# olofson/audiality2

Hardware: AMD Instinct MI355X
Metric: voice-samples/sec + max realtime voices @48kHz (higher is better)
Workload: dtype int32; 1 GPU; 65536 voices 2xwtosc->panmix, 256 per group voice inline->fbdelay->fbdelay (benchmark/fmtest4.a2s delay settings; 256 groups, 512 fbdelays), 48 kHz, fragment=64, stereo (BASELINE configs[3]); voices_per_gpu=65536, chain=osc2-pan, groups=256

## Files before the change

audiality2_amd/build.py:

```python
import hashlib
import os
import shutil
import subprocess

HERE = os.path.dirname(os.path.abspath(__file__))
ROOT = os.path.dirname(HERE)
HIPCC = shutil.which("hipcc") or "/opt/rocm/bin/hipcc"


MARK = b"A2AMD_SRCHASH:"


def source_hash(sources, cmd=()):
    h = hashlib.sha256()
    for s in sources:
        h.update(os.path.basename(s).encode() + b"\0")
        with open(s, "rb") as f:
            h.update(f.read())
        h.update(b"\0")
    h.update(" ".join(cmd).encode())
    return h.hexdigest()[:32]


def stamped_hash(lib, mark=MARK):
    if not os.path.exists(lib):
        return None
    with open(lib, "rb") as f:
        blob = f.read()
    i = blob.find(mark)
    if i < 0:
        return None
    return blob[i + len(mark):i + len(mark) + 32].decode("ascii", "replace")


ENGMARK = b"A2AMD_ENGHASH:"


def engine_hash(engine):
    files = []
    for d in ("include", "src", os.path.join("src", "units"), os.path.join("src", "drivers")):
        p = os.path.join(engine, d)
        if os.path.isdir(p):
            files += [os.path.join(p, f) for f in sorted(os.listdir(p)) if f.endswith((".h", ".h.cmake", ".h.in"))]
    return source_hash(files, (stamped_hash(os.path.join(HERE, "liba2amd_units.so")) or "",))


def _stale(target, want):
    return stamped_hash(target) != want


def _define(h):
    return '-DA2AMD_SRCHASH="%s"' % h


def build_lib(force=False):
    csrc = os.path.join(HERE, "csrc")
    srcs = [os.path.join(csrc, f) for f in ("a2amd_host.cpp", "a2amd_sched.cpp", "a2amd_render.cpp", "a2amd_dist.cpp",
                                            "a2amd_vm.cpp", "a2amd_kernels.hip", "a2amd_fast.hip", "a2amd_vm.hip", "a2amd_wavecap.hip", "a2amd_wavepost.hip", "a2amd_win.hip", "a2amd_vmwin.hip", "a2amd_noise.hip", "a2amd_noisepan.hip", "a2amd_noisefiltpan.hip", "a2amd_cutsweep.hip", "a2amd_oscbare.hip", "a2amd_osc3filtpan.hip")]
    deps = srcs + [os.path.join(csrc, "a2amd_host.h"), os.path.join(csrc, "a2amd_switches.h"), os.path.join(csrc, "a2amd_device.h"), os.path.join(csrc, "a2amd_dsp.h"),
                   os.path.join(csrc, "a2amd_fm.h"), os.path.join(csrc, "a2amd_vmcore.h"), os.path.join(csrc, "a2amd_taps.h"), os.path.join(csrc, "a2amd_winctl.h"), os.path.join(csrc, "a2amd_vmdev.h"), os.path.join(csrc, "a2amd_noisemap.h"), os.path.join(csrc, "a2amd_noisevoice.h"), os.path.join(csrc, "a2amd_settled.h"), os.path.join(csrc, "a2amd_cutsweep.h"), os.path.join(csrc, "a2amd_filt.h"), os.path.join(csrc, "a2amd_wavepads.h"), os.path.join(ROOT, "include", "a2amd.h"),
                   os.path.join(ROOT, "include", "a2amd_noise.h"), os.path.join(ROOT, "include", "a2amd_noisepan.h"), os.path.join(ROOT, "include", "a2amd_noisefilt.h"), os.path.join(ROOT, "include", "a2amd_sweep.h"), os.path.join(ROOT, "include", "a2amd_wavepost.h"),
                   os.path.join(ROOT, "include", "a2amd_bus.h"), os.path.join(ROOT, "include", "a2amd_oscbare.h"), os.path.join(ROOT, "include", "a2amd_osc3filt.h"), os.path.join(ROOT, "include", "a2amd_fbdpan.h"), os.path.join(ROOT, "include", "a2amd_buswin.h"), os.path.join(ROOT, "include", "a2amd_vmbatch.h"), os.path.join(ROOT, "include", "a2amd_osc2.h"), os.path.join(ROOT, "include", "a2amd_osc2lds.h"), os.path.join(ROOT, "include", "a2amd_vm.h")]
    out = os.path.join(HERE, "liba2amd.so")
    flags = ["--offload-arch=gfx950", "-O3", "-std=c++17", "-fPIC", "-shared", "-Wno-unused-value"]
    want = source_hash(deps, flags)
    if force or _stale(out, want):
        subprocess.run([HIPCC] + flags + [_define(want), "-o", out] + srcs, check=True)
    return out


def build_units(force=False):
    src = os.path.join(HERE, "csrc", "a2amd_units.c")
    deps = [src, os.path.join(ROOT, "include", "a2amd.h"), os.path.join(ROOT, "include", "a2amd_noise.h"), os.path.join(ROOT, "include", "a2amd_noisepan.h"),
            os.path.join(ROOT, "include", "a2amd_noisefilt.h"), os.path.join(ROOT, "include", "a2amd_sweep.h"), os.path.join(ROOT, "include", "a2amd_bus.h"),
            os.path.join(ROOT, "include", "a2amd_wavepost.h"), os.path.join(ROOT, "include", "a2amd_oscbare.h"), os.path.join(ROOT, "include", "a2amd_osc3filt.h"), os.path.join(ROOT, "include", "a2amd_fbdpan.h"), os.path.join(ROOT, "include", "a2amd_buswin.h"), os.path.join(ROOT, "include", "a2amd_vmbatch.h"), os.path.join(ROOT, "include", "a2amd_osc2.h"), os.path.join(ROOT, "include", "a2amd_osc2lds.h"), os.path.join(ROOT, "include", "a2amd_plugin.h"),
            os.path.join(ROOT, "include", "a2amd_walk.h"), os.path.join(ROOT, "include", "a2amd_vm.h")]
    out = os.path.join(HERE, "liba2amd_units.so")
    flags = ["-O2", "-Wall", "-fPIC", "-shared"]
    want = source_hash(deps, flags)
    if force or _stale(out, want):
        subprocess.run(["gcc"] + flags + [_define(want), "-o", out, src,
                        "-L" + HERE, "-la2amd", "-ldl", "-lpthread", "-lm", "-Wl,-rpath,$ORIGIN"], check=True)
    return out


def build_walk(force=False, engine=None):
    engine = engine or os.environ.get("A2_ENGINE_SRC", "/root/reference")
    out = os.path.join(HERE, "liba2amd_walk.so")
    src = os.path.join(HERE, "csrc", "a2amd_walk.c")
    own = [src, os.path.join(ROOT, "include", "a2amd_walk.h"), os.path.join(ROOT, "include", "a2amd_vm.h"),
           os.path.join(ROOT, "include", "a2amd_plugin.h")]
    flags = ["-O2", "-Wall", "-fPIC", "-shared"]
    want = source_hash(own, flags)
    kept = os.path.join(ROOT, "oracle", "_ref", "liba2amd_walk.so")
    if not (os.path.exists(os.path.join(engine, "src", "internals.h")) and shutil.which("cmake")):
        if (not os.path.exists(out) or _stale(out, want)) and not _stale(kept, want):
            shutil.copyfile(kept, out)
        if os.path.exists(out) and _stale(out, want):
            raise RuntimeError(f"{out} was not built from this tree's a2amd_walk.c (stamp {stamped_hash(out)}, "
                               f"sources {want}) and the engine's source tree ({engine}) is not here to rebuild it")
        return out if os.path.exists(out) else None
    inc = os.path.join(HERE, "_engine_include")
    weng = engine_hash(engine)
    if force or _stale(out, want) or stamped_hash(out, ENGMARK) != weng:
        subprocess.run(["cmake", f"-DENGINE={engine}", f"-DOUT={inc}", "-P", os.path.join(HERE, "csrc", "engine_header.cmake")],
                       check=True, stdout=subprocess.DEVNULL)
        subprocess.run(["gcc"] + flags + [_define(want), '-DA2AMD_ENGHASH="%s"' % weng, "-I" + inc] +
                       ["-I" + os.path.join(engine, d) for d in ("include", "src", "src/units", "src/drivers")] +
                       ["-o", out, src, "-L" + HERE, "-la2amd_units", "-la2amd", "-ldl", "-lpthread", "-Wl,-rpath,$ORIGIN"],
                       check=True)
    if stamped_hash(kept) != want or stamped_hash(kept, ENGMARK) != weng:
        os.makedirs(os.path.dirname(kept), exist_ok=True)
        shutil.copyfile(out, kept)
    return out


def build_oracle(force=False):
    odir = os.path.join(ROOT, "oracle")
    targets = ["restate"]
    if os.path.exists("/root/reference/src/core.c") and shutil.which("cmake"):
        targets += ["ref", "tools", "optionb"]
    subprocess.run(["make", "-s", "-C", odir] + (["-B"] if force else []) + targets, check=True)
    return os.path.join(odir, "liba2oracle.so")


def build_all(force=False):
    lib = build_lib(force)
    build_units(force)
    build_walk(force)
    return lib, build_oracle(force)
```

audiality2_amd/csrc/a2amd_device.h:

```cpp
#pragma once
#include <stdint.h>

#define A2D_MAXCHAIN   16
#define A2D_CHAIN_INLINE 8
#define A2D_MAXBATCH 256
#define FBW_MAXWIN (2 * A2D_MAXBATCH)
#define A2D_USTATE    24
#define A2D_MAXCH      8
#define A2D_FRAG      64
#define A2D_MIPS      10
#define A2D_FBD_BUFSIZE 131072
#define A2D_MAXPHINC  512
#define A2D_COEF_WORDS 3
#define A2D_WTOSC_MAXLENGTH (0x01000000 - 1 - 131)

enum { A2D_WTOSC = 0, A2D_PANMIX, A2D_FILTER12, A2D_FBDELAY, A2D_INLINE, A2D_XINSERT,
	A2D_FM1, A2D_FM2, A2D_FM3, A2D_FM4, A2D_FM3P, A2D_FM4P, A2D_FM2R, A2D_FM4R,
	A2D_DC, A2D_WAVESHAPER, A2D_DCBLOCK, A2D_LIMITER, A2D_XSINK, A2D_XSOURCE };
#define A2D_IS_FM(k) ((k) >= A2D_FM1 && (k) <= A2D_FM4R)

enum { A2D_OSC_OFF = 0, A2D_OSC_NOISE, A2D_OSC_WAVE, A2D_OSC_MIPWAVE };

#define A2D_DESC(kind, add, nin, nout, wired) \
	(((uint32_t)(kind) << 24) | ((uint32_t)(add) << 4) | ((uint32_t)(nin) << 8) | \
	 ((uint32_t)(nout) << 12) | ((uint32_t)(wired) << 16))
#define A2D_KIND(d)  ((d) >> 24)
#define A2D_ADD(d)   (((d) >> 4) & 1u)
#define A2D_NIN(d)   (((d) >> 8) & 15u)
#define A2D_NOUT(d)  (((d) >> 12) & 15u)
#define A2D_WIRED(d) (((d) >> 16) & 1u)

enum {
	OW_MODE = 0, OW_WAVE, OW_DPHASE, OW_PHASE_LO, OW_PHASE_HI, OW_NOISE,
	OW_PRAMPING, OW_P = 7, OW_A = 11, OW_SEED = 15 };
enum {
	PW_VOL = 0, PW_PAN = 4 };
enum {
	FW_Q = 0, FW_LP = 4, FW_BP, FW_HP, FW_F1, FW_D1A, FW_D1B, FW_D2A, FW_D2B,
	FW_F1NEXT, FW_RAMP };
enum {
	DW_FBDELAY = 0, DW_LDELAY, DW_RDELAY, DW_DRYGAIN, DW_FBGAIN, DW_LGAIN,
	DW_RGAIN, DW_BUFPOS, DW_BUFIDX };

enum {
	CW_VALUE = 0, CW_MODE = 4 };
enum {
	SW_AMOUNT = 0 };
enum {
	BW_F1 = 0, BW_D1A, BW_D1B, BW_D2A, BW_D2B };
enum {
	LW_RELEASE = 0, LW_THRESHOLD, LW_PEAK };
enum {
	MW_SLOT = 0 };
enum {
	FO_A = 0, FO_FB = 4, FO_P = 8, FO_LASTPITCH = 12, FO_PHASE, FO_DPHASE, FO_LAST, FO_WORDS };
#define A2D_FMSTATE 64

#define A2D_WF_RAWTAPS 0x40000000u

struct A2DWave {
	int32_t  type;
	uint32_t flags;
	uint32_t period;
	uint32_t size[A2D_MIPS];
	uint32_t off[A2D_MIPS];
	uint32_t periodic;
};

struct A2DVoice {
	int32_t nunits;
	int32_t unit[A2D_CHAIN_INLINE];
	int32_t out_off, out_nch;
	int32_t own_off, own_nch;
	int32_t pad[3];
};

static_assert(sizeof(A2DVoice) == 64, "the voice record is one 64-byte line");
struct A2DVoiceExt { int32_t unit[A2D_MAXCHAIN - A2D_CHAIN_INLINE]; };

struct A2DRec {
	uint32_t head;
	int32_t  value;
	uint32_t dur;
	uint32_t start;
};
enum { R_SEG = 1, R_WRITE, R_INIT, R_KILL, R_F1SET, R_F1RAMP, R_NOISESEED, R_NOP };
#define A2D_HEAD(frag, op, unit, reg) \
	((uint32_t)(frag) | ((uint32_t)(op) << 16) | ((uint32_t)(unit) << 24) | ((uint32_t)(reg) << 28))
#define A2D_RFRAG(h) ((h) & 0xffffu)
#define A2D_ROP(h)   (((h) >> 16) & 0xffu)
#define A2D_RUNIT(h) (((h) >> 24) & 15u)
#define A2D_RREG(h)  (((h) >> 28) & 15u)

struct A2DRun { int32_t first, count; };

#define A2D_VM_NOWRITE 0xffu
#define A2D_VM_TRAPWRITE 0xfeu
#define A2D_VM_MAXCUT  2
#define A2D_VM_MAXENV  2
#define A2D_VM_MAXPOS  8
#define A2D_VM_ENVPOS  14
#define A2D_ENV_LUTSHIFT 6
#define A2D_ENV_LUTSIZE  (1 << A2D_ENV_LUTSHIFT)
#define A2D_ENV_LUTS     8
struct A2DVmEnv {
	int32_t ramper[4];
	int32_t lut;
	int32_t scale, offset, out;
	int32_t active;
	uint8_t regbase;
	uint8_t k;
	uint8_t target;
	uint8_t pad;
};
struct A2DVmVoice {
	uint32_t waketime;
	uint32_t code, ncode;
	uint16_t pc;
	uint8_t  state, ncut;
	int32_t  voice;
	int32_t  fault;
	uint8_t  cmap[64];
	uint8_t  kind[A2D_MAXCHAIN];
	uint8_t  cutpos[A2D_VM_MAXCUT];
	uint8_t  pad[2];
	int32_t  cut[A2D_VM_MAXCUT][4];
	A2DVmEnv env[A2D_VM_MAXENV];
	int32_t  nenv;
	uint32_t exit_when;
	int32_t  has_exit;
	int32_t  r[64];
};

struct A2DVmParams {
	A2DVmVoice     *vmv;
	const int      *list;
	int32_t         n;
	const uint32_t *code;
	const uint32_t *ptab;
	const int32_t  *f1tab;
	const uint16_t *envlut;
	A2DRun         *runs;
	A2DRun         *vmrun;
	A2DRec         *recs;
	uint32_t        rec_base, rec_cap;
	uint32_t       *total;
	uint32_t        now;
	uint32_t        msdur;
	int32_t         samplerate, basepitch;
	int32_t         nfrags;
	uint8_t         fragframes[A2D_MAXBATCH];
	uint8_t         fragbase[A2D_MAXBATCH];
};

enum { XW_SLOT = 0, XW_MODE = 1 };
#define A2D_XIO_HALF ((size_t)A2D_MAXBATCH * 8 * A2D_FRAG)
#define A2D_XIO_SLOT (2 * A2D_XIO_HALF)

#define A2D_FAST_FCH 8
#define A2D_OSC2_FCH 4
#define A2D_OSC2_SCH 16
#define A2D_OSC2_LDS_ENT 128
#define A2D_MAXVPW   32

struct A2DParams {
	const A2DVoice *voices;
	const A2DVoiceExt *vext;
	const uint32_t *udesc;
	int32_t        *ustate;
	int32_t        *vactive;
	const A2DRun   *runs;
	const A2DRec   *recs;
	const A2DWave  *waves;
	const int16_t  *wavepool;
	const int32_t  *wavecoef;
	int32_t        *busmem;
	int32_t        *fbdmem;
	const uint32_t *ptab;
	int32_t        *fmstate;
	const uint32_t *fmsine;
	int32_t *xio;
	const uint32_t *nseed;
	const int32_t  *nslot;
	int32_t         nnoise;
	const int32_t  *cutf;
	const int32_t  *cslot;
	int32_t         ncut;
	int32_t         nfrags;
	int32_t         samplerate;
	int32_t         debug;
	uint8_t         fragframes[A2D_MAXBATCH];
	uint16_t        fragstart[A2D_MAXBATCH];
};

#ifdef __HIPCC__
#define A2D_HD static inline __host__ __device__
#else
#define A2D_HD static inline
#endif
A2D_HD bool a2d_osc2_slice(int nfrags, int ysplit, int slice, int *c_lo, int *c_hi, int *nslices)
{
	const int nchunks = (nfrags + A2D_OSC2_FCH - 1) / A2D_OSC2_FCH;
	const int per = (nchunks + ysplit - 1) / ysplit;
	*c_lo = slice * per;
	*c_hi = *c_lo + per < nchunks ? *c_lo + per : nchunks;
	*nslices = (nchunks + per - 1) / per;
	return *c_lo < nchunks;
}
A2D_HD bool a2d_osc2_whole(unsigned start_first, unsigned start_last, unsigned frames_last, int n)
{
	return start_last + frames_last - start_first == (unsigned)n * A2D_FRAG;
}

A2D_HD unsigned a2d_osc2_stage(unsigned size0, unsigned periodic0, unsigned size1, unsigned periodic1)
{
	const bool c0 = periodic0 && size0 && !(size0 & (size0 - 1)) && size0 <= A2D_OSC2_LDS_ENT;
	const bool c1 = periodic1 && size1 && !(size1 & (size1 - 1)) && size1 <= A2D_OSC2_LDS_ENT;
	return (c0 ? 1u : 0u) | (c1 && (c0 ? size0 : 0u) + size1 <= A2D_OSC2_LDS_ENT ? 2u : 0u);
}

#ifdef __HIPCC__
static inline __host__ __device__ bool a2d_noise_seed(const A2DParams &p, int f, int ui, unsigned *seed)
{
	if(!p.nseed)
		return false;
	const int k = p.nslot[ui];
	if(k <= 0 || k > p.nnoise)
		return false;
	*seed = p.nseed[(size_t)f * (size_t)p.nnoise + (size_t)(k - 1)];
	return true;
}
#endif

#ifdef __HIPCC__
static inline __host__ __device__ bool a2d_cut_coeff(const A2DParams &p, int f, int ui, int *f1)
{
	if(p.ncut <= 0)
		return false;
#if defined(__HIP_DEVICE_COMPILE__)
	typedef const __attribute__((address_space(4))) A2DParams *CP;
	typedef const __attribute__((address_space(4))) int32_t *CI;
	uintptr_t qa = (uintptr_t)&p;
	asm volatile("" : "+s"(qa));
	const CP q = (CP)qa;
	const int ncut = q->ncut;
	const int k = *((CI)(uintptr_t)q->cslot + ui);
	if(k <= 0 || k > ncut)
		return false;
	const int v = *((CI)(uintptr_t)q->cutf + ((size_t)f * (size_t)ncut + (size_t)(k - 1)));
#else
	const int k = p.cslot[ui];
	if(k <= 0 || k > p.ncut)
		return false;
	const int v = p.cutf[(size_t)f * (size_t)p.ncut + (size_t)(k - 1)];
#endif
	if(v < 0)
		return false;
	*f1 = v;
	return true;
}
#endif

struct A2DCutSweep { int32_t ramper[4]; int32_t unit, slot, pad[2]; };
int a2d_launch_cut_sweep(const A2DCutSweep *list, int n, int f0, int count, unsigned frames, int32_t *cutf, int stride,
		size_t words, int32_t *cslot, int nunits, void *stream);
int a2d_launch_cut_resolve(int32_t *cutf, size_t words, const int32_t *f1tab, void *stream);

struct A2DNoiseOsc { uint32_t ph_lo, ph_hi, dphase; int32_t unit, slot, pad[3]; };
int a2d_launch_noise_seeds(const A2DNoiseOsc *osc, int n, uint32_t start, int f0, int count, unsigned frames,
		uint32_t *seed, int stride, size_t seed_words, int32_t *nslot, int nunits, void *stream);

int a2d_launch_leaf_noisepan(const A2DParams *dparams, const A2DParams &hp, const int *dlist, int nlist, int vpw, void *stream);
int a2d_launch_leaf_noisefiltpan(const A2DParams *dparams, const A2DParams &hp, const int *dlist, int nlist, int vpg, void *stream);
int a2d_launch_leaf_oscbare(const A2DParams *dparams, const A2DParams &hp, const int *dlist, int nlist, int vpw, void *stream);
int a2d_launch_leaf_osc3filtpan(const A2DParams *dparams, const A2DParams &hp, const int *dlist, int nlist, int vpg, void *stream);

int a2d_launch_vm(const A2DVmParams &vp, int emit, void *stream);
int a2d_launch_vm_pool(const A2DVmParams &vp, unsigned *out, void *stream);
#define A2D_WIN_STAGED 2
struct A2DVmwOut {
	A2DVmVoice *vmv;
	int        *ustate;
	int        *vactive;
	A2DRun     *runs;
	uint32_t   *total;
	uint32_t   *idle;
};
int a2d_launch_vm_commit(const A2DVmParams &vp, const A2DParams &hp, int nosc, int filt, const A2DVmwOut &from, void *stream);
int a2d_launch_vm_win(const A2DVmParams &vp, const A2DParams &hp, int nosc, int filt, int fa, int fb, uint32_t now_fa,
		uint32_t batch_end, int *wslot, int *wext, int *wscr, unsigned *widx, unsigned *wtop, unsigned wcap, void *stream,
		const A2DVmwOut *out = nullptr);
#define A2D_VMW_ROW (64 - 1 - 1)

int a2d_launch_voices(const A2DParams *dparams, const int *dlist, int nlist, int vpw, void *stream);
enum { A2D_STAGED_NONE = 0, A2D_STAGED_PHASES, A2D_STAGED_FULL };
struct A2DCommit { const int *list; int nlist, nosc; const int *ustage; const unsigned char *staged; };
struct A2DCommitSet { A2DCommit c[2]; int n; };
int a2d_launch_leaf_oscpan(const A2DParams *dparams, const A2DParams &hp, const int *dlist, int nlist,
		int vpw, int ysplit, int *ustage, unsigned char *staged, void *stream, void *event_after_main, A2DCommit *defer);
int a2d_launch_bus_driver(const A2DParams *dparams, const int *dlist, int nlist, int nfrags, int consume,
		const A2DCommitSet *commits, void *stream, int *master_host = nullptr, int ramping = 0);
int a2d_launch_commit(const A2DParams &hp, const A2DCommit &cm, void *stream);
int a2d_launch_bus_fbdchain(const A2DParams *dparams, const int *dlist, int nlist, int consume, void *stream);
int a2d_launch_bus_fbdpan(const A2DParams *dparams, const int *dlist, int nlist, int consume, void *stream, int windows = 0);
int a2d_launch_park(int32_t *stage, int32_t *bus, unsigned words, void *stream);
int a2d_launch_add_bus(int32_t *dst, int32_t *src, unsigned words, void *stream);
int a2d_launch_add_inject(const int32_t *inj, int32_t *bus, int nch, int n, int nfrags, void *stream);
int a2d_launch_build_coef(const int16_t *pool, int *coef, unsigned lo, unsigned hi, void *stream);
int a2d_launch_capture(const int32_t *bus, int32_t *dst, const uint32_t *fragpos, int nfrags, int nch, void *stream);
int a2d_launch_wave_from_pcm(const int32_t *pcm, int16_t *pool, const uint32_t *off, const uint32_t *size, int levels, int looped,
		int pre, int post, void *stream);
int a2d_launch_wave_level0(const int32_t *pcm, int16_t *d, unsigned size, void *stream);
int a2d_launch_wave_finish(int16_t *pool, const uint32_t *off, const uint32_t *size, int levels, int looped, int pre, int post,
		void *stream);
unsigned a2d_wavepost_scratch_words(unsigned size, unsigned flags, unsigned chunk);
int a2d_launch_wave_level0_post(const int32_t *pcm, int16_t *d, unsigned size, unsigned flags, unsigned chunk, uint32_t *scratch,
		void *stream);
int a2d_osc2filtpan_max_vpg(void);
int a2d_launch_leaf_osc2filtpan(const A2DParams *dparams, const A2DParams &hp, const int *dlist, int nlist,
		int vpg, void *stream);
int a2d_launch_leaf_oscfiltpan(const A2DParams *dparams, const A2DParams &hp, const int *dlist, int nlist,
		int vpw, void *stream);
int a2d_launch_scatter_runs(const int *didx, const A2DRun *dval, int n, A2DRun *druns, void *stream);
int a2d_launch_leaf_osc2pan(const A2DParams *dparams, const A2DParams &hp, const int *dlist, int nlist,
		int vpw, int ysplit, int *ustage, unsigned char *staged, void *stream, A2DCommit *defer, int voice_major, int lds_taps,
		int *ysplit_used);
struct A2Switches;
int a2d_launch_leaf_recs(const A2Switches &sw, const A2DParams *dparams, const A2DParams &hp, int nosc, int filt, const int *dlist,
		int nlist, int vpw, void *stream, int skip_empty = 0);
#define A2D_WIN_WORDS 24
#define A2D_WIN_SLOTWORDS(nosc, filt) ((filt) ? ((nosc) == 1 ? 20 : 24) : ((nosc) == 1 ? 12 : 20))
int a2d_launch_win_ctl(const A2DParams *dparams, const A2DParams &hp, int nosc, int filt, const int *dlist, int nlist,
		int skip_empty, int fa, int fb, int *wslot, int *wext, unsigned *widx, unsigned *wtop, unsigned wcap, int *wrc,
		void *stream);
int a2d_launch_win_render(const A2Switches &sw, const A2DParams &hp, int nosc, int filt, const int *dlist, int nlist, int fa, int fb,
		const int *wslot, const int *wext, const unsigned *widx, void *stream);
int a2d_launch_leaf_recs_all(const A2Switches &sw, const A2DParams *dparams, const A2DParams &hp, const int *const *lists, const int *counts,
		int vpw, void *stream, int skip_mask = 0);
int a2d_launch_leaf_fmpan(const A2DParams *dparams, const A2DParams &hp, int kind, const int *dlist, int nlist,
		int vpw, void *stream);
int a2d_launch_leaf_fmpan_all(const A2DParams *dparams, const A2DParams &hp, const int *dlist,
		const int *count8, int vpw, void *stream);
```

audiality2_amd/csrc/a2amd_fast.hip:

```cpp
#include <hip/hip_runtime.h>
#include <type_traits>
#include <algorithm>
#include <stdlib.h>
#include "a2amd_device.h"
#include "a2amd_switches.h"
#include "a2amd_dsp.h"
#include "a2amd_fm.h"
#include "a2amd_filt.h"

#include "a2amd_taps.h"

__global__ void k_build_coef(const int16_t *__restrict__ pool, int *__restrict__ coef, unsigned lo, unsigned hi)
{
	const unsigned j = lo + blockIdx.x * blockDim.x + threadIdx.x;
	if(j >= hi)
		return;
	const int dm = pool[j - 1], d0 = pool[j], d1 = pool[j + 1], d2 = pool[j + 2];
	const int c = (d1 - dm) >> 1;
	const int a = (3 * (d0 - d1) + d2 - dm) >> 1;
	const int b = dm - d0 + c - a;
	int *e = coef + A2D_COEF_WORDS * (size_t)j;
	e[0] = a;
	e[1] = b;
	e[2] = (int)(((unsigned)c << 16) | ((unsigned)d0 & 0xffffu));
}

int a2d_launch_build_coef(const int16_t *pool, int *coef, unsigned lo, unsigned hi, void *stream)
{
	if(hi <= lo)
		return 0;
	hipLaunchKernelGGL(k_build_coef, dim3((hi - lo + 255) / 256), dim3(256), 0, (hipStream_t)stream, pool, coef, lo, hi);
	return (int)hipGetLastError();
}

__device__ __attribute__((noinline)) int cold_ramp_delta(int target, int value, int timer, int frames,
		int *newtimer)
{
	if(frames <= (timer >> 8)) {
		*newtimer = wsub(timer, frames << 8);
		if(timer > 0)
			return (int)div_trunc_exact((int64_t)wsub(target, value) * 256, timer);
		return (int)((((int64_t)wsub(target, value)) * 256) / timer);
	}
	*newtimer = 0;
	if(frames > 0)
		return (int)div_trunc_exact((int64_t)wsub(target, value), frames);
	return wsub(target, value) / frames;
}

__device__ __attribute__((noinline)) uint64_t cold_umod64(uint64_t a, uint64_t m)
{
	return a % m;
}

DEV uint64_t wrap_phase(uint64_t ph, unsigned size)
{
	if(ph >> 56) {
		uint64_t r = cold_umod64(ph, (uint64_t)size << 24);
		return (uint64_t)(unsigned)rfl((int)(unsigned)r) | ((uint64_t)(unsigned)rfl((int)(unsigned)(r >> 32)) << 32);
	}
	unsigned hi = (unsigned)(ph >> 24);
	if(hi >= size) {
		if(!(size & (size - 1)))
			hi &= size - 1;
		else
			hi = (unsigned)rfl((int)(hi % size));
		ph = ((uint64_t)hi << 24) | (ph & 0xffffffu);
	}
	return ph;
}

DEV void ramp_prepare_s(Ramp &r, int frames)
{
	if(r.timer == 0) {
		r.value = r.target;
		r.delta = 0;
	} else {
		int nt;
		int d = cold_ramp_delta(r.target, r.value, r.timer, frames, &nt);
		r.delta = rfl(d);
		r.timer = rfl(nt);
	}
}

struct OscS {
	int mode, wave;
	unsigned dphase;
	uint64_t phase;
	int p_ramping;
	Ramp p, a;
	int noise;
	unsigned seed;
};

struct FastPtrs {
	const int16_t *wavepool;
	const A2DWave *waves;
	const uint32_t *ptab;
	int dbg;
};

struct OscPend { Quad16 qa, qb; unsigned ph, ph2; int ak, x; bool taps; };

DEV int osc_fragment_end(const OscPend &pd)
{
	if(pd.taps)
		return mul64s(inter_quads(pd.qa, pd.qb, pd.ph, pd.ph2), pd.ak, 17);
	return pd.x;
}

DEV OscPend osc_fragment_begin(const FastPtrs &g, OscS &o, int nframes, int lane)
{
	OscPend pd;
	pd.qa.lo = pd.qa.hi = pd.qb.lo = pd.qb.hi = 0;
// ... 55 lines not shown
		ramp_prepare_s(o.a, nframes);
		const uint64_t phk = o.phase + (uint64_t)(unsigned)(in ? lane : 0) * o.dphase;
		const uint64_t nph = phk + o.dphase;
		const bool draw = in && ((o.dphase >= (1u << 23)) || ((nph ^ phk) >> 23));
		const unsigned long long m = __ballot(draw);
		const int me = (int)(threadIdx.x & 63);
		const unsigned long long below = (me >= 63) ? ~0ull : ((2ull << me) - 1ull);
		const int mine = __popcll(m & below), total = __popcll(m);
		int held = o.noise, myval = o.noise;
		unsigned st = o.seed;
		for(int j = 1; j <= total; ++j) {
			held = noise_next(st) - 32767;
			if(j == mine)
				myval = held;
		}
		o.seed = st;
		o.noise = held;
		if(in) {
			int ak = wadd(o.a.value, wmul(o.a.delta, lane));
			x = wmul(myval, ak >> 10) >> 6;
		}
		o.phase += (uint64_t)(unsigned)nframes * o.dphase;
		ramp_run(o.a, nframes);
	} else {
		ramp_prepare_s(o.p, nframes);
		ramp_prepare_s(o.a, nframes);
		ramp_run(o.p, nframes);
		ramp_run(o.a, nframes);
	}
	pd.x = x;
	return pd;
}

DEV int osc_fragment_s(const FastPtrs &g, OscS &o, int nframes, int lane)
{
	const OscPend pd = osc_fragment_begin(g, o, nframes, lane);
	return osc_fragment_end(pd);
}

DEV void pan_fragment_s(Ramp &vol, Ramp &pan, int x, int nframes, int lane, int &acc0, int &acc1)
{
	const bool clamp = a2s_pan_over(pan.target) || a2s_pan_over(pan.value);
	ramp_prepare_s(vol, nframes);
	ramp_prepare_s(pan, nframes);
	if((unsigned)lane < (unsigned)nframes) {
		int vk = wadd(vol.value, wmul(vol.delta, lane));
		int pk = wadd(pan.value, wmul(pan.delta, lane));
		int vp = mul64s(pk, vk, 24);
		int v0 = wsub(vk, vp), v1 = wadd(vk, vp);
		if(clamp) {
			int lim = wshl(vk, 1);
			if(v0 > lim) v0 = lim;
			if(v1 > lim) v1 = lim;
		}
		acc0 = wadd(acc0, mul64s(x, v0, 24));
		acc1 = wadd(acc1, mul64s(x, v1, 24));
	}
	ramp_run(vol, nframes);
	ramp_run(pan, nframes);
}

DEV void oscpan_fragment(const FastPtrs &g, OscS &o, Ramp &vol, Ramp &pan,
		int nframes, int lane, int &acc0, int &acc1)
{
	int x = osc_fragment_s(g, o, nframes, lane);
	pan_fragment_s(vol, pan, x, nframes, lane, acc0, acc1);
}

DEV int frames_of(const int (&ffr)[A2D_MAXBATCH / 64], int f)
{
	int r = 0;
#pragma unroll
	for(int k = 0; k < A2D_MAXBATCH / 64; ++k)
		if((f >> 6) == k)
			r = rdl(ffr[k], f & 63);
	return r;
}

enum { SV_MODE = 0, SV_WAVE, SV_DPHASE, SV_PHLO, SV_PHHI, SV_PRAMP, SV_P = 6, SV_A = 10,
	SV_VOL = 14, SV_PAN = 18, SV_NWORDS = 22 };

enum { DV_SETTLED = 0, DV_MM, DV_DPH, DV_SIZEM, DV_DOFF, DV_V0, DV_V1, DV_NWORDS };

DEV bool settled_wave(const A2DWave *w, unsigned dphase, int *d, bool settled = true, unsigned *periodic = nullptr)
{
	unsigned dph;
	const unsigned mm = a2s_mip(dphase, w->period, &dph);
	d[0] = (int)mm;
	d[1] = (int)dph;
	d[2] = (int)w->size[mm];
	d[3] = (int)w->off[mm];
	if(periodic)
		*periodic = (w->periodic >> mm) & 1u;
	return settled && a2s_wave_ok(w->size[0], w->flags, dph);
}

DEV void osc_from_mem(OscS &o, const volatile int *w)
{
	o.mode = rfl(w[OW_MODE]);
	o.wave = rfl(w[OW_WAVE]);
	o.dphase = (unsigned)rfl(w[OW_DPHASE]);
	o.phase = (uint64_t)(unsigned)rfl(w[OW_PHASE_LO]) | ((uint64_t)(unsigned)rfl(w[OW_PHASE_HI]) << 32);
	o.p_ramping = rfl(w[OW_PRAMPING]);
	o.p.value = rfl(w[OW_P]); o.p.target = rfl(w[OW_P + 1]);
	o.p.delta = rfl(w[OW_P + 2]); o.p.timer = rfl(w[OW_P + 3]);
	o.a.value = rfl(w[OW_A]); o.a.target = rfl(w[OW_A + 1]);
	o.a.delta = rfl(w[OW_A + 2]); o.a.timer = rfl(w[OW_A + 3]);
	o.noise = 0;
	o.seed = 0;
}

DEV void osc_to_mem(int *w, const OscS &o)
{
	w[OW_MODE] = o.mode;
	w[OW_WAVE] = o.wave;
	w[OW_DPHASE] = (int)o.dphase;
	w[OW_PHASE_LO] = (int)(unsigned)o.phase;
	w[OW_PHASE_HI] = (int)(unsigned)(o.phase >> 32);
	w[OW_PRAMPING] = o.p_ramping;
	w[OW_P] = o.p.value; w[OW_P + 1] = o.p.target; w[OW_P + 2] = o.p.delta; w[OW_P + 3] = o.p.timer;
	w[OW_A] = o.a.value; w[OW_A + 1] = o.a.target; w[OW_A + 2] = o.a.delta; w[OW_A + 3] = o.a.timer;
}

DEV void stage_mark(unsigned char *m, bool mine, bool settled, bool last_slice, bool walker)
{
	if(mine && !settled) {
		if(walker)
			*m = A2D_STAGED_FULL;
	} else if(last_slice)
		*m = mine ? A2D_STAGED_PHASES : A2D_STAGED_NONE;
}

#define OSC1_WPE 4
__global__ __launch_bounds__(64 * FAST_WPB) __attribute__((amdgpu_waves_per_eu(OSC1_WPE, OSC1_WPE)))
void k_leaf_oscpan(const A2DParams *__restrict__ pp, const int *__restrict__ list, int nlist, int vpw,
		int ysplit, const A2DVoice *__restrict__ voices, const int *ustate,
		int *ustage, const int16_t *__restrict__ wavepool,
		const A2DWave *__restrict__ waves, const uint32_t *__restrict__ ptab, int *__restrict__ busmem,
		const int *__restrict__ wavecoef, unsigned char *__restrict__ staged)
{
	const A2DParams &p = *pp;
	const int wv = rfl((int)(threadIdx.x >> 6));
	const int lane = threadIdx.x & 63;
	const int first = (blockIdx.x * FAST_WPB + wv) * vpw;
	if(first >= nlist)
		return;
	const int nv = min(vpw, nlist - first);
	const int nfrags = p.nfrags;
	const int dbg = p.debug;
	FastPtrs g = { wavepool, waves, ptab, dbg };
	const CoefRsrc crs = coef_rsrc(wavecoef);

	const int nchunks = (nfrags + FAST_FCH - 1) / FAST_FCH;
	const int per = (nchunks + ysplit - 1) / ysplit;
	const int slice = blockIdx.y;
	const int c_lo = slice * per, c_hi = min(nchunks, c_lo + per);
	const bool last_slice = c_hi >= nchunks;
	if(c_lo >= nchunks)
		return;
	const int nslices = (nchunks + per - 1) / per;

	int ffr[A2D_MAXBATCH / 64], fst[A2D_MAXBATCH / 64];
#pragma unroll
	for(int k = 0; k < A2D_MAXBATCH / 64; ++k) {
		ffr[k] = (k * 64 + lane < nfrags) ? p.fragframes[k * 64 + lane] : 0;
		fst[k] = (k * 64 + lane < nfrags) ? p.fragstart[k * 64 + lane] : 0;
	}

	int dv[DV_NWORDS], amp_l = 0, phlo_l = 0, phhi_l = 0;
	int u0 = 0, u1 = 0, my_off = -1, my_nch = 2;
	bool mine = false;
#pragma unroll
	for(int k = 0; k < DV_NWORDS; ++k)
		dv[k] = 0;
	if(lane < nv)
		mine = p.runs[list[first + lane]].count == 0;
// ... 183 lines not shown
			flush_acc(busmem, cur_off, cur_nch, f0, nf, lane, dbg, acc0, acc1);
			__builtin_amdgcn_fence(__ATOMIC_RELEASE, "wavefront");
			__builtin_amdgcn_s_waitcnt(0);
		}
	}

	if(mine && dv[DV_SETTLED] && last_slice) {
		int *w0 = ustage + (size_t)u0 * A2D_USTATE;
		w0[OW_PHASE_LO] = phlo_l;
		w0[OW_PHASE_HI] = phhi_l;
	}
	if(ustage != ustate && lane < nv)
		stage_mark(staged + first + lane, mine, dv[DV_SETTLED] != 0, last_slice, lane % nslices == slice);
}

DEV void commit_block(const A2DCommit &cm, int block, const A2DVoice *__restrict__ voices, int *__restrict__ ustate)
{
	const int i = block * 256 + threadIdx.x;
	if(i >= cm.nlist * cm.nosc)
		return;
	const int e = i / cm.nosc, o = i - e * cm.nosc;
	const int what = cm.staged[e];
	if(what == A2D_STAGED_NONE)
		return;
	const A2DVoice &vc = voices[cm.list[e]];
	const size_t a = (size_t)vc.unit[o] * A2D_USTATE;
	ustate[a + OW_PHASE_LO] = cm.ustage[a + OW_PHASE_LO];
	ustate[a + OW_PHASE_HI] = cm.ustage[a + OW_PHASE_HI];
	if(what != A2D_STAGED_FULL)
		return;
	for(int k = 0; k < 15; ++k)
		if(k != OW_NOISE && k != OW_PHASE_LO && k != OW_PHASE_HI)
			ustate[a + k] = cm.ustage[a + k];
	if(o == 0) {
		const size_t ap = (size_t)vc.unit[cm.nosc] * A2D_USTATE;
		for(int k = 0; k < 8; ++k)
			ustate[ap + k] = cm.ustage[ap + k];
	}
}

DEV int commit_blocks(const A2DCommit &cm) { return (cm.nlist * cm.nosc + 255) / 256; }

__global__ __launch_bounds__(256)
void k_commit_oscpan(A2DCommit cm, const A2DVoice *__restrict__ voices, int *__restrict__ ustate)
{
	commit_block(cm, blockIdx.x, voices, ustate);
}

#define OSC2_FCH A2D_OSC2_FCH
#define OSC2_SCH A2D_OSC2_SCH
static_assert(OSC2_SCH % OSC2_FCH == 0, "a super-chunk is whole chunks");
enum { OV_MODE = 0, OV_WAVE, OV_DPHASE, OV_PHLO, OV_PHHI, OV_PRAMP, OV_P = 6, OV_A = 10, OV_NWORDS = 14 };
enum { OD_MM = 0, OD_DPH, OD_SIZEM, OD_DOFF, OD_NWORDS };

DEV void osc_from_lanes(OscS &o, const int (&so)[OV_NWORDS], int v)
{
	o.mode = rdl(so[OV_MODE], v);
	o.wave = rdl(so[OV_WAVE], v);
	o.dphase = (unsigned)rdl(so[OV_DPHASE], v);
	o.phase = (uint64_t)(unsigned)rdl(so[OV_PHLO], v) | ((uint64_t)(unsigned)rdl(so[OV_PHHI], v) << 32);
	o.p_ramping = rdl(so[OV_PRAMP], v);
	o.p.value = rdl(so[OV_P], v); o.p.target = rdl(so[OV_P + 1], v);
	o.p.delta = rdl(so[OV_P + 2], v); o.p.timer = rdl(so[OV_P + 3], v);
	o.a.value = rdl(so[OV_A], v); o.a.target = rdl(so[OV_A + 1], v);
	o.a.delta = rdl(so[OV_A + 2], v); o.a.timer = rdl(so[OV_A + 3], v);
	o.noise = 0;
	o.seed = 0;
}

DEV void osc_to_lanes(int (&so)[OV_NWORDS], const OscS &o, bool me)
{
	WRL(so[OV_MODE], o.mode);
	WRL(so[OV_WAVE], o.wave);
	WRL(so[OV_DPHASE], (int)o.dphase);
	WRL(so[OV_PHLO], (int)(unsigned)o.phase);
	WRL(so[OV_PHHI], (int)(unsigned)(o.phase >> 32));
	WRL(so[OV_PRAMP], o.p_ramping);
	WRL(so[OV_P], o.p.value); WRL(so[OV_P + 1], o.p.target);
	WRL(so[OV_P + 2], o.p.delta); WRL(so[OV_P + 3], o.p.timer);
	WRL(so[OV_A], o.a.value); WRL(so[OV_A + 1], o.a.target);
	WRL(so[OV_A + 2], o.a.delta); WRL(so[OV_A + 3], o.a.timer);
}

struct Osc2Voice {
	unsigned dph[2], sizem[2];
	int cb[2], amp[2];
	uint64_t ph[2], end[2];
};
struct Osc2Lds {
	const LdsInt *level[2];
	unsigned lg[2];
};

template<bool WHOLE, int ST = 0>
DEV void osc2_chunk(const CoefRsrc &crs, Osc2Voice &s, const unsigned (&ldph)[2], const int (&nfr)[OSC2_FCH],
		const unsigned (&pre)[OSC2_FCH], int nf, bool park, int (&xs)[OSC2_FCH], const Osc2Lds &lv = Osc2Lds())
{
	Coef4 ka[2][OSC2_FCH], kb[2][OSC2_FCH];
	unsigned pa[2][OSC2_FCH], pb[2][OSC2_FCH];
#pragma unroll
	for(int o = 0; o < 2; ++o) {
		const unsigned dph = s.dph[o], sizem = s.sizem[o];
		uint64_t ph = s.ph[o];
		uint64_t phs[OSC2_FCH];
		if(!(sizem & (sizem - 1)) && !(ph >> 48)) {
			const uint64_t mask = ((uint64_t)sizem << 24) - 1;
#pragma unroll
			for(int j = 0; j < OSC2_FCH; ++j)
				phs[j] = (ph + (uint64_t)dph * (WHOLE ? (unsigned)(j * A2D_FRAG) : pre[j])) & mask;
			ph = phs[OSC2_FCH - 1] + (uint64_t)dph * (WHOLE ? (unsigned)A2D_FRAG : (unsigned)nfr[OSC2_FCH - 1]);
		} else {
#pragma unroll
			for(int j = 0; j < OSC2_FCH; ++j) {
				ph = wrap_phase(ph, sizem);
				phs[j] = ph;
				ph += (uint64_t)dph * (WHOLE ? (unsigned)A2D_FRAG : (unsigned)nfr[j]);
			}
		}
#pragma unroll
		for(int j = 0; j < OSC2_FCH; ++j) {
			pa[o][j] = tap_phase(phs[j], ldph[o]);
			asm("" : "+v"(pa[o][j]));
			pb[o][j] = pa[o][j] + (dph >> 17);
			if((ST >> o) & 1) {
				ka[o][j] = coef_lds(lv.level[o], pa[o][j], lv.lg[o]);
				kb[o][j] = coef_lds(lv.level[o], pb[o][j], lv.lg[o]);
			} else {
				ka[o][j] = coef_at(crs, s.cb[o], pa[o][j]);
				kb[o][j] = coef_at(crs, s.cb[o], pb[o][j]);
			}
		}
		if(park) {
			uint64_t e = ph;
#pragma unroll
			for(int j = OSC2_FCH - 2; j >= 0; --j)
				if(nf == j + 1)
					e = phs[j] + (uint64_t)dph * (WHOLE ? (unsigned)A2D_FRAG : (unsigned)nfr[j]);
			s.end[o] = e;
		}
		s.ph[o] = ph;
	}
#pragma unroll
	for(int o = 0; o < 2; ++o)
#pragma unroll
		for(int j = 0; j < OSC2_FCH; ++j) {
			const int y = mul64s(inter_coefs(ka[o][j], pa[o][j], kb[o][j], pb[o][j]), s.amp[o], 17);
			xs[j] = o ? wadd(xs[j], y) : y;
		}
}

DEV void osc2_voice_from_lanes(Osc2Voice &s, unsigned (&ldph)[2], unsigned (&mm)[2], const int (&od)[2][OD_NWORDS],
		const int (&amp_l)[2], const int (&phlo_l)[2], const int (&phhi_l)[2], int v, unsigned before, int lane)
{
#pragma unroll
	for(int o = 0; o < 2; ++o) {
		mm[o] = (unsigned)rdl(od[o][OD_MM], v);
		s.dph[o] = (unsigned)rdl(od[o][OD_DPH], v);
		s.sizem[o] = (unsigned)rdl(od[o][OD_SIZEM], v);
		s.cb[o] = coef_base((unsigned)rdl(od[o][OD_DOFF], v));
		s.amp[o] = rdl(amp_l[o], v);
		const uint64_t phase = (uint64_t)(unsigned)rdl(phlo_l[o], v) | ((uint64_t)(unsigned)rdl(phhi_l[o], v) << 32);
		s.ph[o] = (phase >> mm[o]) + (uint64_t)before * s.dph[o];
		ldph[o] = lane_dph(lane, s.dph[o]);
	}
}

template<int ST>
DEV void osc2_voice_chunks(const CoefRsrc &crs, Osc2Voice &s, const unsigned (&ldph)[2], const unsigned (&mm)[2],
		const Osc2Lds &lv, int nsc, int nfs, bool last, int v0, int v1, int v, int lane, int (*tile)[2][A2D_FRAG],
		int (&phlo_l)[2], int (&phhi_l)[2])
{
	const int nopre_i[OSC2_FCH] = { 0, 0, 0, 0 };
	const unsigned nopre_u[OSC2_FCH] = { 0, 0, 0, 0 };
	for(int k = 0; k < nsc; ++k) {
		const bool park = last && k == nsc - 1;
		int xs[OSC2_FCH];
		osc2_chunk<true, ST>(crs, s, ldph, nopre_i, nopre_u, nfs - k * OSC2_FCH, park, xs, lv);
#pragma unroll
		for(int j = 0; j < OSC2_FCH; ++j) {
			tile_add(&tile[k * OSC2_FCH + j][0][lane], mul64s(xs[j], v0, 24));
			tile_add(&tile[k * OSC2_FCH + j][1][lane], mul64s(xs[j], v1, 24));
		}
		if(park) {
			const bool me = lane == v;
#pragma unroll
			for(int o = 0; o < 2; ++o) {
				const uint64_t endph = s.end[o] << mm[o];
				WRL(phlo_l[o], (int)(unsigned)endph);
				WRL(phhi_l[o], (int)(unsigned)(endph >> 32));
			}
		}
	}
}

template<bool STAGE>
DEV void osc2_superchunk(const CoefRsrc &crs, const int *wavecoef, int *busmem, const int (&od)[2][OD_NWORDS],
		const int (&amp_l)[2], int (&phlo_l)[2], int (&phhi_l)[2], int settled_l, int my_off, int my_nch, int v0l, int v1l,
		int nv, int nsc, int fa, int nfs, bool last, unsigned before, int lane, int dbg, int (*tile)[2][A2D_FRAG],
		LdsInt *level)
{
	int cur_off = rdl(my_off, 0), cur_nch = rdl(my_nch, 0);
	for(int v = 0; v < nv; ++v) {
		const int sl = rdl(settled_l, v);
		if(!sl)
			continue;
		const int voff = rdl(my_off, v);
		if(voff != cur_off) {
			flush_tile(busmem, cur_off, cur_nch, fa, nfs, nsc * OSC2_FCH, lane, dbg, tile);
			cur_off = voff;
			cur_nch = rdl(my_nch, v);
		}
		const int v0 = rdl(v0l, v), v1 = rdl(v1l, v);
		Osc2Voice s;
		unsigned ldph[2], mm[2];
		osc2_voice_from_lanes(s, ldph, mm, od, amp_l, phlo_l, phhi_l, v, before, lane);
		Osc2Lds lv = { { level, level }, { 0, 0 } };
		if(!STAGE) {
			osc2_voice_chunks<0>(crs, s, ldph, mm, lv, nsc, nfs, last, v0, v1, v, lane, tile, phlo_l, phhi_l);
			continue;
		}
		const int st = sl >> 1;
		if(st) {
			lds_wave_fence();
			if(st & 1) {
				lv.lg[0] = (unsigned)__builtin_ctz(s.sizem[0]);
				stage_level(level, wavecoef, s.cb[0], s.sizem[0], lane);
			}
			if(st & 2) {
				LdsInt *const l1 = (st & 1) ? level + s.sizem[0] * A2D_COEF_WORDS : level;
				lv.level[1] = l1;
				lv.lg[1] = (unsigned)__builtin_ctz(s.sizem[1]);
				stage_level(l1, wavecoef, s.cb[1], s.sizem[1], lane);
			}
			lds_wave_fence();
		}
		switch(st) {
		case 0: osc2_voice_chunks<0>(crs, s, ldph, mm, lv, nsc, nfs, last, v0, v1, v, lane, tile, phlo_l, phhi_l); break;
		case 1: osc2_voice_chunks<1>(crs, s, ldph, mm, lv, nsc, nfs, last, v0, v1, v, lane, tile, phlo_l, phhi_l); break;
		case 2: osc2_voice_chunks<2>(crs, s, ldph, mm, lv, nsc, nfs, last, v0, v1, v, lane, tile, phlo_l, phhi_l); break;
		default: osc2_voice_chunks<3>(crs, s, ldph, mm, lv, nsc, nfs, last, v0, v1, v, lane, tile, phlo_l, phhi_l); break;
		}
	}
	flush_tile(busmem, cur_off, cur_nch, fa, nfs, nsc * OSC2_FCH, lane, dbg, tile);
}

#define OSC2_WPE 4
__global__ __launch_bounds__(64 * FAST_WPB) __attribute__((amdgpu_waves_per_eu(OSC2_WPE, OSC2_WPE)))
void k_leaf_osc2pan(const A2DParams *__restrict__ pp, const int *__restrict__ list, int nlist, int vpw,
		int ysplit, const A2DVoice *__restrict__ voices, const int *ustate, int *ustage,
		const int16_t *__restrict__ wavepool, const A2DWave *__restrict__ waves,
		const uint32_t *__restrict__ ptab, int *__restrict__ busmem, const int *__restrict__ wavecoef,
		unsigned char *__restrict__ staged, int vmajor, int lds_taps)
{
	const A2DParams &p = *pp;
	const int wv = rfl((int)(threadIdx.x >> 6));
	const int lane = threadIdx.x & 63;
	const int first = (blockIdx.x * FAST_WPB + wv) * vpw;
	if(first >= nlist)
		return;
	const int nv = min(vpw, nlist - first);
	const int nfrags = p.nfrags;
	const int dbg = p.debug;
	FastPtrs g = { wavepool, waves, ptab, dbg };
	const CoefRsrc crs = coef_rsrc(wavecoef);

	const int slice = blockIdx.y;
	int c_lo, c_hi, nslices;
	if(!a2d_osc2_slice(nfrags, ysplit, slice, &c_lo, &c_hi, &nslices))
		return;
	const bool last_slice = c_hi * OSC2_FCH >= nfrags;

	int ffr[A2D_MAXBATCH / 64], fst[A2D_MAXBATCH / 64];
#pragma unroll
	for(int k = 0; k < A2D_MAXBATCH / 64; ++k) {
		ffr[k] = (k * 64 + lane < nfrags) ? p.fragframes[k * 64 + lane] : 0;
		fst[k] = (k * 64 + lane < nfrags) ? p.fragstart[k * 64 + lane] : 0;
	}

	int od[2][OD_NWORDS], amp_l[2] = { 0, 0 }, phlo_l[2] = { 0, 0 }, phhi_l[2] = { 0, 0 };
	int v0l = 0, v1l = 0, settled_l = 0;
	int uu[3] = { 0, 0, 0 }, my_off = -1, my_nch = 2;
	bool mine = false;
#pragma unroll
	for(int o = 0; o < 2; ++o)
#pragma unroll
		for(int k = 0; k < OD_NWORDS; ++k)
			od[o][k] = 0;
	if(lane < nv)
		mine = p.runs[list[first + lane]].count == 0;
	if(mine) {
		const A2DVoice &vc = voices[list[first + lane]];
		my_off = vc.out_off;
		my_nch = vc.out_nch;
		bool settled = true;
		int wave_l[2], dphase_l[2];
		unsigned periodic[2] = { 0, 0 };
#pragma unroll
		for(int o = 0; o < 2; ++o) {
			uu[o] = vc.unit[o];
			const int *w = ustate + (size_t)uu[o] * A2D_USTATE;
			wave_l[o] = w[OW_WAVE];
			dphase_l[o] = w[OW_DPHASE];
			amp_l[o] = w[OW_A];
			phlo_l[o] = w[OW_PHASE_LO];
			phhi_l[o] = w[OW_PHASE_HI];
			settled = settled && a2s_osc_settled(w[OW_MODE], (unsigned)dphase_l[o], w[OW_PRAMPING], w + OW_P, w + OW_A);
		}
		uu[2] = vc.unit[2];
		const int *wp = ustate + (size_t)uu[2] * A2D_USTATE;
		int sp[8];
#pragma unroll
		for(int k = 0; k < 8; ++k)
			sp[k] = wp[k];
		settled = settled && a2s_arrived(sp + PW_VOL, sp + PW_PAN);
		if(settled) {
#pragma unroll
			for(int o = 0; o < 2; ++o)
				settled = settled_wave(waves + wave_l[o], (unsigned)dphase_l[o], od[o], settled, &periodic[o]);
			a2s_pan_gains(sp[PW_VOL], sp[PW_PAN], a2s_pan_over(sp[PW_PAN]), &v0l, &v1l);
		}
		settled_l = settled ? 1 : 0;
		if(settled && lds_taps)
			settled_l |= (int)a2d_osc2_stage((unsigned)od[0][OD_SIZEM], periodic[0], (unsigned)od[1][OD_SIZEM], periodic[1]) << 1;
	}
	const unsigned long long unsettled_mask = __ballot(mine && !settled_l);
	const bool any_staged = __ballot(settled_l > 1) != 0;

	__shared__ int tiles[FAST_WPB][OSC2_SCH][2][A2D_FRAG];
	__shared__ int levels[FAST_WPB][A2D_OSC2_LDS_ENT * A2D_COEF_WORDS];
	int (*const tile)[2][A2D_FRAG] = tiles[wv];
	LdsInt *const level = (LdsInt *)levels[wv];
	if(vmajor)
#pragma unroll
		for(int r = 0; r < OSC2_SCH; ++r)
			tile[r][0][lane] = tile[r][1][lane] = 0;
	for(int s_lo = c_lo; s_lo < c_hi; s_lo += OSC2_SCH / OSC2_FCH) {
		const int s_hi = min(c_hi, s_lo + OSC2_SCH / OSC2_FCH);
		const int fa = s_lo * OSC2_FCH, nfs = min(nfrags, s_hi * OSC2_FCH) - fa;
		const bool last = last_slice && s_hi == c_hi;
		const unsigned before = (unsigned)frames_of(fst, fa);
		if(vmajor && a2d_osc2_whole(before, (unsigned)frames_of(fst, fa + nfs - 1), (unsigned)frames_of(ffr, fa + nfs - 1), nfs)) {
			if(any_staged)
				osc2_superchunk<true>(crs, wavecoef, busmem, od, amp_l, phlo_l, phhi_l, settled_l, my_off, my_nch, v0l, v1l,
						nv, s_hi - s_lo, fa, nfs, last, before, lane, dbg, tile, level);
			else
				osc2_superchunk<false>(crs, wavecoef, busmem, od, amp_l, phlo_l, phhi_l, settled_l, my_off, my_nch, v0l, v1l,
						nv, s_hi - s_lo, fa, nfs, last, before, lane, dbg, tile, level);
			continue;
		}
		for(int c = s_lo; c < s_hi; ++c) {
			const int f0 = c * OSC2_FCH;
			const int nf = min((int)OSC2_FCH, nfrags - f0);
			int acc0[OSC2_FCH], acc1[OSC2_FCH], nfr[OSC2_FCH];
#pragma unroll
			for(int j = 0; j < OSC2_FCH; ++j) {
				acc0[j] = acc1[j] = 0;
				nfr[j] = (j < nf) ? frames_of(ffr, f0 + j) : 0;
			}
			const unsigned before = (unsigned)frames_of(fst, f0);
			unsigned pre[OSC2_FCH];
			pre[0] = 0;
#pragma unroll
			for(int j = 1; j < OSC2_FCH; ++j)
				pre[j] = pre[j - 1] + (unsigned)nfr[j - 1];
			const bool park = last && c == s_hi - 1;
			int cur_off = rdl(my_off, 0), cur_nch = rdl(my_nch, 0);
			for(int v = 0; v < nv; ++v) {
				if(!rdl(settled_l, v))
					continue;
				const int voff = rdl(my_off, v);
				if(voff != cur_off) {
					flush_acc(busmem, cur_off, cur_nch, f0, nf, lane, dbg, acc0, acc1);
					cur_off = voff;
					cur_nch = rdl(my_nch, v);
				}
				const int v0 = rdl(v0l, v), v1 = rdl(v1l, v);
				Osc2Voice s;
				unsigned ldph[2], mm[2];
				int xs[OSC2_FCH];
				osc2_voice_from_lanes(s, ldph, mm, od, amp_l, phlo_l, phhi_l, v, before, lane);
				osc2_chunk<false>(crs, s, ldph, nfr, pre, nf, park, xs);
#pragma unroll
				for(int j = 0; j < OSC2_FCH; ++j) {
					const int x = (lane < nfr[j]) ? xs[j] : 0;
					acc0[j] = wadd(acc0[j], mul64s(x, v0, 24));
					acc1[j] = wadd(acc1[j], mul64s(x, v1, 24));
				}
				if(park) {
					const bool me = lane == v;
#pragma unroll
					for(int o = 0; o < 2; ++o) {
						const uint64_t endph = s.end[o] << mm[o];
						WRL(phlo_l[o], (int)(unsigned)endph);
						WRL(phhi_l[o], (int)(unsigned)(endph >> 32));
					}
				}
			}
			flush_acc(busmem, cur_off, cur_nch, f0, nf, lane, dbg, acc0, acc1);
		}
	}

	const unsigned long long todo_mask = unsettled_mask & __ballot(lane % nslices == slice);
	if(todo_mask) {
		for(int f0 = 0; f0 < nfrags; f0 += OSC2_FCH) {
			const int nf = min((int)OSC2_FCH, nfrags - f0);
			int acc0[OSC2_FCH], acc1[OSC2_FCH];
#pragma unroll
			for(int j = 0; j < OSC2_FCH; ++j)
				acc0[j] = acc1[j] = 0;
			int cur_off = rdl(my_off, 0), cur_nch = rdl(my_nch, 0);
			for(int v = 0; v < nv; ++v) {
				if(!((todo_mask >> v) & 1ull))
					continue;
				const int voff = rdl(my_off, v);
				if(voff != cur_off) {
					flush_acc(busmem, cur_off, cur_nch, f0, nf, lane, dbg, acc0, acc1);
					cur_off = voff;
					cur_nch = rdl(my_nch, v);
				}
				OscS oa, ob;
				Ramp vol, pan;
				const int *src = f0 ? ustage : ustate;
				osc_from_mem(oa, src + (size_t)rdl(uu[0], v) * A2D_USTATE);
				osc_from_mem(ob, src + (size_t)rdl(uu[1], v) * A2D_USTATE);
				{
// ... 1838 lines not shown
						++r;
					wk = lane - ((fr[r][4] >> 8) & 0xff);
				}
				const int vk = wadd(fr[r][0], wmul(fr[r][1], wk));
				const int pk = wadd(fr[r][2], wmul(fr[r][3], wk));
				const int vp = mul64s(pk, vk, 24);
				v0 = wsub(vk, vp); v1 = wadd(vk, vp);
				if(WIN ? fr[r][4] & 1 : fr[r][4]) {
					const int lim = wshl(vk, 1);
					if(v0 > lim) v0 = lim;
					if(v1 > lim) v1 = lim;
				}
			}
			const int o0 = mul64s(x0, v0, 24), o1 = mul64s(x1, v1, 24);
			int *dst = out + (size_t)f * out_nch * A2D_FRAG;
			if(o0)
				atomicAdd(&dst[lane], o0);
			if(o1)
				atomicAdd(&dst[A2D_FRAG + lane], o1);
		}
		if(fend < nfrags)
			__syncthreads();
	}
	if(threadIdx.x == 0) {
		int total = 0;
		for(int f = 0; f < nfrags; ++f)
			total += p.fragframes[f];
#pragma unroll
		for(int k = 0; k < FBC_MAXD; ++k)
			if(k < nd)
				p.ustate[(size_t)vc.unit[k + 1] * A2D_USTATE + DW_BUFPOS] = wadd(d[k].pos, total);
	}
}

__global__ __launch_bounds__(FBC_THREADS)
void k_bus_fbdpan(const A2DParams *__restrict__ pp, const int *__restrict__ list, int nlist, int consume)
{
	bus_fbdpan<false>(pp, list, consume);
}

__global__ __launch_bounds__(FBC_THREADS)
void k_bus_fbdpan_win(const A2DParams *__restrict__ pp, const int *__restrict__ list, int nlist, int consume)
{
	bus_fbdpan<true>(pp, list, consume);
}

int a2d_launch_bus_fbdpan(const A2DParams *dparams, const int *dlist, int nlist, int consume, void *stream, int windows)
{
	if(nlist <= 0)
		return 0;
	hipLaunchKernelGGL(windows ? k_bus_fbdpan_win : k_bus_fbdpan, dim3(nlist), dim3(FBC_THREADS), 0, (hipStream_t)stream,
			dparams, dlist, nlist, consume);
	return (int)hipGetLastError();
}

int a2d_launch_leaf_oscpan(const A2DParams *dparams, const A2DParams &hp, const int *dlist, int nlist,
		int vpw, int ysplit, int *ustage, unsigned char *staged, void *stream, void *event_after_main, A2DCommit *defer)
{
	if(nlist <= 0)
		return 0;
	vpw = vpw < 1 ? 1 : (vpw > 64 ? 64 : vpw);
	if(ysplit < 1 || !ustage || !staged)
		ysplit = 1;
	int nwaves = (nlist + vpw - 1) / vpw;
	int nblocks = (nwaves + FAST_WPB - 1) / FAST_WPB;
	hipLaunchKernelGGL(k_leaf_oscpan, dim3(nblocks, ysplit), dim3(64 * FAST_WPB), 0, (hipStream_t)stream,
			dparams, dlist, nlist, vpw, ysplit, hp.voices, (const int *)hp.ustate,
			ysplit > 1 ? ustage : hp.ustate, hp.wavepool, hp.waves, hp.ptab, hp.busmem, hp.wavecoef, staged);
	if(event_after_main)
		hipEventRecord((hipEvent_t)event_after_main, (hipStream_t)stream);
	if(ysplit > 1) {
		A2DCommit cm = { dlist, nlist, 1, ustage, staged };
		if(defer)
			*defer = cm;
		else
			a2d_launch_commit(hp, cm, stream);
	} else if(defer)
		defer->nlist = 0;
	return (int)hipGetLastError();
}

int a2d_launch_leaf_osc2pan(const A2DParams *dparams, const A2DParams &hp, const int *dlist, int nlist,
		int vpw, int ysplit, int *ustage, unsigned char *staged, void *stream, A2DCommit *defer, int voice_major, int lds_taps,
		int *ysplit_used)
{
	if(nlist <= 0)
		return 0;
	vpw = vpw < 1 ? 1 : (vpw > 64 ? 64 : vpw);
	if(ysplit < 1 || !ustage || !staged)
		ysplit = 1;
	if(ysplit_used)
		*ysplit_used = ysplit;
	int nwaves = (nlist + vpw - 1) / vpw;
	int nblocks = (nwaves + FAST_WPB - 1) / FAST_WPB;
	hipLaunchKernelGGL(k_leaf_osc2pan, dim3(nblocks, ysplit), dim3(64 * FAST_WPB), 0, (hipStream_t)stream,
			dparams, dlist, nlist, vpw, ysplit, hp.voices, (const int *)hp.ustate,
			ysplit > 1 ? ustage : hp.ustate, hp.wavepool, hp.waves, hp.ptab, hp.busmem, hp.wavecoef, staged, voice_major, lds_taps);
	if(ysplit > 1) {
		A2DCommit cm = { dlist, nlist, 2, ustage, staged };
		if(defer)
			*defer = cm;
		else
			a2d_launch_commit(hp, cm, stream);
	} else if(defer)
		defer->nlist = 0;
	return (int)hipGetLastError();
}

__global__ void k_scatter_runs(const int *__restrict__ idx, const A2DRun *__restrict__ val, int n,
		A2DRun *__restrict__ runs)
{
	int i = blockIdx.x * blockDim.x + threadIdx.x;
	if(i < n)
		runs[idx[i]] = val[i];
}

int a2d_launch_scatter_runs(const int *didx, const A2DRun *dval, int n, A2DRun *druns, void *stream)
{
	if(n <= 0)
		return 0;
	hipLaunchKernelGGL(k_scatter_runs, dim3((n + 255) / 256), dim3(256), 0, (hipStream_t)stream,
			didx, dval, n, druns);
	return (int)hipGetLastError();
}

int a2d_launch_leaf_oscfiltpan(const A2DParams *dparams, const A2DParams &hp, const int *dlist, int nlist,
		int vpg, void *stream)
{
	if(nlist <= 0)
		return 0;
	vpg = vpg < 1 ? 1 : (vpg > FILT_MAXV ? FILT_MAXV : vpg);
	int nblocks = (nlist + vpg - 1) / vpg;
	size_t lds = (size_t)3 * vpg * FILT_PITCH * sizeof(int);
	hipLaunchKernelGGL(k_leaf_oscfiltpan, dim3(nblocks), dim3(64 * FILT_WAVES), lds, (hipStream_t)stream,
			dparams, dlist, nlist, vpg, hp.voices, hp.ustate, hp.wavepool, hp.waves, hp.ptab, hp.busmem, hp.wavecoef);
	return (int)hipGetLastError();
}

int a2d_osc2filtpan_max_vpg(void)
{
	const int nfull = FILT_WAVES - 1 - (FILT_WAVES / 4 - 1);
	const int v = nfull * (FILT2_LAUNCHV < FILT2_FASTV ? FILT2_LAUNCHV : FILT2_FASTV);
	return v > FILT_MAXV ? FILT_MAXV : v;
}

int a2d_launch_leaf_osc2filtpan(const A2DParams *dparams, const A2DParams &hp, const int *dlist, int nlist,
		int vpg, void *stream)
{
	if(nlist <= 0)
		return 0;
	vpg = vpg < 1 ? 1 : (vpg > FILT_MAXV ? FILT_MAXV : vpg);
	int nblocks = (nlist + vpg - 1) / vpg;
	size_t lds = (size_t)3 * vpg * FILT_PITCH * sizeof(int);
	hipLaunchKernelGGL(k_leaf_osc2filtpan, dim3(nblocks), dim3(64 * FILT_WAVES), lds, (hipStream_t)stream,
			dparams, dlist, nlist, vpg, hp.voices, hp.ustate, hp.wavepool, hp.waves, hp.ptab, hp.busmem, hp.wavecoef);
	return (int)hipGetLastError();
}

enum { PV_VOL = 0, PV_PAN = 4, PV_NWORDS = 8 };

DEV void pan_window_s(Ramp &vol, Ramp &pan, int x, int off, int len, int lane, int &acc0, int &acc1)
{
	const bool clamp = a2s_pan_over(pan.target) || a2s_pan_over(pan.value);
	ramp_prepare_s(vol, len);
	ramp_prepare_s(pan, len);
	const int k = lane - off;
	if(k >= 0 && k < len) {
		int vk = wadd(vol.value, wmul(vol.delta, k));
		int pk = wadd(pan.value, wmul(pan.delta, k));
		int vp = mul64s(pk, vk, 24);
		int v0 = wsub(vk, vp), v1 = wadd(vk, vp);
		if(clamp) {
			int lim = wshl(vk, 1);
			if(v0 > lim) v0 = lim;
			if(v1 > lim) v1 = lim;
		}
		acc0 = wadd(acc0, mul64s(x, v0, 24));
		acc1 = wadd(acc1, mul64s(x, v1, 24));
	}
	ramp_run(vol, len);
// ... 459 lines not shown
```

audiality2_amd/csrc/a2amd_host.cpp:

```cpp
#include "a2amd_host.h"
#include "a2amd_noisemap.h"
#include "a2amd_cutsweep.h"
#include "a2amd_settled.h"
#include "a2amd_wavepads.h"

namespace a2h { thread_local char g_err[256] = ""; }

extern "C" {

const char *a2amd_version(void) { return "a2amd 0.1 (gfx950)"; }
#ifndef A2AMD_SRCHASH
#define A2AMD_SRCHASH "unstamped"
#endif
const char *a2amd_source_stamp(void) { return "A2AMD_SRCHASH:" A2AMD_SRCHASH; }

const char *a2amd_last_error(const a2amd_ctx *c) { return c ? c->err : g_err; }

int a2amd_device_count(void)
{
	int n = 0;
	return hipGetDeviceCount(&n) == hipSuccess ? n : 0;
}


int a2amd_open(const a2amd_config *cfg, a2amd_ctx **out)
{
	if(!cfg || !out || cfg->channels < 1 || cfg->channels > A2D_MAXCH || cfg->samplerate <= 0) {
		snprintf(g_err, sizeof(g_err), "a2amd_open: bad configuration");
		return A2AMD_EINVAL;
	}
	int ndev = 0;
	hipError_t e = hipGetDeviceCount(&ndev);
	if(e != hipSuccess || ndev <= 0 || cfg->device >= ndev) {
		snprintf(g_err, sizeof(g_err), "a2amd_open: no usable HIP device (%s, %d devices, want #%d); "
				"this library has no CPU fallback", hipGetErrorString(e), ndev, cfg->device);
		return A2AMD_ENODEVICE;
	}
	a2amd_ctx *c = new a2amd_ctx();
	c->cfg = *cfg;
	c->err[0] = 0;
	if(!c->cfg.max_batch)
		c->cfg.max_batch = 1;
	if(c->cfg.max_batch > A2D_MAXBATCH)
		c->cfg.max_batch = A2D_MAXBATCH;
	memset(&c->stats, 0, sizeof(c->stats));
	build_pitch_table(c->ptab);
	a2amd_read_switches(&c->sw);
	c->bus_stride_frames = (size_t)c->cfg.max_batch * A2D_FRAG;
	c->bus_used = c->bus_stride_frames * (size_t)c->cfg.channels;
#define OPENCHK(call) do { hipError_t e_ = (call); if(e_ != hipSuccess) { \
	snprintf(g_err, sizeof(g_err), "a2amd_open: %s: %s", #call, hipGetErrorString(e_)); \
	delete c; return A2AMD_EHIP; } } while(0)
	OPENCHK(hipSetDevice(cfg->device));
	if(cfg->stream)
		c->stream = (hipStream_t)cfg->stream;
	else {
		OPENCHK(hipStreamCreateWithFlags(&c->stream, hipStreamNonBlocking));
		c->own_stream = true;
	}
	OPENCHK(hipEventCreate(&c->ev0));
	OPENCHK(hipEventCreate(&c->ev1));
	OPENCHK(hipEventCreate(&c->ev2));
	c->ev_pool.push_back(c->ev0);
	c->ev_pool.push_back(c->ev1);
	c->ev_pool.push_back(c->ev2);
	OPENCHK(hipMalloc((void **)&c->d_ptab, sizeof(c->ptab)));
	OPENCHK(hipMalloc((void **)&c->d_wavepool.d, (size_t)(8u << 20) * sizeof(int16_t)));
	c->d_wavepool.cap = 8u << 20;
	OPENCHK(hipMalloc((void **)&c->d_wavecoef.d, (size_t)(8u << 20) * A2D_COEF_WORDS * sizeof(int32_t)));
	c->d_wavecoef.cap = 8u << 20;
#undef OPENCHK
	*out = c;
	return A2AMD_OK;
}

void a2amd_close(a2amd_ctx *c)
{
	if(!c)
		return;
	use_device(c);
	hipStreamSynchronize(c->stream);
	if(c->vm.pred_stream)
		hipStreamSynchronize(c->vm.pred_stream);
	drop_graphs(c);
	if(c->comm && g_rccl.CommDestroy)
		g_rccl.CommDestroy(c->comm);
	if(c->grp_ev)
		hipEventDestroy(c->grp_ev);
	hipFree(c->d_voices.d); hipFree(c->d_vext.d); hipFree(c->d_udesc.d); hipFree(c->d_ustate.d); hipFree(c->d_ustage.d);
	hipFree(c->d_vactive.d); hipFree(c->d_runs.d); hipFree(c->d_recs.d);
	hipFree(c->d_nseed.d); hipFree(c->d_nslot.d);
	hipFree(c->d_cutf.d); hipFree(c->d_cslot.d);
	hipFree(c->d_win.d); hipFree(c->d_wext.d); hipFree(c->d_wscr.d); hipFree(c->d_wrc.d); hipFree(c->d_widx.d); hipFree(c->d_wtop);
	if(c->h_wtop)
		hipHostFree(c->h_wtop);
	if(c->wtop_ev)
		hipEventDestroy(c->wtop_ev);
	if(c->win_stream)
		hipStreamDestroy(c->win_stream);
	for(int k = 0; k < 7; ++k)
		if(c->win_fork[k])
			hipStreamDestroy(c->win_fork[k]);
	for(int k = 0; k < 8; ++k)
		if(c->win_fev[k])
			hipEventDestroy(c->win_fev[k]);
	for(int k = 0; k < 5; ++k)
		if(c->win_ev[k])
			hipEventDestroy(c->win_ev[k]);
	hipFree(c->d_waves.d); hipFree(c->d_wavepool.d); hipFree(c->d_wavecoef.d); hipFree(c->d_busmem.d);
	vm_close(c);
	hipFree(c->capture.d); hipFree(c->capture.d_fragpos); hipFree(c->d_wavepost.d);
	hipFree(c->d_fbdmem.d); hipFree(c->d_fmstate.d); hipFree(c->d_xio.d); hipFree(c->d_fmsine); hipFree(c->d_list.d); hipFree(c->d_staged.d); hipFree(c->d_scatter.d); hipFree(c->d_ptab); hipFree(c->d_blob.d);
	for(int k = 0; k < 2; ++k) { if(c->h_blob[k]) hipHostFree(c->h_blob[k]); if(c->blob_ev[k]) hipEventDestroy(c->blob_ev[k]); }
	if(c->h_master)
		hipHostFree(c->h_master);
	for(int k = 0; k < 2; ++k) { if(c->rb[k].h) hipHostFree(c->rb[k].h); if(c->rb[k].ev) hipEventDestroy(c->rb[k].ev); }
	for(hipEvent_t e : c->ev_pool)
		hipEventDestroy(e);
	if(c->own_stream)
		hipStreamDestroy(c->stream);
	delete c;
}

int a2amd_set_pitch_table(a2amd_ctx *c, const uint32_t *t)
{
	memcpy(c->ptab, t, sizeof(c->ptab));
	c->ptab_dirty = true;
	return A2AMD_OK;
}

int a2amd_get_pitch_table(const a2amd_ctx *c, uint32_t *t)
{
	memcpy(t, c->ptab, sizeof(c->ptab));
	return A2AMD_OK;
}

}
namespace a2h {
void wave_tap_policy(a2amd_ctx *c)
{
	const int force = c->sw.raw;
	const size_t budget = (size_t)c->sw.coef_cache_mb << 20;
	const bool big = c->wavepool_used * (4 * A2D_COEF_WORDS) > budget;
	for(size_t i = 0; i < c->waves.size(); ++i) {
		HWave &w = c->waves[i];
		if(!w.live || w.dw.type != A2AMD_WMIPWAVE)
			continue;
		const bool raw = force >= 0 ? force != 0 : (big && w.dw.size[0] >= 4096);
		const uint32_t f = (w.dw.flags & ~A2D_WF_RAWTAPS) | (raw ? A2D_WF_RAWTAPS : 0u);
		if(f != w.dw.flags) {
			w.dw.flags = f;
			c->mwaves[i].flags = f;
			c->waves_dirty = true;
		}
	}
}
}
extern "C" {
}

struct a2amd_capture {
	int32_t *d;
	size_t n;
	int device;
};

namespace a2h {
int capture_append(a2amd_ctx *c)
{
	a2amd_ctx::Capture &cp = c->capture;
	std::vector<uint32_t> pos((size_t)c->nfrags + 1);
	size_t n = cp.n;
	for(int f = 0; f < c->nfrags; ++f) {
		pos[f] = (uint32_t)n;
		n += c->fragframes[f];
	}
	pos[c->nfrags] = (uint32_t)n;
	if(n > 0x7fffffffu)
		return c->fail(A2AMD_ENOMEM, "capture beyond 2^31 frames");
	if(n > cp.cap) {
		const size_t ncap = std::max(n * 2, (size_t)1 << 16);
		int32_t *nd = nullptr;
		HIPCHK(c, hipMalloc((void **)&nd, ncap * sizeof(int32_t)));
		if(cp.n)
			HIPCHK(c, hipMemcpyAsync(nd, cp.d, cp.n * sizeof(int32_t), hipMemcpyDeviceToDevice, c->stream));
		HIPCHK(c, hipStreamSynchronize(c->stream));
		hipFree(cp.d);
		cp.d = nd;
		cp.cap = ncap;
	}
	if(!cp.d_fragpos)
		HIPCHK(c, hipMalloc((void **)&cp.d_fragpos, (A2D_MAXBATCH + 1) * sizeof(uint32_t)));
	HIPCHK(c, hipMemcpyAsync(cp.d_fragpos, pos.data(), pos.size() * sizeof(uint32_t), hipMemcpyHostToDevice, c->stream));
	HIPCHK(c, hipStreamSynchronize(c->stream));
	if(a2d_launch_capture(c->d_busmem.d, cp.d, cp.d_fragpos, c->nfrags, c->cfg.channels, c->stream))
		return c->fail(A2AMD_EHIP, "capture launch failed");
	cp.n = n;
	return 0;
}
}

extern "C" {

int a2amd_capture_begin(a2amd_ctx *c)
{
	if(c->comm)
		return c->fail(A2AMD_EUNSUPPORTED, "capture in a distributed context");
	c->capture.on = true;
	c->capture.n = 0;
	drop_graphs(c);
	return A2AMD_OK;
}

int a2amd_capture_end(a2amd_ctx *c, a2amd_capture **out)
{
	if(!out)
		return c->fail(A2AMD_EINVAL, "capture_end: null");
	*out = nullptr;
	use_device(c);
	HIPCHK(c, hipStreamSynchronize(c->stream));
	if(c->capture.on && c->capture.n) {
		a2amd_capture *cap = new a2amd_capture;
		cap->d = c->capture.d;
		cap->n = c->capture.n;
		cap->device = c->cfg.device;
		c->capture.d = nullptr;
// ... 43 lines not shown
	if(cap->device != c->cfg.device)
		return c->fail(A2AMD_EUNSUPPORTED, "wave_upload_captured: the capture lives on GPU %d, the context on %d", cap->device, c->cfg.device);
	if(w->type != A2AMD_WWAVE && w->type != A2AMD_WMIPWAVE)
		return c->fail(A2AMD_EUNSUPPORTED, "wave_upload_captured: wave type %d", w->type);
	if((size_t)w->size[0] != cap->n)
		return c->fail(A2AMD_EUNSUPPORTED, "wave_upload_captured: the wave has %u samples, the capture %zu", w->size[0], cap->n);
	for(int l = 1; l < (w->type == A2AMD_WMIPWAVE ? A2D_MIPS : 1); ++l)
		if(w->size[l] != ((w->size[0] + (1u << l) - 1) >> l))
			return c->fail(A2AMD_EINVAL, "wave_upload_captured: level %d has %u samples", l, w->size[l]);
	return A2AMD_OK;
}

int a2amd_wave_upload_captured(a2amd_ctx *c, uint64_t key, const a2amd_wavedesc *w, const a2amd_capture *cap)
{
	if(w && cap && (w->flags & 0x000d0000u))
		return c->fail(A2AMD_EUNSUPPORTED, "wave_upload_captured: flags %#x ask for post-processing", w->flags);
	if(int r = captured_refusals(c, w, cap))
		return r;
	return wave_place(c, key, w, cap);
}

int a2amd_wave_upload_captured_post(a2amd_ctx *c, uint64_t key, const a2amd_wavedesc *w, const a2amd_capture *cap, unsigned chunk)
{
	if(int r = captured_refusals(c, w, cap))
		return r;
	if(w->flags & 0x00080000u)
		return c->fail(A2AMD_EUNSUPPORTED, "wave_upload_captured_post: A2_REVMIX (the reference's result is not defined)");
	if((w->flags & 0x00040000u) && w->size[0] < 2)
		return c->fail(A2AMD_EUNSUPPORTED, "wave_upload_captured_post: A2_XFADE on %u samples", w->size[0]);
	if((w->flags & 0x00010000u) && !chunk)
		return c->fail(A2AMD_EUNSUPPORTED, "wave_upload_captured_post: A2_NORMALIZE needs the size of the writes");
	use_device(c);
	if(int r = grow(c, c->d_wavepost, a2d_wavepost_scratch_words(w->size[0], w->flags, chunk), 1, false))
		return r;
	return wave_place(c, key, w, cap, chunk);
}

static int wave_place(a2amd_ctx *c, uint64_t key, const a2amd_wavedesc *w, const a2amd_capture *cap, unsigned chunk)
{
	use_device(c);
	int id = -1;
	for(size_t i = 0; i < c->waves.size(); ++i)
		if(c->waves[i].live && c->waves[i].key == key)
			id = (int)i;
	if(id < 0) {
		if(!c->free_wave_slots.empty()) {
			id = c->free_wave_slots.back();
			c->free_wave_slots.pop_back();
		} else {
			id = (int)c->waves.size();
			c->waves.push_back(HWave());
			c->mwaves.push_back(A2DWave());
		}
	} else {
		if(c->waves[id].pool_len)
			c->deferred_wavepool_free.push_back(std::make_pair(c->waves[id].pool_off, c->waves[id].pool_len));
		--c->stats.live_waves;
	}
	HWave &hw = c->waves[id];
	hw.live = true;
	hw.key = key;
	memset(&hw.dw, 0, sizeof(hw.dw));
	hw.dw.type = w->type;
	hw.dw.flags = w->flags;
	hw.dw.period = w->period;
	int levels = w->type == A2AMD_WMIPWAVE ? A2D_MIPS : w->type == A2AMD_WWAVE ? 1 : 0;
	size_t total = 0;
	for(int l = 0; l < levels; ++l)
		total += A2AMD_WAVEPRE + (size_t)w->size[l] + A2AMD_WAVEPOST;
	total = (total + 7) & ~(size_t)7;
	size_t pos = (size_t)-1;
	for(size_t k = 0; k < c->wavepool_free.size() && total; ++k)
		if(c->wavepool_free[k].second >= total) {
			pos = c->wavepool_free[k].first;
			c->wavepool_free[k].first += total;
			c->wavepool_free[k].second -= total;
			if(!c->wavepool_free[k].second)
				c->wavepool_free.erase(c->wavepool_free.begin() + (long)k);
			HIPCHK(c, hipStreamSynchronize(c->stream));
			break;
		}
	if(pos == (size_t)-1) {
		if(c->wavepool_used + total > c->d_wavepool.cap) {
			if((c->wavepool_used + total) * (4 * A2D_COEF_WORDS) > (((size_t)1 << 32) - 4096))
				return c->fail(A2AMD_ENOMEM, "wave pool beyond %zu samples", (((size_t)1 << 32) - 4096) / (4 * A2D_COEF_WORDS));
			if(int r = grow(c, c->d_wavepool, c->wavepool_used + total, 1, true)) return r;
			if(int r = grow(c, c->d_wavecoef, c->d_wavepool.cap, A2D_COEF_WORDS, false)) return r;
			if(c->wavepool_used > 3 && a2d_launch_build_coef(c->d_wavepool.d, c->d_wavecoef.d, 1,
					(unsigned)c->wavepool_used - 2, c->stream))
				return c->fail(A2AMD_EHIP, "coefficient build failed");
			c->waves_dirty = true;
			drop_graphs(c);
			c->blob_quiet = false;
		}
		pos = c->wavepool_used;
		c->wavepool_used += total;
	}
	hw.pool_off = pos;
	hw.pool_len = total;
	uint32_t loff[A2D_MIPS] = { 0 }, lsize[A2D_MIPS] = { 0 };
	const size_t pos0 = pos;
	for(int l = 0; l < levels; ++l) {
		size_t n = A2AMD_WAVEPRE + (size_t)w->size[l] + A2AMD_WAVEPOST;
		if(!cap) {
			HIPCHK(c, hipMemcpy(c->d_wavepool.d + pos, w->data[l], n * sizeof(int16_t), hipMemcpyHostToDevice));
			c->wave_h2d_bytes += n * sizeof(int16_t);
			if((w->flags & 0x100u) && a2w_pads_periodic(w->data[l], w->size[l], A2AMD_WAVEPRE, A2AMD_WAVEPOST))
				hw.dw.periodic |= 1u << l;
		}
		loff[l] = (uint32_t)(pos - pos0);
		lsize[l] = w->size[l];
		hw.dw.size[l] = w->size[l];
		hw.dw.off[l] = (uint32_t)(pos + A2AMD_WAVEPRE);
		pos += n;
	}
	if(cap) {
		int16_t *pool0 = c->d_wavepool.d + pos0;
		const int looped = (w->flags & 0x100u) != 0;
		if(levels && ((w->flags & 0x00050000u)
				? a2d_launch_wave_level0_post(cap->d, pool0 + A2AMD_WAVEPRE, lsize[0], w->flags, chunk, c->d_wavepost.d, c->stream) ||
					a2d_launch_wave_finish(pool0, loff, lsize, levels, looped, A2AMD_WAVEPRE, A2AMD_WAVEPOST, c->stream)
				: a2d_launch_wave_from_pcm(cap->d, pool0, loff, lsize, levels, looped, A2AMD_WAVEPRE, A2AMD_WAVEPOST, c->stream)))
			return c->fail(A2AMD_EHIP, "wave build from capture failed");
		++c->waves_resident;
	} else
		++c->waves_uploaded;
	if(total > 3 && a2d_launch_build_coef(c->d_wavepool.d, c->d_wavecoef.d, (unsigned)hw.pool_off + 1,
			(unsigned)(hw.pool_off + total) - 2, c->stream))
		return c->fail(A2AMD_EHIP, "coefficient build failed");
	c->mwaves[id] = hw.dw;
	c->waves_dirty = true;
	++c->stats.live_waves;
	wave_tap_policy(c);
	return id;
}

int a2amd_wave_drop(a2amd_ctx *c, uint64_t key)
{
	for(size_t i = 0; i < c->waves.size(); ++i)
		if(c->waves[i].live && c->waves[i].key == key) {
			c->waves[i].live = false;
			c->waves[i].dw.size[0] = 0;
			if(c->waves[i].pool_len)
				c->deferred_wavepool_free.push_back(std::make_pair(c->waves[i].pool_off, c->waves[i].pool_len));
			c->waves[i].pool_len = 0;
			c->waves[i].key = 0;
			c->deferred_wave_slots.push_back((int)i);
			if(!c->nfrags && !c->frag_open) {
				for(auto &r : c->deferred_wavepool_free)
					wavepool_release(c, r.first, r.second);
				c->deferred_wavepool_free.clear();
			}
			c->mwaves[i] = c->waves[i].dw;
			c->waves_dirty = true;
			--c->stats.live_waves;
			return A2AMD_OK;
		}
	return c->fail(A2AMD_EINVAL, "wave_drop: unknown key");
}

int a2amd_fragment(a2amd_ctx *c, unsigned frames)
{
	if(!frames || frames > A2D_FRAG)
		return c->fail(A2AMD_EINVAL, "fragment of %u frames", frames);
	if(!c->stack.empty())
		return c->fail(A2AMD_ESTATE, "fragment inside an inline window");
	if(c->uploaded)
		return c->fail(A2AMD_ESTATE, "batch already uploaded; finish the render first");
	close_fragment(c);
	if(c->nfrags >= (int)c->cfg.max_batch)
		return c->fail(A2AMD_ESTATE, "more than max_batch=%u fragments without a render", c->cfg.max_batch);
	if(!c->nfrags)
		c->vm.batch_time = c->walk_time;
	c->cur_frag = c->nfrags++;
	c->walk_serial = c->serial_base + c->cur_frag;
	c->fragframes[c->cur_frag] = frames;
	c->fragbase[c->cur_frag] = 0;
	c->frag_open = true;
	c->walked_started = 0;
	c->building = -1;
	if(c->defmap_dirty || c->defmap.size() < c->voices.size() + 4096) {
		if(c->defmap.size() < c->voices.size() + 4096)
			c->defmap.assign(c->voices.size() * 2 + 65536, 0);
		else
			std::fill(c->defmap.begin(), c->defmap.begin() + std::min(c->defmap.size(), c->voices.size()), 0);
		c->defmap_dirty = false;
	}
	c->defmap_used = false;
	return A2AMD_OK;
}

int a2amd_fragment_offset(a2amd_ctx *c, unsigned offset)
{
	if(!c->frag_open || c->uploaded)
		return c->fail(A2AMD_ESTATE, "fragment_offset outside a fragment");
	if(offset + c->fragframes[c->cur_frag] > A2D_FRAG)
		return c->fail(A2AMD_EINVAL, "fragment_offset %u with %u frames", offset, c->fragframes[c->cur_frag]);
	c->fragbase[c->cur_frag] = (uint8_t)offset;
	return A2AMD_OK;
}

namespace {
int sweep_stretch_check(a2amd_ctx *c, const char *who, unsigned frames, unsigned count)
{
	if(!frames || frames > A2D_FRAG)
		return c->fail(A2AMD_EINVAL, "fragment of %u frames", frames);
	if(!c->stack.empty())
		return c->fail(A2AMD_ESTATE, "fragment inside an inline window");
	if(c->uploaded)
		return c->fail(A2AMD_ESTATE, "batch already uploaded; finish the render first");
// ... 1170 lines not shown
```

audiality2_amd/csrc/a2amd_host.h:

```cpp
#ifndef A2AMD_HOST_H
#define A2AMD_HOST_H
#include <hip/hip_runtime.h>
#include <rccl/rccl.h>
#include <dlfcn.h>
#include <math.h>
#include <stdarg.h>
#include <stdio.h>
#include <stdlib.h>
#include <string.h>
#include <algorithm>
#include <map>
#include <vector>
#include <future>

#include "../../include/a2amd.h"
#include "../../include/a2amd_vm.h"
#include "a2amd_device.h"
#include "a2amd_switches.h"

#ifndef M_PI
#define M_PI 3.14159265358979323846
#endif

namespace a2h {
// ... 339 lines not shown
	a2amd_sweep_batch_info last_sweeps = {};
	uint32_t n_cut_standin = 0;
	uint32_t n_cut_windows = 0;
	bool owners_all_driver = false;
	bool consume_ok = false;
	bool others_clean = false;
	bool root_clean = false;
	bool capturing = false;
	int n_clients = 0;
	int sub_resume = -1;
	int paused_at = 0;
	std::vector<int32_t> snap_ustate, snap_vactive;
	bool snap_valid = false;
	std::vector<uint8_t> defmap;
	bool defmap_used = false;
	bool defmap_dirty = false;
	std::vector<uint8_t> held;
	size_t n_held = 0;
	uint64_t walk_time = 0;
	unsigned prev_frames = 0;

	bool frag_open = false;
	int cur_frag = 0, nfrags = 0;
	unsigned fragframes[A2D_MAXBATCH];
	uint8_t fragbase[A2D_MAXBATCH];
	bool uploaded = false;

	std::vector<A2DVoice> mvoices;
	std::vector<A2DVoiceExt> mvext;
	bool long_chains = false;
	std::vector<uint32_t> mudesc;
	std::vector<A2DWave> mwaves;
	bool voices_dirty = true, udesc_dirty = true, waves_dirty = true, lists_dirty = true, ptab_dirty = true;
	std::vector<int> list_all;
	ListRange leaf[LEAF_N];
	int fm_kind_count[8] = { 0 };
	std::vector<DepthRange> depth_ranges;
	ListRange dyn[DYN_N];
	A2Switches sw;
	a2amd_batch_info last_batch = {};
	a2amd_noise_batch_info last_noise = {};
	uint32_t n_noise_standin = 0, n_noise_quiet = 0;
	uint32_t n_noise_filt_quiet = 0;
	a2amd_noise_filter_batch_info last_noise_filter = {};
	uint32_t n_bare_quiet = 0, n_bare_gliding = 0, n_bare_records = 0, n_mono_drivers = 0;
	a2amd_bare_batch_info last_bare = {};
	uint32_t n_o3f_quiet = 0, n_o3f_gliding = 0, n_o3f_records = 0;
	a2amd_osc3filt_batch_info last_osc3filt = {};
	a2amd_osc2_batch_info last_osc2 = {};
	a2amd_fbdpan_batch_info last_fbdpan = {};
	a2amd_bus_windows_info last_buswin = {};
	a2amd_bus_info last_bus = {};
	uint32_t n_bus_windows_dropped = 0;

	size_t bus_stride_frames;
	size_t bus_used = 0;
	std::map<int, std::vector<int>> bus_free;
	std::vector<std::pair<int,int>> deferred_bus_free;

	int fbd_count = 0;
	std::vector<int> fbd_free, fbd_deferred_free, fbd_to_zero;
	int fm_count = 0;
	std::vector<int> fm_free, fm_deferred_free;

	std::vector<XioSlot> xio;
	std::vector<int> xio_free, xio_deferred_free;

	size_t wavepool_used = 0;
	std::vector<std::pair<size_t, size_t>> wavepool_free;
	std::vector<std::pair<size_t, size_t>> deferred_wavepool_free;
	std::vector<int> free_wave_slots, deferred_wave_slots;

	DevBuf<A2DVoice> d_voices;
	DevBuf<A2DVoiceExt> d_vext;
	DevBuf<uint32_t> d_udesc;
	DevBuf<int32_t> d_ustate;
	DevBuf<int32_t> d_ustage;
	DevBuf<int32_t> d_vactive;
	DevBuf<A2DRun> d_runs;
	DevBuf<A2DRec> d_recs;
	DevBuf<A2DWave> d_waves;
	DevBuf<int16_t> d_wavepool;
	DevBuf<int32_t> d_wavecoef;
	DevBuf<int32_t> d_busmem;
	DevBuf<int32_t> d_fbdmem;
	DevBuf<int32_t> d_fmstate;
	DevBuf<int32_t> d_xio;
	uint32_t *d_fmsine = nullptr;
	DevBuf<int> d_list;
	DevBuf<unsigned char> d_staged;
	DevBuf<int> d_scatter;
	uint32_t *d_ptab = nullptr;
	A2DParams *d_params = nullptr;
	DevBuf<char> d_blob;
	char *h_blob[2] = { nullptr, nullptr };
	size_t h_blob_cap[2] = { 0, 0 };
	hipEvent_t blob_ev[2] = { nullptr, nullptr };
	bool blob_busy[2] = { false, false };
	int blob_i = 0;
	const int *d_dyn = nullptr;
	A2DParams hparams;
	hipGraph_t graph[12] = {};
	hipGraphExec_t gexec[12] = {};
	const int32_t *gdst[12] = {};
	bool gdirect[12] = {};
	uint32_t gconsume[12] = {};
	struct Capture { int32_t *d = nullptr; size_t cap = 0, n = 0; bool on = false; uint32_t *d_fragpos = nullptr; } capture;
	DevBuf<uint32_t> d_wavepost;
	uint64_t wave_h2d_bytes = 0;
	uint32_t waves_uploaded = 0, waves_resident = 0;
	int32_t *master_dst = nullptr;
	bool master_direct = false;
	int32_t *h_master = nullptr;
	size_t h_master_cap = 0;
	bool blob_quiet = false;
	int blob_nfrags = 0;
	unsigned blob_frames[A2D_MAXBATCH];
	int quiet_streak = 0;
	struct Readback {
		int32_t *h = nullptr;
		size_t cap = 0;
		hipEvent_t ev = nullptr;
		int nfrags = 0;
		unsigned total = 0;
		uint8_t frames[A2D_MAXBATCH];
	} rb[2];
	int rb_head = 0, rb_count = 0;

	ncclComm_t comm = nullptr;
	int dist_rank = 0, dist_ranks = 1;
	bool dist_local = false;
	hipEvent_t grp_ev = nullptr;

	std::vector<int> moving;
	size_t n_moving_listed = 0;
	DevBuf<int> d_win, d_wext, d_wrc, d_wscr;
	DevBuf<unsigned> d_widx;
	unsigned *d_wtop = nullptr;
	unsigned *h_wtop = nullptr;
	hipEvent_t wtop_ev = nullptr;
	bool wtop_pending = false;
	hipStream_t win_fork[7] = { nullptr, nullptr, nullptr, nullptr, nullptr, nullptr, nullptr };
	hipEvent_t win_fev[8] = { nullptr, nullptr, nullptr, nullptr, nullptr, nullptr, nullptr, nullptr };
	hipStream_t win_stream = nullptr;
	hipEvent_t win_ev[5] = { nullptr, nullptr, nullptr, nullptr, nullptr };

	a2amd_stats stats;
	VmHost vm;

	int fail(int code, const char *fmt, ...)
	{
		va_list ap;
		va_start(ap, fmt);
		vsnprintf(err, sizeof(err), fmt, ap);
		va_end(ap);
		snprintf(g_err, sizeof(g_err), "%s", err);
		return code;
	}
};

static inline void use_device(const a2amd_ctx *c) { (void)hipSetDevice(c->cfg.device); }

namespace a2h {
template<class T>
int grow(a2amd_ctx *c, DevBuf<T> &b, size_t need, size_t elem_mult, bool keep)
{
	if(need <= b.cap)
		return 0;
	size_t ncap = std::max(need, b.cap ? b.cap * 2 : (elem_mult >= 65536 ? (size_t)2 : (size_t)1024));
	T *nd = nullptr;
	HIPCHK(c, hipMalloc((void **)&nd, ncap * elem_mult * sizeof(T)));
	if(keep && b.d && b.cap) {
		HIPCHK(c, hipStreamSynchronize(c->stream));
		HIPCHK(c, hipMemcpyAsync(nd, b.d, b.cap * elem_mult * sizeof(T), hipMemcpyDeviceToDevice, c->stream));
	}
	if(keep)
		HIPCHK(c, hipMemsetAsync((char *)nd + b.cap * elem_mult * sizeof(T), 0,
				(ncap - b.cap) * elem_mult * sizeof(T), c->stream));
	if(keep)
		HIPCHK(c, hipStreamSynchronize(c->stream));
	if(b.d) {
		HIPCHK(c, hipStreamSynchronize(c->stream));
		if(c->vm.pred_stream)
			HIPCHK(c, hipStreamSynchronize(c->vm.pred_stream));
		HIPCHK(c, hipFree(b.d));
	}
	b.d = nd;
	b.cap = ncap;
	return 0;
}

inline int rec_tag(const a2amd_ctx *c) { return c->frag_open ? c->cur_frag : c->nfrags; }
static inline bool is_held(const a2amd_ctx *c, int vi)
{
	return (size_t)vi < c->held.size() && c->held[vi];
}

static inline void unhold(a2amd_ctx *c, int vi)
{
	if(is_held(c, vi)) {
		c->held[vi] = 0;
		--c->n_held;
	}
}

inline bool cutoff_moving(const HUnit &u) { return u.cutoff.timer || u.cutoff.delta || u.cutoff.value != u.cutoff.target; }
inline void sweep_track(a2amd_ctx *c, int ui)
{
	HUnit &u = c->units[ui];
	const bool on = u.live && u.kind == A2AMD_FILTER12 && cutoff_moving(u);
	if(on == (u.sweep_idx >= 0))
		return;
	if(on) {
		u.sweep_idx = (int)c->sweeping.size();
		c->sweeping.push_back(ui);
	} else {
		const int last = c->sweeping.back();
		c->sweeping[u.sweep_idx] = last;
		c->units[last].sweep_idx = u.sweep_idx;
		c->sweeping.pop_back();
		u.sweep_idx = -1;
	}
}
inline bool leaf_mode(int mode) { return mode == A2D_OSC_MIPWAVE || mode == A2D_OSC_OFF || mode == A2D_OSC_NOISE; }
inline bool fbd_tap_ok(int frames) { return frames >= A2D_FRAG && frames <= A2D_FBD_BUFSIZE - A2D_FRAG; }
void drop_graphs(a2amd_ctx *c);
void touch(a2amd_ctx *c, int vi);
void spell_out_pending(a2amd_ctx *c, int vi);
void push_rec(a2amd_ctx *c, int vi, int op, int unit, int reg, int value, unsigned dur, unsigned start);
int bus_alloc(a2amd_ctx *c, int nch);
int close_fragment(a2amd_ctx *c);
void resolve_out(a2amd_ctx *c, HVoice &v);
void sync_voice_mirror(a2amd_ctx *c, int vi);
int upload(a2amd_ctx *c);
void wavepool_release(a2amd_ctx *c, size_t off, size_t len);
void end_batch(a2amd_ctx *c);
int issue_kernels(a2amd_ctx *c, unsigned phases, hipEvent_t e0, hipEvent_t e1, hipEvent_t e2);
int ensure_clean(a2amd_ctx *c);
int build_graph(a2amd_ctx *c, int slot, int steps, unsigned phases = A2AMD_RENDER_SUBTREES | A2AMD_RENDER_ROOT);
long long now_serial(const a2amd_ctx *c);
void wave_tap_policy(a2amd_ctx *c);
int capture_append(a2amd_ctx *c);
double *dbg_counters();
double *dbg_why();
int fetch_taps(a2amd_ctx *c, bool final);
int dist_reduce_root(a2amd_ctx *c);
int vm_prepare_batch(a2amd_ctx *c);
int vm_build_lists(a2amd_ctx *c);
int vm_issue(a2amd_ctx *c, bool fused);
void vm_class_params(a2amd_ctx *c, int k, A2DVmParams *vp);
int vm_fused_done(a2amd_ctx *c);
int vm_predict(a2amd_ctx *c);
bool vm_spec_wanted(a2amd_ctx *c);
void vm_note_batch(a2amd_ctx *c, bool asked);
bool vm_spec_plan(a2amd_ctx *c, int *nfrags, uint8_t *ff, uint8_t *fb);
int vm_speculate(a2amd_ctx *c);
int vm_take_back(a2amd_ctx *c, int vi, bool inclusive, a2amd_vm_state *out, a2amd_vm_env *envs_out = nullptr);
void vm_end_batch(a2amd_ctx *c);
void vm_close(a2amd_ctx *c);
void vm_build_f1tab(a2amd_ctx *c);
void vm_start_f1tab(a2amd_ctx *c);
int vm_blob_room(a2amd_ctx *c);

}

#endif
```

audiality2_amd/csrc/a2amd_render.cpp:

```cpp
#include "a2amd_host.h"
#include "a2amd_wavepads.h"

extern "C" {
static double now_us()
{
	timespec ts;
	clock_gettime(CLOCK_MONOTONIC, &ts);
	return ts.tv_sec * 1e6 + ts.tv_nsec * 1e-3;
}
static double g_t[4], g_n;
static double g_why[13];
static double g_cnt[6];
struct TimingDump { ~TimingDump() {
	A2Switches sw; a2amd_read_switches(&sw); if(sw.hosttiming && g_n) fprintf(stderr,
	"a2amd host timing per render: upload %.1f us, issue %.1f us, readback %.1f us (%g renders; %g quiet uploads, "
	"%g graph launches, %g records, %g voices with records, %g walk scans, %g R_NOPs)\n",
	g_t[0] / g_n, g_t[1] / g_n, g_t[2] / g_n, g_n, g_cnt[0], g_cnt[5], g_cnt[1], g_cnt[4], g_cnt[2], g_cnt[3]);
	if(sw.hosttiming && g_n) { fprintf(stderr, "a2amd uploads by first reason against the quiet path "
	"(blob, recs, prev recs, voices, udesc, waves, lists, ptab, dirty voices, fbd, nfrags, bus, none):");
	for(int k = 0; k < 13; ++k) fprintf(stderr, " %g", g_why[k]); fprintf(stderr, "\n"); } } } g_timing_dump;

}
namespace a2h { double *dbg_counters() { return g_cnt; } double *dbg_why() { return g_why; } }
extern "C" {

}
int a2h::fetch_taps(a2amd_ctx *c, bool final)
{
	bool any = false;
	for(size_t k = 0; k < c->xio.size(); ++k) {
		XioSlot &x = c->xio[k];
		if(x.unit >= 0 && x.tapped) {
			if(final)
				x.tapped = (c->units[x.unit].xio_mode & A2AMD_XIO_TAP) != 0;
			HIPCHK(c, hipMemcpyAsync(x.tap.data(), c->d_xio.d + k * A2D_XIO_SLOT,
					(size_t)c->nfrags * A2AMD_MAXCHANNELS * A2D_FRAG * sizeof(int32_t),
					hipMemcpyDeviceToHost, c->stream));
			any = true;
		}
	}
	if(any)
		HIPCHK(c, hipStreamSynchronize(c->stream));
	return 0;
}

extern "C" {
int a2amd_render(a2amd_ctx *c, unsigned phases, int32_t *const *out, unsigned cap)
{
	use_device(c);
	const bool timing = c->sw.hosttiming;
	double t0 = timing ? now_us() : 0;
	if(!c->stack.empty())
		return c->fail(A2AMD_ESTATE, "render inside an inline window");
	if((phases & A2AMD_RENDER_KEEP) && !c->noise_st.empty())
		return c->fail(A2AMD_EUNSUPPORTED, "A2AMD_RENDER_KEEP on a batch with device-seeded noise windows "
				"(a2amd_fragment_repeat_noise): a re-run would need a new generator word");
	if((phases & A2AMD_RENDER_KEEP) && !c->cut_st.empty())
		return c->fail(A2AMD_EUNSUPPORTED, "A2AMD_RENDER_KEEP on a batch with a cutoff sweep table "
				"(a2amd_fragment_repeat with a sweeping filter): a re-run would need the ramp to go on");
	close_fragment(c);
	unsigned total = 0;
	for(int f = 0; f < c->nfrags; ++f)
		total += c->fragframes[f];
	if(!c->nfrags) {
		if(!(phases & A2AMD_RENDER_KEEP))
			;
		return 0;
	}
	c->snap_valid = false;
	if(c->vm.unwalked >= 0)
		return c->fail(A2AMD_ESTATE, "voice %d is run by the device VM, but the host's walk left it out of a fragment "
				"(no default window reported, no call)", c->vm.unwalked);
	if(phases & A2AMD_RENDER_UPLOAD)
		if(int r = upload(c))
			return r;
	double t1 = timing ? now_us() : 0;
	if(timing)
		g_t[0] += t1 - t0;
	if((phases & (A2AMD_RENDER_SUBTREES | A2AMD_RENDER_ROOT)) && !c->uploaded)
		return c->fail(A2AMD_ESTATE, "render phases out of order: upload first");

	if((phases & A2AMD_RENDER_SUBTREES) && c->profiling) {
		if(c->ev_used + 3 > c->ev_pool.size())
			for(int i = 0; i < 3; ++i) {
// ... 349 lines not shown
{
	if(!c || !out)
		return A2AMD_EINVAL;
	*out = c->last_noise_filter;
	out->min_voices = (uint32_t)c->sw.nzf_min;
	return A2AMD_OK;
}

int a2amd_last_batch_sweeps(const a2amd_ctx *c, a2amd_sweep_batch_info *out)
{
	if(!c || !out)
		return A2AMD_EINVAL;
	*out = c->last_sweeps;
	return A2AMD_OK;
}

int a2amd_last_batch_buses(const a2amd_ctx *c, a2amd_bus_info *out)
{
	if(!c || !out)
		return A2AMD_EINVAL;
	*out = c->last_bus;
	out->master_direct = c->master_direct;
	return A2AMD_OK;
}

int a2amd_last_batch_bare(const a2amd_ctx *c, a2amd_bare_batch_info *out)
{
	if(!c || !out)
		return A2AMD_EINVAL;
	*out = c->last_bare;
	return A2AMD_OK;
}

int a2amd_last_batch_osc3filt(const a2amd_ctx *c, a2amd_osc3filt_batch_info *out)
{
	if(!c || !out)
		return A2AMD_EINVAL;
	*out = c->last_osc3filt;
	return A2AMD_OK;
}

int a2amd_last_batch_osc2(const a2amd_ctx *c, a2amd_osc2_batch_info *out)
{
	if(!c || !out)
		return A2AMD_EINVAL;
	*out = c->last_osc2;
	if(!out->launched || c->blob_nfrags < 1 || c->blob_nfrags > A2D_MAXBATCH)
		return A2AMD_OK;
	unsigned start[A2D_MAXBATCH];
	for(int f = 0, acc = 0; f < c->blob_nfrags; ++f) {
		start[f] = (unsigned)acc;
		acc += (int)c->blob_frames[f];
	}
	unsigned n = 0;
	for(int slice = 0; slice < (int)out->ysplit; ++slice) {
		int c_lo, c_hi, nslices;
		if(!a2d_osc2_slice(c->blob_nfrags, (int)out->ysplit, slice, &c_lo, &c_hi, &nslices))
			break;
		for(int s_lo = c_lo; s_lo < c_hi; s_lo += A2D_OSC2_SCH / A2D_OSC2_FCH, ++n) {
			const int s_hi = std::min(c_hi, s_lo + A2D_OSC2_SCH / A2D_OSC2_FCH);
			const int fa = s_lo * A2D_OSC2_FCH, fb = std::min(c->blob_nfrags, s_hi * A2D_OSC2_FCH);
			if(out->voice_major && a2d_osc2_whole(start[fa], start[fb - 1], c->blob_frames[fb - 1], fb - fa))
				++out->superchunks_voice_major;
			else {
				++out->superchunks_chunk_major;
				if(n < 64)
					out->chunk_major_mask |= 1ull << n;
			}
		}
	}
	return A2AMD_OK;
}

unsigned a2amd_osc2_stage_rule(unsigned size0, int periodic0, unsigned size1, int periodic1)
{
	return a2d_osc2_stage(size0, periodic0 != 0, size1, periodic1 != 0);
}

int a2amd_wave_level_periodic(const int16_t *level, unsigned size)
{
	return a2w_pads_periodic(level, size, A2AMD_WAVEPRE, A2AMD_WAVEPOST);
}

int a2amd_last_batch_fbdpan(const a2amd_ctx *c, a2amd_fbdpan_batch_info *out)
{
	if(!c || !out)
		return A2AMD_EINVAL;
	*out = c->last_fbdpan;
	return A2AMD_OK;
}

int a2amd_last_batch_bus_windows(const a2amd_ctx *c, a2amd_bus_windows_info *out)
{
	if(!c || !out)
		return A2AMD_EINVAL;
	*out = c->last_buswin;
	out->window_cap = FBW_MAXWIN;
	return A2AMD_OK;
}

int a2amd_set_profiling(a2amd_ctx *c, int on)
{
	if(int r = drain_events(c))
		return r;
	if(on) {
		c->stats.timed_leaf_ms = c->stats.timed_all_ms = 0;
		c->stats.timed_batches = 0;
	}
	c->profiling = on != 0;
	return A2AMD_OK;
}

}
```

audiality2_amd/csrc/a2amd_sched.cpp:

```cpp
#include "a2amd_host.h"
#include "a2amd_cutsweep.h"
#include <functional>

namespace a2h {




void touch(a2amd_ctx *c, int vi)
{
	HVoice &v = c->voices[vi];
	const long long serial = c->serial_base + rec_tag(c);
	if(v.touched != serial) {
		v.touched = serial;
		v.frag_mark = v.recs.size();
	}
}



void spell_out_pending(a2amd_ctx *c, int vi)
{
	HVoice &dv = c->voices[vi];
	const bool marked = c->frag_open && c->defmap_used && (size_t)vi < c->defmap.size() && c->defmap[vi];
// ... 822 lines not shown
				std::stable_sort(dyn[k].begin(), dyn[k].end(), by_bus_dyn);
			c->dyn[k] = append_range(dyn_all, dyn[k]);
		}
		c->consume_ok = c->owners_all_driver;
		for(size_t d = 0; d < dyn_bus.size(); ++d) {
			c->depth_ranges[d].dyn = append_range(dyn_all, dyn_bus[d]);
			if(!dyn_bus[d].empty())
				c->consume_ok = false;
			c->depth_ranges[d].fbdpan_win = append_range(dyn_all, fbdpan_win[d]);
		}
		a2amd_bus_info &bi = c->last_bus;
		bi = a2amd_bus_info{};
		bi.driver_windows_dropped = c->n_bus_windows_dropped;
		std::vector<int> ramp;
		c->n_mono_drivers = 0;
		for(size_t d = 0; d < c->depth_ranges.size(); ++d) {
			DepthRange &r = c->depth_ranges[d];
			ramp.clear();
			for(int k = 0; k < r.driver.count; ++k) {
				const int vi = c->list_all[r.driver.first + k];
				const HVoice &v = c->voices[vi];
				c->n_mono_drivers += v.own_nch == 1;
				if(!v.recs.empty())
					continue;
				++bi.driver_voices;
				if(v.moving_until > c->vm.batch_time)
					ramp.push_back(vi);
			}
			bi.driver_ramping += (uint32_t)ramp.size();
			r.ramp = append_range(dyn_all, ramp);
			for(int k = 0; k < r.fbd.count; ++k)
				bi.fbd_voices += c->voices[c->list_all[r.fbd.first + k]].recs.empty();
			bi.generic_voices += (uint32_t)(r.generic.count + r.dyn.count);
		}
		a2amd_fbdpan_batch_info &fp = c->last_fbdpan;
		fp = a2amd_fbdpan_batch_info{};
		for(const DepthRange &r : c->depth_ranges)
			for(int k = 0; k < r.fbdpan.count; ++k) {
				const HVoice &v = c->voices[c->list_all[r.fbdpan.first + k]];
				++fp.class_voices;
				fp.max_delays = std::max(fp.max_delays, (uint32_t)(v.nunits - 2));
				if(!v.recs.empty()) {
					++fp.record_voices;
					continue;
				}
				++fp.quiet_voices;
				fp.gliding_voices += v.moving_until > c->vm.batch_time;
			}
		c->n_bare_quiet = c->n_bare_gliding = c->n_bare_records = 0;
		const ListRange bare = c->leaf[LEAF_OSCBARE];
		for(int k = 0; k < bare.count; ++k) {
			const HVoice &v = c->voices[c->list_all[bare.first + k]];
			if(!v.recs.empty() || v.moving_run == c->serial_base) {
				++c->n_bare_records;
				continue;
			}
			++c->n_bare_quiet;
			c->n_bare_gliding += v.moving_until > c->vm.batch_time;
		}
		c->n_o3f_quiet = c->n_o3f_gliding = c->n_o3f_records = 0;
		const ListRange o3f = c->leaf[LEAF_OSC3FILTPAN];
		for(int k = 0; k < o3f.count; ++k) {
			const HVoice &v = c->voices[c->list_all[o3f.first + k]];
			if(!v.recs.empty() || v.moving_run == c->serial_base) {
				++c->n_o3f_records;
				continue;
			}
			++c->n_o3f_quiet;
			c->n_o3f_gliding += v.moving_until > c->vm.batch_time;
		}
	}

	A2DParams p;
	memset(&p, 0, sizeof(p));
	p.voices = c->d_voices.d;
	p.vext = c->long_chains ? c->d_vext.d : nullptr;
	p.udesc = c->d_udesc.d;
	p.ustate = c->d_ustate.d;
	p.vactive = c->d_vactive.d;
	p.runs = c->d_runs.d;
	p.waves = c->d_waves.d;
	p.wavepool = c->d_wavepool.d;
	p.wavecoef = c->d_wavecoef.d;
	p.busmem = c->d_busmem.d;
	p.fbdmem = c->d_fbdmem.d;
	p.ptab = c->d_ptab;
	p.fmstate = c->d_fmstate.d;
	p.xio = c->d_xio.d;
	p.fmsine = c->d_fmsine;
	if(!c->noise_st.empty()) {
		p.nseed = c->d_nseed.d;
		p.nslot = c->d_nslot.d;
		p.nnoise = c->noise_slots;
	}
	if(!c->cut_st.empty()) {
		p.cutf = c->d_cutf.d;
		p.cslot = c->d_cslot.d;
		p.ncut = c->cut_slots;
	}
	p.nfrags = c->nfrags;
	p.samplerate = c->cfg.samplerate;
	p.debug = c->sw.debug;
	for(int f = 0, acc = 0; f < c->nfrags; ++f) {
		p.fragframes[f] = (uint8_t)c->fragframes[f];
		p.fragstart[f] = (uint16_t)acc;
		acc += (int)c->fragframes[f];
	}

	auto up256 = [](size_t x) { return (x + 255) & ~(size_t)255; };
	const size_t nsc = sc_idx.size();
	const size_t o_recs = up256(sizeof(A2DParams));
	const size_t o_idx = o_recs + up256((recs.size() + 1) * sizeof(A2DRec));
	const size_t o_val = o_idx + up256(nsc * sizeof(int));
	const size_t o_dyn = o_val + up256(nsc * sizeof(A2DRun));
	const size_t o_noise = o_dyn + up256(dyn_all.size() * sizeof(int));
	const size_t o_cut = o_noise + up256(c->noise_osc.size() * sizeof(A2DNoiseOsc));
	const size_t host_total = o_cut + up256(c->cut_list.size() * sizeof(A2DCutSweep));
	const size_t vm_room = (size_t)vm_blob_room(c);
	const size_t total = host_total;
	if(int r = grow(c, c->d_blob, host_total + vm_room * sizeof(A2DRec), 1, false)) return r;
	c->vm.rec_off = host_total;
	c->vm.rec_cap = (uint32_t)((c->d_blob.cap - host_total) / sizeof(A2DRec));
	const int bi = c->blob_i;
	c->blob_i ^= 1;
	if(c->blob_busy[bi]) {
		HIPCHK(c, hipEventSynchronize(c->blob_ev[bi]));
		c->blob_busy[bi] = false;
	}
	if(total > c->h_blob_cap[bi]) {
		if(c->h_blob[bi])
			HIPCHK(c, hipHostFree(c->h_blob[bi]));
		c->h_blob_cap[bi] = std::max(total * 2, (size_t)65536);
		HIPCHK(c, hipHostMalloc((void **)&c->h_blob[bi], c->h_blob_cap[bi], hipHostMallocDefault));
	}
	if(!c->blob_ev[bi])
		HIPCHK(c, hipEventCreateWithFlags(&c->blob_ev[bi], hipEventDisableTiming));
	char *hb = c->h_blob[bi];
	p.recs = (const A2DRec *)(c->d_blob.d + o_recs);
	c->hparams = p;
	memcpy(hb, &p, sizeof(p));
	if(!recs.empty())
		memcpy(hb + o_recs, recs.data(), recs.size() * sizeof(A2DRec));
	if(nsc) {
		memcpy(hb + o_idx, sc_idx.data(), nsc * sizeof(int));
		memcpy(hb + o_val, sc_val.data(), nsc * sizeof(A2DRun));
	}
	if(!dyn_all.empty())
		memcpy(hb + o_dyn, dyn_all.data(), dyn_all.size() * sizeof(int));
	if(!c->noise_osc.empty())
		memcpy(hb + o_noise, c->noise_osc.data(), c->noise_osc.size() * sizeof(A2DNoiseOsc));
	if(!c->cut_list.empty())
		memcpy(hb + o_cut, c->cut_list.data(), c->cut_list.size() * sizeof(A2DCutSweep));
	HIPCHK(c, hipMemcpyAsync(c->d_blob.d, hb, total, hipMemcpyHostToDevice, c->stream));
	HIPCHK(c, hipEventRecord(c->blob_ev[bi], c->stream));
	c->blob_busy[bi] = true;
	c->d_params = (A2DParams *)c->d_blob.d;
	c->d_dyn = (const int *)(c->d_blob.d + o_dyn);
	if(nsc)
		if(a2d_launch_scatter_runs((const int *)(c->d_blob.d + o_idx), (const A2DRun *)(c->d_blob.d + o_val),
				(int)nsc, c->d_runs.d, c->stream))
			return c->fail(A2AMD_EHIP, "scatter launch failed");
	if(!c->noise_st.empty())
		HIPCHK(c, hipMemsetAsync(c->d_nslot.d, 0, c->d_nslot.cap * sizeof(int32_t), c->stream));
	for(const a2amd_ctx::NoiseStretch &st : c->noise_st)
		if(const int e = a2d_launch_noise_seeds((const A2DNoiseOsc *)(c->d_blob.d + o_noise) + st.first, (int)st.n, st.start, st.f0,
				st.count, st.frames, c->d_nseed.d, c->noise_slots, c->d_nseed.cap, c->d_nslot.d, (int)c->d_nslot.cap, c->stream))
// ... 493 lines not shown
		if((c->leaf[k].count != 0) != (k == LEAF_OSCPAN))
			return false;
	return c->dyn[DYN_REST].first + c->dyn[DYN_REST].count == 0;
}

struct LeafPass {
	A2DCommitSet *pend;
	hipEvent_t e1;
	bool use_win;
	bool solo;
	bool done;
};

static int launch_leaves(a2amd_ctx *c, LeafPass &lp)
{
	if(lp.done)
		return 0;
	lp.done = true;
	A2DCommitSet &pend = *lp.pend;
	const int *const list = c->d_list.d;
	auto none_quiet = [&](int k, int nleaf) {
		return (c->sw.vmskip & (k == 2 ? 2 : 1)) && c->vm.spec_use && !c->vm.list.empty() && c->vm.n_cls[k] == nleaf && c->vm.spec_idle[k] == 0;
	};
	const ListRange oscpan = c->leaf[LEAF_OSCPAN];
	if(oscpan.count && none_quiet(0, oscpan.count)) {
		if(lp.solo && lp.e1)
			HIPCHK(c, hipEventRecord(lp.e1, c->stream));
		++c->vm.quiet_skipped;
	} else if(oscpan.count) {
		int vpw, ysplit;
		pick_fast_shape(c->sw, oscpan.count, c->nfrags, &vpw, &ysplit);
		if(a2d_launch_leaf_oscpan(c->d_params, c->hparams, list + oscpan.first, oscpan.count,
				vpw, ysplit, c->d_ustage.d, c->d_staged.d + oscpan.first, c->stream, lp.solo ? (void *)lp.e1 : nullptr,
				&pend.c[pend.n]))
			return c->fail(A2AMD_EHIP, "fast leaf launch failed: %s", hipGetErrorString(hipGetLastError()));
		if(pend.c[pend.n].nlist)
			++pend.n;
		++c->stats.launches;
		c->vm.last.quiet_launched[0] = 1;
	}
	const ListRange noisepan = c->leaf[LEAF_NOISEPAN];
	if(noisepan.count && !c->noise_st.empty() && c->n_noise_quiet) {
		const int vpw = c->sw.nzvpw_set ? c->sw.nzvpw : (noisepan.count + 1023) / 1024;
		if(a2d_launch_leaf_noisepan(c->d_params, c->hparams, list + noisepan.first, noisepan.count, vpw, c->stream))
			return c->fail(A2AMD_EHIP, "noise leaf launch failed: %s", hipGetErrorString(hipGetLastError()));
		++c->stats.launches;
		c->last_noise.quiet_launched = 1;
	}
	const ListRange noisefilt = c->leaf[LEAF_NOISEFILTPAN];
	if(noisefilt.count && !c->noise_st.empty() && c->n_noise_filt_quiet) {
		const int vpg = c->sw.nzfvpg_set ? c->sw.nzfvpg : (noisefilt.count + 255) / 256;
		if(a2d_launch_leaf_noisefiltpan(c->d_params, c->hparams, list + noisefilt.first, noisefilt.count, vpg, c->stream))
			return c->fail(A2AMD_EHIP, "noise filter leaf launch failed: %s", hipGetErrorString(hipGetLastError()));
		++c->stats.launches;
		c->last_noise_filter.quiet_launched = 1;
	}
	const ListRange bare = c->leaf[LEAF_OSCBARE];
	if(bare.count && c->n_bare_quiet) {
		const int vpw = std::min(std::max(c->sw.vpw_set ? c->sw.vpw : (bare.count + 1023) / 1024, 1), 64);
		if(a2d_launch_leaf_oscbare(c->d_params, c->hparams, list + bare.first, bare.count, vpw, c->stream))
			return c->fail(A2AMD_EHIP, "bare oscillator leaf launch failed: %s", hipGetErrorString(hipGetLastError()));
		++c->stats.launches;
		c->last_bare.launched = 1;
		c->last_bare.vpw = (uint32_t)vpw;
	}
	const ListRange o3f = c->leaf[LEAF_OSC3FILTPAN];
	if(o3f.count && c->n_o3f_quiet) {
		const int vpg = std::min(std::max(c->sw.f2vpw ? c->sw.f2vpw : (o3f.count + 255) / 256, 1), 64);
		if(a2d_launch_leaf_osc3filtpan(c->d_params, c->hparams, list + o3f.first, o3f.count, vpg, c->stream))
			return c->fail(A2AMD_EHIP, "3-osc filter leaf launch failed: %s", hipGetErrorString(hipGetLastError()));
		++c->stats.launches;
		c->last_osc3filt.launched = 1;
		c->last_osc3filt.vpg = (uint32_t)vpg;
		c->last_osc3filt.workgroups = (uint32_t)((o3f.count + vpg - 1) / vpg);
	}
	const ListRange osc2pan = c->leaf[LEAF_OSC2PAN];
	if(osc2pan.count && none_quiet(1, osc2pan.count))
		++c->vm.quiet_skipped;
	else if(osc2pan.count) {
		int vpw, ysplit;
		pick_fast_shape(c->sw, osc2pan.count, c->nfrags * A2D_FAST_FCH / A2D_OSC2_FCH, &vpw, &ysplit, 16);
		const int voice_major = !(c->sw.debug & 16);
		const int lds_taps = !(c->sw.debug & (1 << 17));
		if(a2d_launch_leaf_osc2pan(c->d_params, c->hparams, list + osc2pan.first, osc2pan.count,
				vpw, ysplit, c->d_ustage.d, c->d_staged.d + osc2pan.first, c->stream, &pend.c[pend.n], voice_major, lds_taps, &ysplit))
			return c->fail(A2AMD_EHIP, "2-osc leaf launch failed: %s", hipGetErrorString(hipGetLastError()));
		c->last_osc2.launched = 1;
		c->last_osc2.voices = (uint32_t)osc2pan.count;
		c->last_osc2.vpw = (uint32_t)std::min(std::max(vpw, 1), 64);
		c->last_osc2.ysplit = (uint32_t)ysplit;
		c->last_osc2.voice_major = (uint32_t)voice_major;
		if(pend.c[pend.n].nlist)
			++pend.n;
		++c->stats.launches;
		c->vm.last.quiet_launched[1] = 1;
	}
	const ListRange oscfilt = c->leaf[LEAF_OSCFILTPAN];
	if(oscfilt.count && none_quiet(2, oscfilt.count))
		++c->vm.quiet_skipped;
	else if(oscfilt.count) {
		const int nf = oscfilt.count;
		int vpw = c->sw.fvpw_set ? c->sw.fvpw : std::min(std::max((nf + 255) / 256, 1), 64);
		if(a2d_launch_leaf_oscfiltpan(c->d_params, c->hparams, list + oscfilt.first, nf, vpw, c->stream))
			return c->fail(A2AMD_EHIP, "filter leaf launch failed: %s", hipGetErrorString(hipGetLastError()));
		++c->stats.launches;
		c->vm.last.quiet_launched[2] = 1;
	}
	const ListRange o2f = c->leaf[LEAF_OSC2FILTPAN];
	if(o2f.count && c->o2f_quiet) {
		const int nf = o2f.count;
		const int maxv = a2d_osc2filtpan_max_vpg();
		const int rounds = std::max(1, (nf + 256 * maxv - 1) / (256 * maxv));
		const int vpg = c->sw.f2vpw ? c->sw.f2vpw : std::min(std::max((nf + 256 * rounds - 1) / (256 * rounds), 1), maxv);
		if(a2d_launch_leaf_osc2filtpan(c->d_params, c->hparams, list + o2f.first, nf, vpg, c->stream))
			return c->fail(A2AMD_EHIP, "2-osc filter leaf launch failed: %s", hipGetErrorString(hipGetLastError()));
		++c->stats.launches;
		c->last_batch.o2f_launched = 1;
		c->last_batch.o2f_voices = (uint32_t)nf;
		c->last_batch.o2f_max_vpg = (uint32_t)maxv;
		c->last_batch.o2f_vpg = (uint32_t)std::min(std::max(vpg, 1), 64);
	}
	const ListRange fm = c->leaf[LEAF_FMPAN];
	int fm_kinds = 0;
	for(int k = 0; k < 8; ++k)
		fm_kinds += c->fm_kind_count[k] != 0;
	if(fm_kinds > 1 && fm.count <= 16384 && !c->sw.fmvpw_set) {
		if(a2d_launch_leaf_fmpan_all(c->d_params, c->hparams, list + fm.first, c->fm_kind_count, (fm.count + 1023) / 1024, c->stream))
			return c->fail(A2AMD_EHIP, "fm leaf launch failed: %s", hipGetErrorString(hipGetLastError()));
		++c->stats.launches;
	} else {
		for(int k = 0, at = fm.first; k < 8; at += c->fm_kind_count[k++]) {
			const int n = c->fm_kind_count[k];
			if(!n)
				continue;
			int vpw = c->sw.fmvpw_set ? c->sw.fmvpw : (n + 1023) / 1024;
			vpw = std::min(std::max(vpw, 1), 64);
			if(a2d_launch_leaf_fmpan(c->d_params, c->hparams, A2AMD_FM1 + k, list + at, n, vpw, c->stream))
				return c->fail(A2AMD_EHIP, "fm leaf launch failed: %s", hipGetErrorString(hipGetLastError()));
			++c->stats.launches;
		}
	}
	const ListRange gen = c->leaf[LEAF_GENERIC];
	if(gen.count) {
		if(a2d_launch_voices(c->d_params, list + gen.first, gen.count, pick_vpw(gen.count), c->stream))
			return c->fail(A2AMD_EHIP, "leaf launch failed: %s", hipGetErrorString(hipGetLastError()));
		++c->stats.launches;
	}
	if(!lp.use_win) {
		static const int nosc[4] = { 1, 2, 1, 2 }, filt[4] = { 0, 0, 1, 1 };
		const int *lists[4];
		int counts[4], total = 0, kinds = 0;
		for(int k = 0; k < 4; ++k) {
			lists[k] = c->d_dyn + c->dyn[k].first;
			counts[k] = c->dyn[k].count;
			total += counts[k];
			kinds += counts[k] != 0;
		}
		c->last_batch.recs_voices = (uint32_t)total;
		if(!c->vm.list.empty())
			c->last_batch.recs_voices += (uint32_t)(c->vm.n_cls[0] + c->vm.n_cls[1] + c->vm.n_cls[2]);
		if(kinds > 1 && total <= 4096 && !c->sw.rvpw_set) {
			if(a2d_launch_leaf_recs_all(c->sw, c->d_params, c->hparams, lists, counts, 1, c->stream, c->o2f_quiet ? 8 : 0))
				return c->fail(A2AMD_EHIP, "leaf records launch failed: %s", hipGetErrorString(hipGetLastError()));
			++c->stats.launches;
		} else {
			for(int k = 0; k < 4; ++k)
				if(int r = launch_recs(c, nosc[k], filt[k], lists[k], counts[k], k == DYN_FILT2 && c->o2f_quiet))
					return r;
// ... 199 lines not shown
```

audiality2_amd/csrc/a2amd_taps.h:

```cpp
#pragma once
#include <hip/hip_runtime.h>
#include <stdint.h>
#include "a2amd_device.h"
#include "a2amd_dsp.h"
#include "a2amd_fm.h"

#define FAST_WPB   4
#define FAST_FCH   A2D_FAST_FCH

#define WRL(reg, val) reg = me ? (val) : reg

DEV int hermite_step(int v, unsigned ph)
{
	int p;
	asm("v_mul_i32_i24_sdwa %0, %1, %2 dst_sel:DWORD dst_unused:UNUSED_PAD src0_sel:DWORD src1_sel:BYTE_0"
			: "=v"(p) : "v"(v), "v"(ph));
	return __builtin_amdgcn_sbfe(p, 8, 17);
}

DEV int hermite4(int dm, int d0, int d1, int d2, unsigned ph)
{
	int c = (d1 - dm) >> 1;
	int a = (3 * (d0 - d1) + d2 - dm) >> 1;
	int b = dm - d0 + c - a;
// ... 21 lines not shown

typedef int Coef4 __attribute__((ext_vector_type(3)));
#define A2D_COEF_LOAD "llvm.amdgcn.struct.buffer.load.v3i32"
typedef int CoefRsrc __attribute__((ext_vector_type(4)));
extern "C" __device__ Coef4 a2d_coef_load(CoefRsrc rsrc, int vindex, int voffset, int soffset, int aux)
		__asm(A2D_COEF_LOAD);

DEV CoefRsrc coef_rsrc(const int *wavecoef)
{
	const uint64_t b = (uint64_t)wavecoef;
	CoefRsrc r;
	r.x = rfl((int)(unsigned)b);
	r.y = rfl((int)(((unsigned)(b >> 32) & 0xffffu) | ((4u * A2D_COEF_WORDS) << 16)));
	r.z = -1;
	r.w = 0x00020000;
	return r;
}

DEV int coef_base(unsigned doff) { return (int)(doff * (4u * A2D_COEF_WORDS)); }

DEV int hermite_ct(const Coef4 k, unsigned ph)
{
	int t = hermite_step(k.x, ph);
	t = hermite_step(wadd(t, k.y), ph);
	return hermite_step(wadd(t, k.z >> 16), ph);
}

DEV int inter_coefs(const Coef4 ka, unsigned pa, const Coef4 kb, unsigned pb)
{
	int d;
	asm("v_add_u32_sdwa %0, sext(%1), sext(%2) dst_sel:DWORD dst_unused:UNUSED_PAD src0_sel:WORD_0 src1_sel:WORD_0"
			: "=v"(d) : "v"(ka.z), "v"(kb.z));
	return wadd(wadd(d, hermite_ct(ka, pa)), hermite_ct(kb, pb));
}

DEV int frac_x(unsigned ph)
{
	int x;
	const int seven = 7;
	asm("v_lshlrev_b32_sdwa %0, %1, %2 dst_sel:DWORD dst_unused:UNUSED_PAD src0_sel:DWORD src1_sel:BYTE_0"
			: "=v"(x) : "v"(seven), "v"(ph));
	return x;
}

DEV int hermite_cx(const Coef4 k, unsigned ph)
{
	const int x = frac_x(ph);
	int t = wmul(k.x, x) >> 15;
	t = wmul(wadd(t, k.y), x) >> 15;
	t = wmul(wadd(t, k.z >> 16), x) >> 15;
	return wadd((int)(int16_t)(k.z & 0xffff), t);
}

DEV int inter_coefs_x(const Coef4 ka, unsigned pa, const Coef4 kb, unsigned pb)
{
	return hermite_cx(ka, pa) + hermite_cx(kb, pb);
}

DEV Coef4 coef_at(const CoefRsrc rs, int cb, unsigned ph)
{
	return a2d_coef_load(rs, (int)(ph >> 8), 0, cb, 0);
}

typedef __attribute__((address_space(3))) int LdsInt;
DEV Coef4 coef_lds(const LdsInt *level, unsigned ph, unsigned lg)
{
	const LdsInt *e = level + A2D_COEF_WORDS * __builtin_amdgcn_ubfe(ph, 8, lg);
	Coef4 k;
	k.x = e[0];
	k.y = e[1];
	k.z = e[2];
	return k;
}

DEV void stage_level(LdsInt *level, const int *wavecoef, int cb, unsigned size, int lane)
{
	const int *src = wavecoef + ((unsigned)cb >> 2);
	const unsigned n = size * A2D_COEF_WORDS;
#pragma unroll
	for(int r = 0; r < A2D_OSC2_LDS_ENT * A2D_COEF_WORDS / 64; ++r) {
		const unsigned i = (unsigned)(r * 64 + lane);
		if(i < n)
			level[i] = src[i];
	}
}

DEV void lds_wave_fence()
{
	__builtin_amdgcn_fence(__ATOMIC_ACQ_REL, "wavefront");
	__builtin_amdgcn_wave_barrier();
}

DEV unsigned tap_phase(uint64_t ph, unsigned ldph)
{
	const unsigned lo = (unsigned)ph & 0xffffu, hi = (unsigned)(ph >> 16);
	return hi + ((lo + ldph) >> 16);
}

DEV unsigned lane_dph(int lane, unsigned dph)
{
	unsigned t = (unsigned)lane * dph;
	asm("" : "+v"(t));
	return t;
}

DEV int64_t div_trunc_exact(int64_t n, int d)
{
	int64_t q = (int64_t)((double)n / (double)d);
	const int64_t r = n - q * d;
	if(n >= 0) {
		if(r < 0) --q; else if(r >= d) ++q;
	} else {
		if(r > 0) ++q; else if(r <= -(int64_t)d) --q;
	}
	return q;
}


template<int N>
DEV void flush_acc(int *busmem, int off, int nch, int f0, int nf, int lane, int dbg,
		int (&acc0)[N], int (&acc1)[N])
{
#pragma unroll
	for(int j = 0; j < N; ++j) {
		if(j < nf && off >= 0 && !(dbg & 1)) {
			int *dst = busmem + off + (size_t)(f0 + j) * nch * A2D_FRAG;
			if(acc0[j])
				atomicAdd(&dst[lane], acc0[j]);
			if(acc1[j])
				atomicAdd(&dst[A2D_FRAG + lane], acc1[j]);
		}
		acc0[j] = 0;
		acc1[j] = 0;
	}
}

DEV void tile_add(int *w, int x)
{
	(void)__hip_atomic_fetch_add(w, x, __ATOMIC_RELAXED, __HIP_MEMORY_SCOPE_WAVEFRONT);
}

DEV void flush_tile(int *busmem, int off, int nch, int f0, int nf, int nrows, int lane, int dbg, int (*tile)[2][A2D_FRAG])
{
	for(int r = 0; r < nrows; ++r) {
		const int a0 = tile[r][0][lane], a1 = tile[r][1][lane];
		tile[r][0][lane] = 0;
		tile[r][1][lane] = 0;
		if(r < nf && off >= 0 && !(dbg & 1)) {
			int *dst = busmem + off + (size_t)(f0 + r) * nch * A2D_FRAG;
			if(a0)
				atomicAdd(&dst[lane], a0);
			if(a1)
				atomicAdd(&dst[A2D_FRAG + lane], a1);
		}
	}
}
```

audiality2_amd/replay.py:

```python
import ctypes as C
import gzip
import lzma

import numpy as np

T_FRAGMENT, T_INIT, T_DEINIT, T_WRITE, T_PROCESS, T_INLINE_END, T_WAVE, T_CONFIG, T_WAVEDROP = range(1, 10)
MIPLEVELS = 10
WAVEPRE = 1
WAVEPOST = 131


class Trace:

    def __init__(self, path):
        opener = gzip.open if str(path).endswith(".gz") else lzma.open if str(path).endswith(".xz") else open
        with opener(path, "rb") as f:
            raw = f.read()
        words = np.frombuffer(raw[: len(raw) // 4 * 4], dtype="<i4")
        self.records = []
        self.waves = {}
        self.config = None
        i = 0
        n = len(words)
        while i + 8 <= n:
# ... 115 lines not shown

class a2amd_vm_batch_info(C.Structure):
    _fields_ = [("listed", C.c_uint32), ("class_voices", C.c_uint32 * 3), ("other_voices", C.c_uint32),
                ("pending", C.c_uint32), ("fused", C.c_uint32), ("not_fused", C.c_uint32),
                ("spec_valid", C.c_uint32), ("spec_taken", C.c_uint32), ("spec_miss", C.c_uint32),
                ("spec_next", C.c_uint32), ("spec_why_not", C.c_uint32), ("records", C.c_uint32),
                ("idle_known", C.c_uint32), ("idle", C.c_uint32 * 3), ("quiet_launched", C.c_uint32 * 3)]

    def __repr__(self):
        return ("vm_batch_info(" + ", ".join(f"{n}={list(getattr(self, n)) if n in ('class_voices', 'idle', 'quiet_launched') else getattr(self, n)}"
                                             for n, _ in self._fields_) + ")")


class a2amd_vm_state(C.Structure):
    _fields_ = [("waketime", C.c_uint32), ("state", C.c_uint8), ("func", C.c_uint8), ("pc", C.c_uint16),
                ("r", C.c_int32 * 64)]


class Backend:

    def __init__(self, lib, prefix, samplerate, basepitch, channels=2, device=0,
                 max_batch=64, stream=None):
        self.lib, self.prefix, self.channels = lib, prefix, channels

        def fn(name, restype, *argtypes):
            f = getattr(lib, prefix + name)
            f.restype, f.argtypes = restype, list(argtypes)
            return f

        vp, i32, u32, u64 = C.c_void_p, C.c_int, C.c_uint, C.c_uint64
        self._open = fn("open", i32, C.POINTER(a2amd_config), C.POINTER(vp))
        self._close = fn("close", None, vp)
        self._err = fn("last_error", C.c_char_p, vp)
        self._wave_upload = fn("wave_upload", i32, vp, u64, C.POINTER(a2amd_wavedesc))
        self._wave_drop = fn("wave_drop", i32, vp, u64)
        self._fragment = fn("fragment", i32, vp, u32)
        self._unit_init = fn("unit_init", i32, vp, u64, i32, u32, i32, i32, i32, i32, u32)
        self._unit_deinit = fn("unit_deinit", i32, vp, i32)
        self._unit_write = fn("unit_write", i32, vp, i32, i32, i32, u32, u32, i32)
        self._unit_process = fn("unit_process", i32, vp, i32, u32, u32, C.POINTER(C.c_uint32))
        self._inline_end = fn("inline_end", i32, vp, i32)
        self._unit_clients = fn("unit_clients", i32, vp, i32, u32)
        self._unit_inject = fn("unit_inject", i32, vp, i32, u32, u32, C.POINTER(C.POINTER(C.c_int32)))
        self._unit_tapped = fn("unit_tapped", i32, vp, i32, u32, C.POINTER(C.POINTER(C.c_int32)))
        self._render = fn("render", i32, vp, u32, C.POINTER(C.POINTER(C.c_int32)), u32)
        self._set_pt = fn("set_pitch_table", i32, vp, C.POINTER(C.c_uint32))
        self._get_pt = fn("get_pitch_table", i32, vp, C.POINTER(C.c_uint32))
        self.has_walk = hasattr(lib, prefix + "voice_process")
        if self.has_walk:
            self._voice_process = fn("voice_process", i32, vp, i32, u32, u32, C.POINTER(C.c_uint32))
            self._voice_slot = fn("voice_slot", i32, vp, i32)
            self._default_map = fn("default_map", C.POINTER(C.c_uint8), vp, C.POINTER(u32))
        self._fragment_repeat_noise = None
        if hasattr(lib, prefix + "fragment_repeat_noise"):
            self._fragment_repeat_noise = fn("fragment_repeat_noise", i32, vp, u32, u32, C.POINTER(C.c_uint32))
        self._last_batch_noise = None
        if hasattr(lib, prefix + "last_batch_noise"):
            self._last_batch_noise = fn("last_batch_noise", i32, vp, C.POINTER(a2amd_noise_batch_info))
        self._last_batch_noise_filter = None
        if hasattr(lib, prefix + "last_batch_noise_filter"):
            self._last_batch_noise_filter = fn("last_batch_noise_filter", i32, vp, C.POINTER(a2amd_noise_filter_batch_info))
        self._fragment_repeat = None
        if hasattr(lib, prefix + "fragment_repeat"):
            self._fragment_repeat = fn("fragment_repeat", i32, vp, u32, u32)
        self._last_batch_sweeps = None
        if hasattr(lib, prefix + "last_batch_sweeps"):
            self._last_batch_sweeps = fn("last_batch_sweeps", i32, vp, C.POINTER(a2amd_sweep_batch_info))
        self._last_batch_buses = None
        if hasattr(lib, prefix + "last_batch_buses"):
            self._last_batch_buses = fn("last_batch_buses", i32, vp, C.POINTER(a2amd_bus_info))
        self._last_batch_bare = None
        if hasattr(lib, prefix + "last_batch_bare"):
            self._last_batch_bare = fn("last_batch_bare", i32, vp, C.POINTER(a2amd_bare_batch_info))
        self._last_batch_osc3filt = None
        if hasattr(lib, prefix + "last_batch_osc3filt"):
            self._last_batch_osc3filt = fn("last_batch_osc3filt", i32, vp, C.POINTER(a2amd_osc3filt_batch_info))
        self._last_batch_osc2 = None
        if hasattr(lib, prefix + "last_batch_osc2"):
            self._last_batch_osc2 = fn("last_batch_osc2", i32, vp, C.POINTER(a2amd_osc2_batch_info))
        self._osc2_stage_rule = self._wave_level_periodic = None
        if hasattr(lib, prefix + "osc2_stage_rule"):
            self._osc2_stage_rule = fn("osc2_stage_rule", u32, u32, i32, u32, i32)
            self._wave_level_periodic = fn("wave_level_periodic", i32, C.POINTER(C.c_int16), u32)
        self._last_batch_fbdpan = None
        if hasattr(lib, prefix + "last_batch_fbdpan"):
            self._last_batch_fbdpan = fn("last_batch_fbdpan", i32, vp, C.POINTER(a2amd_fbdpan_batch_info))
        self._last_batch_bus_windows = None
        if hasattr(lib, prefix + "last_batch_bus_windows"):
            self._last_batch_bus_windows = fn("last_batch_bus_windows", i32, vp, C.POINTER(a2amd_bus_windows_info))
        self.has_vm = hasattr(lib, prefix + "vm_adopt")
        if self.has_vm:
            self._fragment_offset = fn("fragment_offset", i32, vp, u32)
            self._vm_program = fn("vm_program", i32, vp, u64, C.POINTER(C.c_uint32), u32)
            self._vm_adopt = fn("vm_adopt", i32, vp, i32, i32, C.POINTER(a2amd_vm_state), C.POINTER(C.c_int32),
                                C.POINTER(C.c_uint8), C.c_uint32, C.c_uint32, vp, i32)
            self._vm_expect_cuts = fn("vm_expect_cuts", i32, vp, C.POINTER(C.c_uint32), i32)
            self._vm_recall = fn("vm_recall", i32, vp, C.POINTER(C.c_int32), u32, C.POINTER(a2amd_vm_state), vp)
        self._last_batch_vm = None
        if hasattr(lib, prefix + "last_batch_vm"):
            self._last_batch_vm = fn("last_batch_vm", i32, vp, C.POINTER(a2amd_vm_batch_info))
        self.has_capture = hasattr(lib, prefix + "wave_upload_captured_post")
        if self.has_capture:
            self._capture_begin = fn("capture_begin", i32, vp)
            self._capture_end = fn("capture_end", i32, vp, C.POINTER(vp))
            self._capture_frames = fn("capture_frames", u32, vp)
            self._capture_free = fn("capture_free", None, vp)
            self._wave_upload_captured = fn("wave_upload_captured", i32, vp, u64, C.POINTER(a2amd_wavedesc), vp)
            self._wave_upload_captured_post = fn("wave_upload_captured_post", i32, vp, u64, C.POINTER(a2amd_wavedesc), vp, u32)
            self._wave_stats = fn("wave_stats", i32, vp, C.POINTER(u64), C.POINTER(u32), C.POINTER(u32))
        cfg = a2amd_config(C.sizeof(a2amd_config), samplerate, basepitch, channels,
                           device, max_batch, stream)
        self.ctx = vp()
        rc = self._open(C.byref(cfg), C.byref(self.ctx))
        if rc != 0:
            raise RuntimeError(f"{prefix}open failed: {rc} "
                               f"{self._err(None).decode(errors='replace')}")
        self.noise = C.c_uint32(0)
        self._keep = []

    def close(self):
        if self.ctx:
            self._close(self.ctx)
            self.ctx = None

    def _chk(self, rc, what):
        if rc < 0:
            msg = self._err(self.ctx)
            raise RuntimeError(f"{self.prefix}{what}: {rc} {msg.decode(errors='replace') if msg else ''}")
        return rc

    def wave_upload(self, key, wtype, flags, period, sizes, data):
        d = a2amd_wavedesc()
        d.type, d.flags, d.period = wtype, flags, period
        for lv, arr in enumerate(data):
            arr = np.ascontiguousarray(arr, dtype=np.int16)
            self._keep.append(arr)
            d.size[lv] = sizes[lv]
            d.data[lv] = arr.ctypes.data_as(C.POINTER(C.c_int16))
        return self._chk(self._wave_upload(self.ctx, key, C.byref(d)), "wave_upload")

    def capture_begin(self):
        return self._chk(self._capture_begin(self.ctx), "capture_begin")

    def capture_end(self):
        cap = C.c_void_p()
        self._chk(self._capture_end(self.ctx, C.byref(cap)), "capture_end")
        return cap if cap.value else None

    def capture_frames(self, cap):
        return self._capture_frames(cap)

    def capture_free(self, cap):
        self._capture_free(cap)

    def wave_upload_captured(self, key, wtype, flags, period, sizes, cap, chunk=None, check=True):
        d = a2amd_wavedesc()
        d.type, d.flags, d.period = wtype, flags, period
        for lv, n in enumerate(sizes):
            d.size[lv] = n
        if chunk is None:
            rc = self._wave_upload_captured(self.ctx, key, C.byref(d), cap)
        else:
            rc = self._wave_upload_captured_post(self.ctx, key, C.byref(d), cap, chunk)
        return self._chk(rc, "wave_upload_captured") if check else rc

    def wave_stats(self):
        h2d, up, res = C.c_uint64(), C.c_uint32(), C.c_uint32()
        self._chk(self._wave_stats(self.ctx, C.byref(h2d), C.byref(up), C.byref(res)), "wave_stats")
        return h2d.value, up.value, res.value

    def wave_drop(self, key):
        return self._chk(self._wave_drop(self.ctx, key), "wave_drop")

    def fragment(self, frames):
        return self._chk(self._fragment(self.ctx, frames), "fragment")

    def fragment_repeat(self, frames, count):
        if self._fragment_repeat is None:
            raise RuntimeError(f"this library has no {self.prefix}fragment_repeat")
        return self._chk(self._fragment_repeat(self.ctx, frames, count), "fragment_repeat")

    def last_batch_sweeps(self):
        if self._last_batch_sweeps is None:
            raise RuntimeError(f"this library has no {self.prefix}last_batch_sweeps")
        bi = a2amd_sweep_batch_info()
        self._chk(self._last_batch_sweeps(self.ctx, C.byref(bi)), "last_batch_sweeps")
        return bi

    def fragment_repeat_noise(self, frames, count):
        if self._fragment_repeat_noise is None:
            raise RuntimeError(f"this library has no {self.prefix}fragment_repeat_noise")
        return self._chk(self._fragment_repeat_noise(self.ctx, frames, count, C.byref(self.noise)),
                         "fragment_repeat_noise")

    def last_batch_noise(self):
        if self._last_batch_noise is None:
            raise RuntimeError(f"this library has no {self.prefix}last_batch_noise")
        bi = a2amd_noise_batch_info()
        self._chk(self._last_batch_noise(self.ctx, C.byref(bi)), "last_batch_noise")
        return bi

    def last_batch_noise_filter(self):
        if self._last_batch_noise_filter is None:
            raise RuntimeError(f"this library has no {self.prefix}last_batch_noise_filter")
        bi = a2amd_noise_filter_batch_info()
        self._chk(self._last_batch_noise_filter(self.ctx, C.byref(bi)), "last_batch_noise_filter")
        return bi

    def last_batch_buses(self):
        if self._last_batch_buses is None:
            raise RuntimeError(f"this library has no {self.prefix}last_batch_buses")
        bi = a2amd_bus_info()
        self._chk(self._last_batch_buses(self.ctx, C.byref(bi)), "last_batch_buses")
        return bi

    def last_batch_bare(self):
        if self._last_batch_bare is None:
            raise RuntimeError(f"this library has no {self.prefix}last_batch_bare")
        bi = a2amd_bare_batch_info()
        self._chk(self._last_batch_bare(self.ctx, C.byref(bi)), "last_batch_bare")
        return bi

    def last_batch_osc3filt(self):
        if self._last_batch_osc3filt is None:
            raise RuntimeError(f"this library has no {self.prefix}last_batch_osc3filt")
        bi = a2amd_osc3filt_batch_info()
        self._chk(self._last_batch_osc3filt(self.ctx, C.byref(bi)), "last_batch_osc3filt")
        return bi

    def last_batch_osc2(self):
        if self._last_batch_osc2 is None:
            raise RuntimeError(f"this library has no {self.prefix}last_batch_osc2")
        bi = a2amd_osc2_batch_info()
        self._chk(self._last_batch_osc2(self.ctx, C.byref(bi)), "last_batch_osc2")
        return bi

    def osc2_stage_rule(self, size0, periodic0, size1, periodic1):
        if self._osc2_stage_rule is None:
            raise RuntimeError(f"this library has no {self.prefix}osc2_stage_rule")
        return int(self._osc2_stage_rule(size0, int(bool(periodic0)), size1, int(bool(periodic1))))

    def wave_level_periodic(self, level):
        if self._wave_level_periodic is None:
            raise RuntimeError(f"this library has no {self.prefix}wave_level_periodic")
        arr = np.ascontiguousarray(level, dtype=np.int16)
        return bool(self._wave_level_periodic(arr.ctypes.data_as(C.POINTER(C.c_int16)), len(arr) - WAVEPRE - WAVEPOST))

    def last_batch_fbdpan(self):
        if self._last_batch_fbdpan is None:
            raise RuntimeError(f"this library has no {self.prefix}last_batch_fbdpan")
        bi = a2amd_fbdpan_batch_info()
        self._chk(self._last_batch_fbdpan(self.ctx, C.byref(bi)), "last_batch_fbdpan")
        return bi

    def last_batch_bus_windows(self):
        if self._last_batch_bus_windows is None:
            raise RuntimeError(f"this library has no {self.prefix}last_batch_bus_windows")
        bi = a2amd_bus_windows_info()
        self._chk(self._last_batch_bus_windows(self.ctx, C.byref(bi)), "last_batch_bus_windows")
        return bi

    def last_batch_vm(self):
        if self._last_batch_vm is None:
            raise RuntimeError(f"this library has no {self.prefix}last_batch_vm")
        bi = a2amd_vm_batch_info()
        self._chk(self._last_batch_vm(self.ctx, C.byref(bi)), "last_batch_vm")
        return bi

    def fragment_offset(self, offset):
        return self._chk(self._fragment_offset(self.ctx, offset), "fragment_offset")

    def vm_program(self, key, words):
        code = (C.c_uint32 * len(words))(*[w & 0xffffffff for w in words])
        return self._chk(self._vm_program(self.ctx, key, code, len(words)), "vm_program")

    def vm_adopt(self, head_unit, prog, state, wires, now, msdur, check=True):
        wu = (C.c_int32 * 64)(*([-1] * 64))
        wr = (C.c_uint8 * 64)()
        for r, (u, ureg) in wires.items():
            wu[r], wr[r] = u, ureg
        rc = self._vm_adopt(self.ctx, head_unit, prog, C.byref(state), wu, wr, now & 0xffffffff, msdur, None, 0)
        return self._chk(rc, "vm_adopt") if check else rc

    def vm_expect_cuts(self, when):
        arr = (C.c_uint32 * max(len(when), 1))(*[w & 0xffffffff for w in when])
        return self._chk(self._vm_expect_cuts(self.ctx, arr, len(when)), "vm_expect_cuts")

    def vm_recall(self, head_units):
        n = len(head_units)
        out = (a2amd_vm_state * n)()
        self._chk(self._vm_recall(self.ctx, (C.c_int32 * n)(*head_units), n, out, None), "vm_recall")
        return list(out)

    def last_error(self):
        msg = self._err(self.ctx)
        return msg.decode(errors="replace") if msg else ""

    def unit_init(self, voice_key, kind, flags, nin, nout, wired, transpose=0, wakefrac=0):
        return self._chk(self._unit_init(self.ctx, voice_key, kind, flags, nin, nout, wired,
                                         transpose, wakefrac), "unit_init")

    def unit_deinit(self, unit):
        return self._chk(self._unit_deinit(self.ctx, unit), "unit_deinit")

    def unit_write(self, unit, reg, value, start=0, dur=0, transpose=0):
        return self._chk(self._unit_write(self.ctx, unit, reg, value, start, dur, transpose),
                         "unit_write")

    def unit_process(self, unit, offset, frames, use_noise=True):
        return self._chk(self._unit_process(self.ctx, unit, offset, frames,
                                            C.byref(self.noise) if use_noise else None),
                         "unit_process")

    def voice_process(self, units, offset, frames):
        if self.has_walk:
            return self._chk(self._voice_process(self.ctx, units[0], offset, frames, C.byref(self.noise)),
                             "voice_process")
        for u in units:
            self.unit_process(u, offset, frames)
        return 0

    def mark_default(self, units):
        n = C.c_uint(0)
# ... 106 lines not shown
```

include/a2amd.h:

```cpp
#ifndef A2AMD_H
#define A2AMD_H

#include <stdint.h>

#ifdef __cplusplus
extern "C" {
#endif

#define A2AMD_MAXFRAG      64
#define A2AMD_MAXCHANNELS   8
#define A2AMD_MIPLEVELS    10
#define A2AMD_WAVEPRE       1
#define A2AMD_WAVEPOST    131
#define A2AMD_MAXCHAIN     16

typedef struct a2amd_ctx a2amd_ctx;

typedef enum a2amd_errors {
	A2AMD_OK = 0,
	A2AMD_ENODEVICE   = -1,
	A2AMD_EINVAL      = -2,
	A2AMD_ENOMEM      = -3,
	A2AMD_EUNSUPPORTED= -4,
	A2AMD_ESTATE      = -5,
// ... 96 lines not shown
#define A2AMD_XIO_INJECT  2u
#define A2AMD_XIO_MUTE    4u
int  a2amd_unit_clients(a2amd_ctx *ctx, int unit, unsigned mode);
int  a2amd_unit_insertable(a2amd_ctx *ctx, int unit);
int  a2amd_render_paused(a2amd_ctx *ctx);
int  a2amd_unit_insert(a2amd_ctx *ctx, int unit, unsigned fragment, unsigned offset, unsigned frames,
		const int32_t *const *bufs);
int  a2amd_unit_inject(a2amd_ctx *ctx, int unit, unsigned offset, unsigned frames,
		const int32_t *const *bufs);
int  a2amd_unit_tapped(a2amd_ctx *ctx, int unit, unsigned fragment, const int32_t **bufs);

int  a2amd_inline_end(a2amd_ctx *ctx, int unit);

#define A2AMD_RENDER_SUBTREES 1u
#define A2AMD_RENDER_ROOT     2u
#define A2AMD_RENDER_UPLOAD   4u
#define A2AMD_RENDER_READBACK 8u
#define A2AMD_RENDER_TAPS     64u
#define A2AMD_RENDER_KEEP    16u
#define A2AMD_RENDER_ASYNC   32u
#define A2AMD_RENDER_EXCHANGE 128u
#define A2AMD_RENDER_ALL     15u
int  a2amd_render(a2amd_ctx *ctx, unsigned phases, int32_t *const *out,
		unsigned out_capacity_frames);
int  a2amd_collect(a2amd_ctx *ctx, int32_t *const *out, unsigned out_capacity_frames);
int  a2amd_replay(a2amd_ctx *ctx, unsigned steps);
int  a2amd_rootbus(a2amd_ctx *ctx, void **devptr, uint64_t *bytes);
int  a2amd_rootbus_copy(a2amd_ctx *ctx, void *stage, int to_stage);

int  a2amd_dist_unique_id(void *id128);
int  a2amd_dist_init(a2amd_ctx *ctx, const void *id128, int rank, int nranks);
int  a2amd_dist_init_local(a2amd_ctx *const *ctxs, int n);
int  a2amd_render_group(a2amd_ctx *const *ctxs, int n, unsigned phases, int32_t *const *out,
		unsigned out_capacity_frames);

int  a2amd_fragment_repeat(a2amd_ctx *ctx, unsigned frames, unsigned count);


typedef struct a2amd_stats {
	uint64_t fragments;
	uint64_t voice_fragments;
	uint64_t records;
	uint64_t launches;
	double   last_kernel_ms;
	double   last_leaf_ms;
	uint32_t live_units, live_voices, live_waves, reserved;
	double   timed_leaf_ms;
	double   timed_all_ms;
	uint64_t timed_batches;
} a2amd_stats;
int  a2amd_get_stats(a2amd_ctx *ctx, a2amd_stats *st);
int  a2amd_set_profiling(a2amd_ctx *ctx, int on);
typedef struct a2amd_batch_info {
	uint32_t o2f_launched;
	uint32_t o2f_voices;
	uint32_t o2f_vpg;
	uint32_t o2f_max_vpg;
	uint32_t o2f_class;
	uint32_t o2f_listed;
	uint32_t recs_voices;
	uint32_t win_voices;
	uint32_t win_slabs;
	uint32_t n_moving_listed;
	uint32_t general_voices;
} a2amd_batch_info;
int  a2amd_last_batch(const a2amd_ctx *ctx, a2amd_batch_info *bi);

#ifdef __cplusplus
}
#endif

#include "a2amd_noise.h"
#include "a2amd_noisepan.h"
#include "a2amd_noisefilt.h"
#include "a2amd_sweep.h"
#include "a2amd_bus.h"
#include "a2amd_wavepost.h"
#include "a2amd_oscbare.h"
#include "a2amd_fbdpan.h"
#include "a2amd_buswin.h"
#include "a2amd_vmbatch.h"
#include "a2amd_osc2.h"
#include "a2amd_osc2lds.h"
#include "a2amd_osc3filt.h"

#endif
```

Before: 536.5 billion voice-samples/s.

## Add tame-wave fused Hermite path with 4-wide coefficient table for osc2 leaf

```diff
diff --git a/audiality2_amd/build.py b/audiality2_amd/build.py
--- a/audiality2_amd/build.py
+++ b/audiality2_amd/build.py
@@ -58,9 +58,9 @@
     srcs = [os.path.join(csrc, f) for f in ("a2amd_host.cpp", "a2amd_sched.cpp", "a2amd_render.cpp", "a2amd_dist.cpp",
                                             "a2amd_vm.cpp", "a2amd_kernels.hip", "a2amd_fast.hip", "a2amd_vm.hip", "a2amd_wavecap.hip", "a2amd_wavepost.hip", "a2amd_win.hip", "a2amd_vmwin.hip", "a2amd_noise.hip", "a2amd_noisepan.hip", "a2amd_noisefiltpan.hip", "a2amd_cutsweep.hip", "a2amd_oscbare.hip", "a2amd_osc3filtpan.hip")]
     deps = srcs + [os.path.join(csrc, "a2amd_host.h"), os.path.join(csrc, "a2amd_switches.h"), os.path.join(csrc, "a2amd_device.h"), os.path.join(csrc, "a2amd_dsp.h"),
-                   os.path.join(csrc, "a2amd_fm.h"), os.path.join(csrc, "a2amd_vmcore.h"), os.path.join(csrc, "a2amd_taps.h"), os.path.join(csrc, "a2amd_winctl.h"), os.path.join(csrc, "a2amd_vmdev.h"), os.path.join(csrc, "a2amd_noisemap.h"), os.path.join(csrc, "a2amd_noisevoice.h"), os.path.join(csrc, "a2amd_settled.h"), os.path.join(csrc, "a2amd_cutsweep.h"), os.path.join(csrc, "a2amd_filt.h"), os.path.join(csrc, "a2amd_wavepads.h"), os.path.join(ROOT, "include", "a2amd.h"),
+                   os.path.join(csrc, "a2amd_fm.h"), os.path.join(csrc, "a2amd_vmcore.h"), os.path.join(csrc, "a2amd_taps.h"), os.path.join(csrc, "a2amd_winctl.h"), os.path.join(csrc, "a2amd_vmdev.h"), os.path.join(csrc, "a2amd_noisemap.h"), os.path.join(csrc, "a2amd_noisevoice.h"), os.path.join(csrc, "a2amd_settled.h"), os.path.join(csrc, "a2amd_cutsweep.h"), os.path.join(csrc, "a2amd_filt.h"), os.path.join(csrc, "a2amd_wavepads.h"), os.path.join(csrc, "a2amd_wavetame.h"), os.path.join(ROOT, "include", "a2amd.h"),
                    os.path.join(ROOT, "include", "a2amd_noise.h"), os.path.join(ROOT, "include", "a2amd_noisepan.h"), os.path.join(ROOT, "include", "a2amd_noisefilt.h"), os.path.join(ROOT, "include", "a2amd_sweep.h"), os.path.join(ROOT, "include", "a2amd_wavepost.h"),
-                   os.path.join(ROOT, "include", "a2amd_bus.h"), os.path.join(ROOT, "include", "a2amd_oscbare.h"), os.path.join(ROOT, "include", "a2amd_osc3filt.h"), os.path.join(ROOT, "include", "a2amd_fbdpan.h"), os.path.join(ROOT, "include", "a2amd_buswin.h"), os.path.join(ROOT, "include", "a2amd_vmbatch.h"), os.path.join(ROOT, "include", "a2amd_osc2.h"), os.path.join(ROOT, "include", "a2amd_osc2lds.h"), os.path.join(ROOT, "include", "a2amd_vm.h")]
+                   os.path.join(ROOT, "include", "a2amd_bus.h"), os.path.join(ROOT, "include", "a2amd_oscbare.h"), os.path.join(ROOT, "include", "a2amd_osc3filt.h"), os.path.join(ROOT, "include", "a2amd_fbdpan.h"), os.path.join(ROOT, "include", "a2amd_buswin.h"), os.path.join(ROOT, "include", "a2amd_vmbatch.h"), os.path.join(ROOT, "include", "a2amd_osc2.h"), os.path.join(ROOT, "include", "a2amd_osc2lds.h"), os.path.join(ROOT, "include", "a2amd_osc2tame.h"), os.path.join(ROOT, "include", "a2amd_vm.h")]
     out = os.path.join(HERE, "liba2amd.so")
     flags = ["--offload-arch=gfx950", "-O3", "-std=c++17", "-fPIC", "-shared", "-Wno-unused-value"]
     want = source_hash(deps, flags)
@@ -73,7 +73,7 @@
     src = os.path.join(HERE, "csrc", "a2amd_units.c")
     deps = [src, os.path.join(ROOT, "include", "a2amd.h"), os.path.join(ROOT, "include", "a2amd_noise.h"), os.path.join(ROOT, "include", "a2amd_noisepan.h"),
             os.path.join(ROOT, "include", "a2amd_noisefilt.h"), os.path.join(ROOT, "include", "a2amd_sweep.h"), os.path.join(ROOT, "include", "a2amd_bus.h"),
-            os.path.join(ROOT, "include", "a2amd_wavepost.h"), os.path.join(ROOT, "include", "a2amd_oscbare.h"), os.path.join(ROOT, "include", "a2amd_osc3filt.h"), os.path.join(ROOT, "include", "a2amd_fbdpan.h"), os.path.join(ROOT, "include", "a2amd_buswin.h"), os.path.join(ROOT, "include", "a2amd_vmbatch.h"), os.path.join(ROOT, "include", "a2amd_osc2.h"), os.path.join(ROOT, "include", "a2amd_osc2lds.h"), os.path.join(ROOT, "include", "a2amd_plugin.h"),
+            os.path.join(ROOT, "include", "a2amd_wavepost.h"), os.path.join(ROOT, "include", "a2amd_oscbare.h"), os.path.join(ROOT, "include", "a2amd_osc3filt.h"), os.path.join(ROOT, "include", "a2amd_fbdpan.h"), os.path.join(ROOT, "include", "a2amd_buswin.h"), os.path.join(ROOT, "include", "a2amd_vmbatch.h"), os.path.join(ROOT, "include", "a2amd_osc2.h"), os.path.join(ROOT, "include", "a2amd_osc2lds.h"), os.path.join(ROOT, "include", "a2amd_osc2tame.h"), os.path.join(ROOT, "include", "a2amd_plugin.h"),
             os.path.join(ROOT, "include", "a2amd_walk.h"), os.path.join(ROOT, "include", "a2amd_vm.h")]
     out = os.path.join(HERE, "liba2amd_units.so")
     flags = ["-O2", "-Wall", "-fPIC", "-shared"]
diff --git a/audiality2_amd/csrc/a2amd_device.h b/audiality2_amd/csrc/a2amd_device.h
--- a/audiality2_amd/csrc/a2amd_device.h
+++ b/audiality2_amd/csrc/a2amd_device.h
@@ -64,8 +64,11 @@
 	uint32_t period;
 	uint32_t size[A2D_MIPS];
 	uint32_t off[A2D_MIPS];
-	uint32_t periodic;
-};
+	uint16_t periodic;
+	uint16_t tame;
+};
+
+static_assert(A2D_MIPS <= 16 && sizeof(A2DWave) == 96, "A2DWave: a bit per level in a half word, 96 bytes");
 
 struct A2DVoice {
 	int32_t nunits;
@@ -191,6 +194,7 @@
 	int32_t         debug;
 	uint8_t         fragframes[A2D_MAXBATCH];
 	uint16_t        fragstart[A2D_MAXBATCH];
+	const int32_t  *wavecoef4;
 };
 
 #ifdef __HIPCC__
@@ -217,6 +221,11 @@
 	const bool c0 = periodic0 && size0 && !(size0 & (size0 - 1)) && size0 <= A2D_OSC2_LDS_ENT;
 	const bool c1 = periodic1 && size1 && !(size1 & (size1 - 1)) && size1 <= A2D_OSC2_LDS_ENT;
 	return (c0 ? 1u : 0u) | (c1 && (c0 ? size0 : 0u) + size1 <= A2D_OSC2_LDS_ENT ? 2u : 0u);
+}
+
+A2D_HD unsigned a2d_osc2_tame(unsigned tame0, unsigned tame1)
+{
+	return tame0 && tame1 ? 1u : 0u;
 }
 
 #ifdef __HIPCC__
@@ -306,7 +315,7 @@
 int a2d_launch_park(int32_t *stage, int32_t *bus, unsigned words, void *stream);
 int a2d_launch_add_bus(int32_t *dst, int32_t *src, unsigned words, void *stream);
 int a2d_launch_add_inject(const int32_t *inj, int32_t *bus, int nch, int n, int nfrags, void *stream);
-int a2d_launch_build_coef(const int16_t *pool, int *coef, unsigned lo, unsigned hi, void *stream);
+int a2d_launch_build_coef(const int16_t *pool, int *coef, int *coef4, unsigned lo, unsigned hi, void *stream);
 int a2d_launch_capture(const int32_t *bus, int32_t *dst, const uint32_t *fragpos, int nfrags, int nch, void *stream);
 int a2d_launch_wave_from_pcm(const int32_t *pcm, int16_t *pool, const uint32_t *off, const uint32_t *size, int levels, int looped,
 		int pre, int post, void *stream);
@@ -324,7 +333,7 @@
 int a2d_launch_scatter_runs(const int *didx, const A2DRun *dval, int n, A2DRun *druns, void *stream);
 int a2d_launch_leaf_osc2pan(const A2DParams *dparams, const A2DParams &hp, const int *dlist, int nlist,
 		int vpw, int ysplit, int *ustage, unsigned char *staged, void *stream, A2DCommit *defer, int voice_major, int lds_taps,
-		int *ysplit_used);
+		int tame, unsigned long long *tame_count, int *ysplit_used);
 struct A2Switches;
 int a2d_launch_leaf_recs(const A2Switches &sw, const A2DParams *dparams, const A2DParams &hp, int nosc, int filt, const int *dlist,
 		int nlist, int vpw, void *stream, int skip_empty = 0);
diff --git a/audiality2_amd/csrc/a2amd_fast.hip b/audiality2_amd/csrc/a2amd_fast.hip
--- a/audiality2_amd/csrc/a2amd_fast.hip
+++ b/audiality2_amd/csrc/a2amd_fast.hip
@@ -10,7 +10,8 @@
 
 #include "a2amd_taps.h"
 
-__global__ void k_build_coef(const int16_t *__restrict__ pool, int *__restrict__ coef, unsigned lo, unsigned hi)
+__global__ void k_build_coef(const int16_t *__restrict__ pool, int *__restrict__ coef, int *__restrict__ coef4, unsigned lo,
+		unsigned hi)
 {
 	const unsigned j = lo + blockIdx.x * blockDim.x + threadIdx.x;
 	if(j >= hi)
@@ -23,13 +24,15 @@
 	e[0] = a;
 	e[1] = b;
 	e[2] = (int)(((unsigned)c << 16) | ((unsigned)d0 & 0xffffu));
-}
-
-int a2d_launch_build_coef(const int16_t *pool, int *coef, unsigned lo, unsigned hi, void *stream)
+	if(coef4)
+		*(Coef4x *)(coef4 + 4 * (size_t)j) = Coef4x{ a, (int)((unsigned)b << 8), (int)((unsigned)c << 8), (int)((unsigned)d0 << 8) };
+}
+
+int a2d_launch_build_coef(const int16_t *pool, int *coef, int *coef4, unsigned lo, unsigned hi, void *stream)
 {
 	if(hi <= lo)
 		return 0;
-	hipLaunchKernelGGL(k_build_coef, dim3((hi - lo + 255) / 256), dim3(256), 0, (hipStream_t)stream, pool, coef, lo, hi);
+	hipLaunchKernelGGL(k_build_coef, dim3((hi - lo + 255) / 256), dim3(256), 0, (hipStream_t)stream, pool, coef, coef4, lo, hi);
 	return (int)hipGetLastError();
 }
 
@@ -251,7 +254,8 @@
 
 enum { DV_SETTLED = 0, DV_MM, DV_DPH, DV_SIZEM, DV_DOFF, DV_V0, DV_V1, DV_NWORDS };
 
-DEV bool settled_wave(const A2DWave *w, unsigned dphase, int *d, bool settled = true, unsigned *periodic = nullptr)
+DEV bool settled_wave(const A2DWave *w, unsigned dphase, int *d, bool settled = true, unsigned *periodic = nullptr,
+		unsigned *tame = nullptr)
 {
 	unsigned dph;
 	const unsigned mm = a2s_mip(dphase, w->period, &dph);
@@ -261,6 +265,8 @@
 	d[3] = (int)w->off[mm];
 	if(periodic)
 		*periodic = (w->periodic >> mm) & 1u;
+	if(tame)
+		*tame = (w->tame >> mm) & 1u;
 	return settled && a2s_wave_ok(w->size[0], w->flags, dph);
 }
 
@@ -610,6 +616,8 @@
 	WRL(so[OV_A + 2], o.a.delta); WRL(so[OV_A + 3], o.a.timer);
 }
 
+template<bool TAME> struct Osc2Entry { typedef Coef4 T; };
+template<> struct Osc2Entry<true> { typedef Coef4x T; };
 struct Osc2Voice {
 	unsigned dph[2], sizem[2];
 	int cb[2], amp[2];
@@ -620,11 +628,11 @@
 	unsigned lg[2];
 };
 
-template<bool WHOLE, int ST = 0>
+template<bool WHOLE, int ST = 0, bool TAME = false>
 DEV void osc2_chunk(const CoefRsrc &crs, Osc2Voice &s, const unsigned (&ldph)[2], const int (&nfr)[OSC2_FCH],
 		const unsigned (&pre)[OSC2_FCH], int nf, bool park, int (&xs)[OSC2_FCH], const Osc2Lds &lv = Osc2Lds())
 {
-	Coef4 ka[2][OSC2_FCH], kb[2][OSC2_FCH];
+	typename Osc2Entry<TAME>::T ka[2][TAME ? OSC2_FCH / 2 : OSC2_FCH], kb[2][TAME ? OSC2_FCH / 2 : OSC2_FCH];
 	unsigned pa[2][OSC2_FCH], pb[2][OSC2_FCH];
 #pragma unroll
 	for(int o = 0; o < 2; ++o) {
@@ -650,7 +658,8 @@
 			pa[o][j] = tap_phase(phs[j], ldph[o]);
 			asm("" : "+v"(pa[o][j]));
 			pb[o][j] = pa[o][j] + (dph >> 17);
-			if((ST >> o) & 1) {
+			if constexpr(TAME) {
+			} else if((ST >> o) & 1) {
 				ka[o][j] = coef_lds(lv.level[o], pa[o][j], lv.lg[o]);
 				kb[o][j] = coef_lds(lv.level[o], pb[o][j], lv.lg[o]);
 			} else {
@@ -668,24 +677,63 @@
 		}
 		s.ph[o] = ph;
 	}
-#pragma unroll
-	for(int o = 0; o < 2; ++o)
-#pragma unroll
-		for(int j = 0; j < OSC2_FCH; ++j) {
-			const int y = mul64s(inter_coefs(ka[o][j], pa[o][j], kb[o][j], pb[o][j]), s.amp[o], 17);
-			xs[j] = o ? wadd(xs[j], y) : y;
-		}
+	if constexpr(TAME) {
+		constexpr int H = OSC2_FCH / 2;
+		auto fetch = [&](int o, int h, int slot) {
+#pragma unroll
+			for(int j = 0; j < H; ++j) {
+				if((ST >> o) & 1) {
+					ka[slot][j] = coef4_lds(lv.level[o], pa[o][h * H + j], lv.lg[o]);
+					kb[slot][j] = coef4_lds(lv.level[o], pb[o][h * H + j], lv.lg[o]);
+				} else {
+					ka[slot][j] = coef4_at(crs, s.cb[o], pa[o][h * H + j]);
+					kb[slot][j] = coef4_at(crs, s.cb[o], pb[o][h * H + j]);
+				}
+			}
+		};
+		auto use = [&](int o, int h, int slot) {
+#pragma unroll
+			for(int j = 0; j < H; ++j) {
+				const int x = wadd(hermite_fused(ka[slot][j], pa[o][h * H + j]), hermite_fused(kb[slot][j], pb[o][h * H + j]));
+				const int y = mul64s(x, s.amp[o], 17);
+				xs[h * H + j] = o ? wadd(xs[h * H + j], y) : y;
+			}
+		};
+		fetch(0, 0, 0);
+		fetch(0, 1, 1);
+		__builtin_amdgcn_sched_barrier(0);
+		use(0, 0, 0);
+		__builtin_amdgcn_sched_barrier(0);
+		fetch(1, 0, 0);
+		__builtin_amdgcn_sched_barrier(0);
+		use(0, 1, 1);
+		__builtin_amdgcn_sched_barrier(0);
+		fetch(1, 1, 1);
+		__builtin_amdgcn_sched_barrier(0);
+		use(1, 0, 0);
+		use(1, 1, 1);
+		return;
+	} else {
+#pragma unroll
+		for(int o = 0; o < 2; ++o)
+#pragma unroll
+			for(int j = 0; j < OSC2_FCH; ++j) {
+				const int y = mul64s(inter_coefs(ka[o][j], pa[o][j], kb[o][j], pb[o][j]), s.amp[o], 17);
+				xs[j] = o ? wadd(xs[j], y) : y;
+			}
+	}
 }
 
 DEV void osc2_voice_from_lanes(Osc2Voice &s, unsigned (&ldph)[2], unsigned (&mm)[2], const int (&od)[2][OD_NWORDS],
-		const int (&amp_l)[2], const int (&phlo_l)[2], const int (&phhi_l)[2], int v, unsigned before, int lane)
+		const int (&amp_l)[2], const int (&phlo_l)[2], const int (&phhi_l)[2], int v, unsigned before, int lane,
+		bool tame = false)
 {
 #pragma unroll
 	for(int o = 0; o < 2; ++o) {
 		mm[o] = (unsigned)rdl(od[o][OD_MM], v);
 		s.dph[o] = (unsigned)rdl(od[o][OD_DPH], v);
 		s.sizem[o] = (unsigned)rdl(od[o][OD_SIZEM], v);
-		s.cb[o] = coef_base((unsigned)rdl(od[o][OD_DOFF], v));
+		s.cb[o] = tame ? coef4_base((unsigned)rdl(od[o][OD_DOFF], v)) : coef_base((unsigned)rdl(od[o][OD_DOFF], v));
 		s.amp[o] = rdl(amp_l[o], v);
 		const uint64_t phase = (uint64_t)(unsigned)rdl(phlo_l[o], v) | ((uint64_t)(unsigned)rdl(phhi_l[o], v) << 32);
 		s.ph[o] = (phase >> mm[o]) + (uint64_t)before * s.dph[o];
@@ -693,7 +741,7 @@
 	}
 }
 
-template<int ST>
+template<int ST, bool TAME = false>
 DEV void osc2_voice_chunks(const CoefRsrc &crs, Osc2Voice &s, const unsigned (&ldph)[2], const unsigned (&mm)[2],
 		const Osc2Lds &lv, int nsc, int nfs, bool last, int v0, int v1, int v, int lane, int (*tile)[2][A2D_FRAG],
 		int (&phlo_l)[2], int (&phhi_l)[2])
@@ -703,7 +751,7 @@
 	for(int k = 0; k < nsc; ++k) {
 		const bool park = last && k == nsc - 1;
 		int xs[OSC2_FCH];
-		osc2_chunk<true, ST>(crs, s, ldph, nopre_i, nopre_u, nfs - k * OSC2_FCH, park, xs, lv);
+		osc2_chunk<true, ST, TAME>(crs, s, ldph, nopre_i, nopre_u, nfs - k * OSC2_FCH, park, xs, lv);
 #pragma unroll
 		for(int j = 0; j < OSC2_FCH; ++j) {
 			tile_add(&tile[k * OSC2_FCH + j][0][lane], mul64s(xs[j], v0, 24));
@@ -721,12 +769,15 @@
 	}
 }
 
-template<bool STAGE>
+template<bool STAGE, bool TAME = false>
 DEV void osc2_superchunk(const CoefRsrc &crs, const int *wavecoef, int *busmem, const int (&od)[2][OD_NWORDS],
 		const int (&amp_l)[2], int (&phlo_l)[2], int (&phhi_l)[2], int settled_l, int my_off, int my_nch, int v0l, int v1l,
 		int nv, int nsc, int fa, int nfs, bool last, unsigned before, int lane, int dbg, int (*tile)[2][A2D_FRAG],
-		LdsInt *level)
-{
+		LdsInt *level, const int *wavecoef4 = nullptr)
+{
+	CoefRsrc crs4 = crs;
+	if(TAME)
+		crs4 = coef4_rsrc(wavecoef4);
 	int cur_off = rdl(my_off, 0), cur_nch = rdl(my_nch, 0);
 	for(int v = 0; v < nv; ++v) {
 		const int sl = rdl(settled_l, v);
@@ -741,6 +792,32 @@
 		const int v0 = rdl(v0l, v), v1 = rdl(v1l, v);
 		Osc2Voice s;
 		unsigned ldph[2], mm[2];
+		if(TAME && (sl & 8)) {
+			osc2_voice_from_lanes(s, ldph, mm, od, amp_l, phlo_l, phhi_l, v, before, lane, true);
+			Osc2Lds lv = { { level, level }, { 0, 0 } };
+			const int st = (sl >> 1) & 3;
+			if(st) {
+				lds_wave_fence();
+				if(st & 1) {
+					lv.lg[0] = (s.sizem[0] - 1) << 4;
+					stage_level4(level, wavecoef4, s.cb[0], s.sizem[0], lane);
+				}
+				if(st & 2) {
+					LdsInt *const l1 = (st & 1) ? level + s.sizem[0] * 4 : level;
+					lv.level[1] = l1;
+					lv.lg[1] = (s.sizem[1] - 1) << 4;
+					stage_level4(l1, wavecoef4, s.cb[1], s.sizem[1], lane);
+				}
+				lds_wave_fence();
+			}
+			switch(st) {
+			case 0: osc2_voice_chunks<0, true>(crs4, s, ldph, mm, lv, nsc, nfs, last, v0, v1, v, lane, tile, phlo_l, phhi_l); break;
+			case 1: osc2_voice_chunks<1, true>(crs4, s, ldph, mm, lv, nsc, nfs, last, v0, v1, v, lane, tile, phlo_l, phhi_l); break;
+			case 2: osc2_voice_chunks<2, true>(crs4, s, ldph, mm, lv, nsc, nfs, last, v0, v1, v, lane, tile, phlo_l, phhi_l); break;
+			default: osc2_voice_chunks<3, true>(crs4, s, ldph, mm, lv, nsc, nfs, last, v0, v1, v, lane, tile, phlo_l, phhi_l); break;
+			}
+			continue;
+		}
 		osc2_voice_from_lanes(s, ldph, mm, od, amp_l, phlo_l, phhi_l, v, before, lane);
 		Osc2Lds lv = { { level, level }, { 0, 0 } };
 		if(!STAGE) {
@@ -773,12 +850,14 @@
 }
 
 #define OSC2_WPE 4
+template<bool TAME_K>
 __global__ __launch_bounds__(64 * FAST_WPB) __attribute__((amdgpu_waves_per_eu(OSC2_WPE, OSC2_WPE)))
 void k_leaf_osc2pan(const A2DParams *__restrict__ pp, const int *__restrict__ list, int nlist, int vpw,
 		int ysplit, const A2DVoice *__restrict__ voices, const int *ustate, int *ustage,
 		const int16_t *__restrict__ wavepool, const A2DWave *__restrict__ waves,
 		const uint32_t *__restrict__ ptab, int *__restrict__ busmem, const int *__restrict__ wavecoef,
-		unsigned char *__restrict__ staged, int vmajor, int lds_taps)
+		unsigned char *__restrict__ staged, int vmajor, int lds_taps, const int *__restrict__ wavecoef4, int tame,
+		unsigned long long *__restrict__ tame_count)
 {
 	const A2DParams &p = *pp;
 	const int wv = rfl((int)(threadIdx.x >> 6));
@@ -822,7 +901,7 @@
 		my_nch = vc.out_nch;
 		bool settled = true;
 		int wave_l[2], dphase_l[2];
-		unsigned periodic[2] = { 0, 0 };
+		unsigned periodic[2] = { 0, 0 }, tame_lv[2] = { 0, 0 };
 #pragma unroll
 		for(int o = 0; o < 2; ++o) {
 			uu[o] = vc.unit[o];
@@ -844,18 +923,25 @@
 		if(settled) {
 #pragma unroll
 			for(int o = 0; o < 2; ++o)
-				settled = settled_wave(waves + wave_l[o], (unsigned)dphase_l[o], od[o], settled, &periodic[o]);
+				settled = settled_wave(waves + wave_l[o], (unsigned)dphase_l[o], od[o], settled, &periodic[o],
+						TAME_K ? &tame_lv[o] : nullptr);
 			a2s_pan_gains(sp[PW_VOL], sp[PW_PAN], a2s_pan_over(sp[PW_PAN]), &v0l, &v1l);
 		}
 		settled_l = settled ? 1 : 0;
 		if(settled && lds_taps)
 			settled_l |= (int)a2d_osc2_stage((unsigned)od[0][OD_SIZEM], periodic[0], (unsigned)od[1][OD_SIZEM], periodic[1]) << 1;
+		if(TAME_K && settled && tame)
+			settled_l |= (int)a2d_osc2_tame(tame_lv[0], tame_lv[1]) << 3;
 	}
 	const unsigned long long unsettled_mask = __ballot(mine && !settled_l);
-	const bool any_staged = __ballot(settled_l > 1) != 0;
+	const bool any_staged = __ballot((settled_l & 6) != 0) != 0;
+	const unsigned long long tame_mask = TAME_K ? __ballot((settled_l & 8) != 0) : 0ull;
+	const bool any_tame = tame_mask != 0;
+	if(TAME_K && any_tame && slice == 0 && lane == 0)
+		atomicAdd(tame_count, (unsigned long long)__popcll(tame_mask));
 
 	__shared__ int tiles[FAST_WPB][OSC2_SCH][2][A2D_FRAG];
-	__shared__ int levels[FAST_WPB][A2D_OSC2_LDS_ENT * A2D_COEF_WORDS];
+	__shared__ __attribute__((aligned(16))) int levels[FAST_WPB][A2D_OSC2_LDS_ENT * (TAME_K ? 4 : A2D_COEF_WORDS)];
 	int (*const tile)[2][A2D_FRAG] = tiles[wv];
 	LdsInt *const level = (LdsInt *)levels[wv];
 	if(vmajor)
@@ -868,7 +954,10 @@
 		const bool last = last_slice && s_hi == c_hi;
 		const unsigned before = (unsigned)frames_of(fst, fa);
 		if(vmajor && a2d_osc2_whole(before, (unsigned)frames_of(fst, fa + nfs - 1), (unsigned)frames_of(ffr, fa + nfs - 1), nfs)) {
-			if(any_staged)
+			if(TAME_K && any_tame)
+				osc2_superchunk<true, TAME_K>(crs, wavecoef, busmem, od, amp_l, phlo_l, phhi_l, settled_l, my_off, my_nch, v0l, v1l,
+						nv, s_hi - s_lo, fa, nfs, last, before, lane, dbg, tile, level, wavecoef4);
+			else if(any_staged)
 				osc2_superchunk<true>(crs, wavecoef, busmem, od, amp_l, phlo_l, phhi_l, settled_l, my_off, my_nch, v0l, v1l,
 						nv, s_hi - s_lo, fa, nfs, last, before, lane, dbg, tile, level);
 			else
@@ -2873,7 +2962,7 @@
 
 int a2d_launch_leaf_osc2pan(const A2DParams *dparams, const A2DParams &hp, const int *dlist, int nlist,
 		int vpw, int ysplit, int *ustage, unsigned char *staged, void *stream, A2DCommit *defer, int voice_major, int lds_taps,
-		int *ysplit_used)
+		int tame, unsigned long long *tame_count, int *ysplit_used)
 {
 	if(nlist <= 0)
 		return 0;
@@ -2884,9 +2973,16 @@
 		*ysplit_used = ysplit;
 	int nwaves = (nlist + vpw - 1) / vpw;
 	int nblocks = (nwaves + FAST_WPB - 1) / FAST_WPB;
-	hipLaunchKernelGGL(k_leaf_osc2pan, dim3(nblocks, ysplit), dim3(64 * FAST_WPB), 0, (hipStream_t)stream,
-			dparams, dlist, nlist, vpw, ysplit, hp.voices, (const int *)hp.ustate,
-			ysplit > 1 ? ustage : hp.ustate, hp.wavepool, hp.waves, hp.ptab, hp.busmem, hp.wavecoef, staged, voice_major, lds_taps);
+	if(tame && hp.wavecoef4 && tame_count)
+		hipLaunchKernelGGL(k_leaf_osc2pan<true>, dim3(nblocks, ysplit), dim3(64 * FAST_WPB), 0, (hipStream_t)stream,
+				dparams, dlist, nlist, vpw, ysplit, hp.voices, (const int *)hp.ustate,
+				ysplit > 1 ? ustage : hp.ustate, hp.wavepool, hp.waves, hp.ptab, hp.busmem, hp.wavecoef, staged, voice_major, lds_taps,
+				hp.wavecoef4, 1, tame_count);
+	else
+		hipLaunchKernelGGL(k_leaf_osc2pan<false>, dim3(nblocks, ysplit), dim3(64 * FAST_WPB), 0, (hipStream_t)stream,
+				dparams, dlist, nlist, vpw, ysplit, hp.voices, (const int *)hp.ustate,
+				ysplit > 1 ? ustage : hp.ustate, hp.wavepool, hp.waves, hp.ptab, hp.busmem, hp.wavecoef, staged, voice_major, lds_taps,
+				(const int *)nullptr, 0, (unsigned long long *)nullptr);
 	if(ysplit > 1) {
 		A2DCommit cm = { dlist, nlist, 2, ustage, staged };
 		if(defer)
diff --git a/audiality2_amd/csrc/a2amd_host.cpp b/audiality2_amd/csrc/a2amd_host.cpp
--- a/audiality2_amd/csrc/a2amd_host.cpp
+++ b/audiality2_amd/csrc/a2amd_host.cpp
@@ -3,6 +3,7 @@
 #include "a2amd_cutsweep.h"
 #include "a2amd_settled.h"
 #include "a2amd_wavepads.h"
+#include "a2amd_wavetame.h"
 
 namespace a2h { thread_local char g_err[256] = ""; }
 
@@ -69,6 +70,12 @@
 	c->d_wavepool.cap = 8u << 20;
 	OPENCHK(hipMalloc((void **)&c->d_wavecoef.d, (size_t)(8u << 20) * A2D_COEF_WORDS * sizeof(int32_t)));
 	c->d_wavecoef.cap = 8u << 20;
+	if(coef4_wanted(c, 0)) {
+		OPENCHK(hipMalloc((void **)&c->d_wavecoef4.d, (size_t)(8u << 20) * 4 * sizeof(int32_t)));
+		c->d_wavecoef4.cap = 8u << 20;
+	}
+	OPENCHK(hipMalloc((void **)&c->d_tame_count, sizeof(unsigned long long)));
+	OPENCHK(hipMemset(c->d_tame_count, 0, sizeof(unsigned long long)));
 #undef OPENCHK
 	*out = c;
 	return A2AMD_OK;
@@ -107,7 +114,7 @@
 	for(int k = 0; k < 5; ++k)
 		if(c->win_ev[k])
 			hipEventDestroy(c->win_ev[k]);
-	hipFree(c->d_waves.d); hipFree(c->d_wavepool.d); hipFree(c->d_wavecoef.d); hipFree(c->d_busmem.d);
+	hipFree(c->d_waves.d); hipFree(c->d_wavepool.d); hipFree(c->d_wavecoef.d); hipFree(c->d_wavecoef4.d); hipFree(c->d_tame_count); hipFree(c->d_busmem.d);
 	vm_close(c);
 	hipFree(c->capture.d); hipFree(c->capture.d_fragpos); hipFree(c->d_wavepost.d);
 	hipFree(c->d_fbdmem.d); hipFree(c->d_fmstate.d); hipFree(c->d_xio.d); hipFree(c->d_fmsine); hipFree(c->d_list.d); hipFree(c->d_staged.d); hipFree(c->d_scatter.d); hipFree(c->d_ptab); hipFree(c->d_blob.d);
@@ -137,11 +144,33 @@
 
 }
 namespace a2h {
+bool coef4_wanted(const a2amd_ctx *c, size_t pool_samples)
+{
+	return c->sw.raw <= 0 && pool_samples * (4 * A2D_COEF_WORDS) <= ((size_t)c->sw.coef_cache_mb << 20);
+}
+
+void coef4_drop(a2amd_ctx *c)
+{
+	if(!c->d_wavecoef4.d)
+		return;
+	hipStreamSynchronize(c->stream);
+	if(c->vm.pred_stream)
+		hipStreamSynchronize(c->vm.pred_stream);
+	hipFree(c->d_wavecoef4.d);
+	c->d_wavecoef4.d = nullptr;
+	c->d_wavecoef4.cap = 0;
+	c->waves_dirty = true;
+	drop_graphs(c);
+	c->blob_quiet = false;
+}
+
 void wave_tap_policy(a2amd_ctx *c)
 {
 	const int force = c->sw.raw;
 	const size_t budget = (size_t)c->sw.coef_cache_mb << 20;
 	const bool big = c->wavepool_used * (4 * A2D_COEF_WORDS) > budget;
+	if(!coef4_wanted(c, c->wavepool_used))
+		coef4_drop(c);
 	for(size_t i = 0; i < c->waves.size(); ++i) {
 		HWave &w = c->waves[i];
 		if(!w.live || w.dw.type != A2AMD_WMIPWAVE)
@@ -351,11 +380,17 @@
 		}
 	if(pos == (size_t)-1) {
 		if(c->wavepool_used + total > c->d_wavepool.cap) {
-			if((c->wavepool_used + total) * (4 * A2D_COEF_WORDS) > (((size_t)1 << 32) - 4096))
-				return c->fail(A2AMD_ENOMEM, "wave pool beyond %zu samples", (((size_t)1 << 32) - 4096) / (4 * A2D_COEF_WORDS));
+			const bool keep4 = c->d_wavecoef4.d && coef4_wanted(c, c->wavepool_used + total);
+			const size_t entry = keep4 ? 16 : 4 * A2D_COEF_WORDS;
+			if((c->wavepool_used + total) * entry > (((size_t)1 << 32) - 4096))
+				return c->fail(A2AMD_ENOMEM, "wave pool beyond %zu samples", (((size_t)1 << 32) - 4096) / entry);
 			if(int r = grow(c, c->d_wavepool, c->wavepool_used + total, 1, true)) return r;
 			if(int r = grow(c, c->d_wavecoef, c->d_wavepool.cap, A2D_COEF_WORDS, false)) return r;
-			if(c->wavepool_used > 3 && a2d_launch_build_coef(c->d_wavepool.d, c->d_wavecoef.d, 1,
+			if(keep4) {
+				if(int r = grow(c, c->d_wavecoef4, c->d_wavepool.cap, 4, false)) return r;
+			} else
+				coef4_drop(c);
+			if(c->wavepool_used > 3 && a2d_launch_build_coef(c->d_wavepool.d, c->d_wavecoef.d, c->d_wavecoef4.d, 1,
 					(unsigned)c->wavepool_used - 2, c->stream))
 				return c->fail(A2AMD_EHIP, "coefficient build failed");
 			c->waves_dirty = true;
@@ -376,6 +411,8 @@
 			c->wave_h2d_bytes += n * sizeof(int16_t);
 			if((w->flags & 0x100u) && a2w_pads_periodic(w->data[l], w->size[l], A2AMD_WAVEPRE, A2AMD_WAVEPOST))
 				hw.dw.periodic |= 1u << l;
+			if(a2w_level_tame(w->data[l], w->size[l], A2AMD_WAVEPRE, A2AMD_WAVEPOST))
+				hw.dw.tame |= 1u << l;
 		}
 		loff[l] = (uint32_t)(pos - pos0);
 		lsize[l] = w->size[l];
@@ -394,7 +431,7 @@
 		++c->waves_resident;
 	} else
 		++c->waves_uploaded;
-	if(total > 3 && a2d_launch_build_coef(c->d_wavepool.d, c->d_wavecoef.d, (unsigned)hw.pool_off + 1,
+	if(total > 3 && a2d_launch_build_coef(c->d_wavepool.d, c->d_wavecoef.d, c->d_wavecoef4.d, (unsigned)hw.pool_off + 1,
 			(unsigned)(hw.pool_off + total) - 2, c->stream))
 		return c->fail(A2AMD_EHIP, "coefficient build failed");
 	c->mwaves[id] = hw.dw;
diff --git a/audiality2_amd/csrc/a2amd_host.h b/audiality2_amd/csrc/a2amd_host.h
--- a/audiality2_amd/csrc/a2amd_host.h
+++ b/audiality2_amd/csrc/a2amd_host.h
@@ -445,6 +445,8 @@
 	DevBuf<A2DWave> d_waves;
 	DevBuf<int16_t> d_wavepool;
 	DevBuf<int32_t> d_wavecoef;
+	DevBuf<int32_t> d_wavecoef4;
+	unsigned long long *d_tame_count = nullptr;
 	DevBuf<int32_t> d_busmem;
 	DevBuf<int32_t> d_fbdmem;
 	DevBuf<int32_t> d_fmstate;
@@ -603,6 +605,8 @@
 int build_graph(a2amd_ctx *c, int slot, int steps, unsigned phases = A2AMD_RENDER_SUBTREES | A2AMD_RENDER_ROOT);
 long long now_serial(const a2amd_ctx *c);
 void wave_tap_policy(a2amd_ctx *c);
+bool coef4_wanted(const a2amd_ctx *c, size_t pool_samples);
+void coef4_drop(a2amd_ctx *c);
 int capture_append(a2amd_ctx *c);
 double *dbg_counters();
 double *dbg_why();
diff --git a/audiality2_amd/csrc/a2amd_render.cpp b/audiality2_amd/csrc/a2amd_render.cpp
--- a/audiality2_amd/csrc/a2amd_render.cpp
+++ b/audiality2_amd/csrc/a2amd_render.cpp
@@ -1,5 +1,6 @@
 #include "a2amd_host.h"
 #include "a2amd_wavepads.h"
+#include "a2amd_wavetame.h"
 
 extern "C" {
 static double now_us()
@@ -515,6 +516,28 @@
 	return a2w_pads_periodic(level, size, A2AMD_WAVEPRE, A2AMD_WAVEPOST);
 }
 
+int a2amd_wave_level_tame(const int16_t *level, unsigned size)
+{
+	return a2w_level_tame(level, size, A2AMD_WAVEPRE, A2AMD_WAVEPOST);
+}
+
+unsigned a2amd_osc2_tame_rule(int tame0, int tame1)
+{
+	return a2d_osc2_tame(tame0 != 0, tame1 != 0);
+}
+
+int a2amd_osc2_tame_voices(a2amd_ctx *c, uint64_t *out)
+{
+	if(!c || !out)
+		return A2AMD_EINVAL;
+	use_device(c);
+	unsigned long long n = 0;
+	HIPCHK(c, hipStreamSynchronize(c->stream));
+	HIPCHK(c, hipMemcpy(&n, c->d_tame_count, sizeof(n), hipMemcpyDeviceToHost));
+	*out = n;
+	return A2AMD_OK;
+}
+
 int a2amd_last_batch_fbdpan(const a2amd_ctx *c, a2amd_fbdpan_batch_info *out)
 {
 	if(!c || !out)
diff --git a/audiality2_amd/csrc/a2amd_sched.cpp b/audiality2_amd/csrc/a2amd_sched.cpp
--- a/audiality2_amd/csrc/a2amd_sched.cpp
+++ b/audiality2_amd/csrc/a2amd_sched.cpp
@@ -928,6 +928,7 @@
 	p.waves = c->d_waves.d;
 	p.wavepool = c->d_wavepool.d;
 	p.wavecoef = c->d_wavecoef.d;
+	p.wavecoef4 = c->d_wavecoef4.d;
 	p.busmem = c->d_busmem.d;
 	p.fbdmem = c->d_fbdmem.d;
 	p.ptab = c->d_ptab;
@@ -1587,8 +1588,9 @@
 		pick_fast_shape(c->sw, osc2pan.count, c->nfrags * A2D_FAST_FCH / A2D_OSC2_FCH, &vpw, &ysplit, 16);
 		const int voice_major = !(c->sw.debug & 16);
 		const int lds_taps = !(c->sw.debug & (1 << 17));
+		const int tame = !(c->sw.debug & (1 << 18));
 		if(a2d_launch_leaf_osc2pan(c->d_params, c->hparams, list + osc2pan.first, osc2pan.count,
-				vpw, ysplit, c->d_ustage.d, c->d_staged.d + osc2pan.first, c->stream, &pend.c[pend.n], voice_major, lds_taps, &ysplit))
+				vpw, ysplit, c->d_ustage.d, c->d_staged.d + osc2pan.first, c->stream, &pend.c[pend.n], voice_major, lds_taps, tame, c->d_tame_count, &ysplit))
 			return c->fail(A2AMD_EHIP, "2-osc leaf launch failed: %s", hipGetErrorString(hipGetLastError()));
 		c->last_osc2.launched = 1;
 		c->last_osc2.voices = (uint32_t)osc2pan.count;
diff --git a/audiality2_amd/csrc/a2amd_taps.h b/audiality2_amd/csrc/a2amd_taps.h
--- a/audiality2_amd/csrc/a2amd_taps.h
+++ b/audiality2_amd/csrc/a2amd_taps.h
@@ -127,6 +127,60 @@
 		const unsigned i = (unsigned)(r * 64 + lane);
 		if(i < n)
 			level[i] = src[i];
+	}
+}
+
+typedef int Coef4x __attribute__((ext_vector_type(4)));
+extern "C" __device__ Coef4x a2d_coef4_load(CoefRsrc rsrc, int vindex, int voffset, int soffset, int aux)
+		__asm("llvm.amdgcn.struct.buffer.load.v4i32");
+
+DEV CoefRsrc coef4_rsrc(const int *wavecoef4)
+{
+	const uint64_t b = (uint64_t)wavecoef4;
+	CoefRsrc r;
+	r.x = rfl((int)(unsigned)b);
+	r.y = rfl((int)(((unsigned)(b >> 32) & 0xffffu) | (16u << 16)));
+	r.z = -1;
+	r.w = 0x00020000;
+	return r;
+}
+
+DEV int coef4_base(unsigned doff) { return (int)(doff * 16u); }
+
+DEV Coef4x coef4_at(const CoefRsrc rs, int cb, unsigned ph)
+{
+	return a2d_coef4_load(rs, (int)(ph >> 8), 0, cb, 0);
+}
+
+DEV int mad24(int v, int f, int k)
+{
+	return wadd(__mul24(v, f), k);
+}
+
+DEV int hermite_fused(const Coef4x k, unsigned ph)
+{
+	const int f = (int)(ph & 0xffu);
+	int t = mad24(k.x, f, k.y) >> 8;
+	t = mad24(t, f, k.z) >> 8;
+	return mad24(t, f, k.w) >> 8;
+}
+
+typedef __attribute__((address_space(3))) Coef4x LdsCoef4x;
+DEV Coef4x coef4_lds(const LdsInt *level, unsigned ph, unsigned mask16)
+{
+	typedef __attribute__((address_space(3))) char LdsChar;
+	return *(const LdsCoef4x *)((const LdsChar *)level + ((ph >> 4) & mask16));
+}
+
+DEV void stage_level4(LdsInt *level, const int *wavecoef4, int cb, unsigned size, int lane)
+{
+	const Coef4x *src = (const Coef4x *)(wavecoef4 + ((unsigned)cb >> 2));
+	LdsCoef4x *dst = (LdsCoef4x *)level;
+#pragma unroll
+	for(int r = 0; r < A2D_OSC2_LDS_ENT / 64; ++r) {
+		const unsigned i = (unsigned)(r * 64 + lane);
+		if(i < size)
+			dst[i] = src[i];
 	}
 }
 
diff --git a/audiality2_amd/csrc/a2amd_wavetame.h b/audiality2_amd/csrc/a2amd_wavetame.h
--- /dev/null
+++ b/audiality2_amd/csrc/a2amd_wavetame.h
@@ -0,0 +1,40 @@
+#pragma once
+#include <stdint.h>
+
+#define A2W_TAME_LIM (1 << 24)
+
+static inline int a2w_window_tame(int dm, int d0, int d1, int d2)
+{
+	const int c = (d1 - dm) >> 1;
+	const int a = (3 * (d0 - d1) + d2 - dm) >> 1;
+	const int b = dm - d0 + c - a;
+	const int ma = a < 0 ? -a : a, mb = b < 0 ? -b : b, mc = c < 0 ? -c : c;
+	if((ma + mb + mc + 2) * 255 < A2W_TAME_LIM)
+		return 1;
+	for(int f = 0; f < 256; ++f) {
+		int p = a * f;
+		if(p < -A2W_TAME_LIM || p >= A2W_TAME_LIM)
+			return 0;
+		p = ((p >> 8) + b) * f;
+		if(p < -A2W_TAME_LIM || p >= A2W_TAME_LIM)
+			return 0;
+		p = ((p >> 8) + c) * f;
+		if(p < -A2W_TAME_LIM || p >= A2W_TAME_LIM)
+			return 0;
+	}
+	return 1;
+}
+
+static inline int a2w_level_tame(const int16_t *d, uint32_t size, uint32_t pre, uint32_t post)
+{
+	if(!d || !size || !pre)
+		return 0;
+	const int64_t last = (int64_t)size + (int64_t)post - 3;
+	if(last < 0)
+		return 0;
+	const int16_t *p = d + pre;
+	for(int64_t i = 0; i <= last; ++i)
+		if(!a2w_window_tame(p[i - 1], p[i], p[i + 1], p[i + 2]))
+			return 0;
+	return 1;
+}
diff --git a/audiality2_amd/replay.py b/audiality2_amd/replay.py
--- a/audiality2_amd/replay.py
+++ b/audiality2_amd/replay.py
@@ -221,6 +221,11 @@
         if hasattr(lib, prefix + "osc2_stage_rule"):
             self._osc2_stage_rule = fn("osc2_stage_rule", u32, u32, i32, u32, i32)
             self._wave_level_periodic = fn("wave_level_periodic", i32, C.POINTER(C.c_int16), u32)
+        self._osc2_tame_rule = self._wave_level_tame = None
+        if hasattr(lib, prefix + "osc2_tame_rule"):
+            self._osc2_tame_rule = fn("osc2_tame_rule", u32, i32, i32)
+            self._wave_level_tame = fn("wave_level_tame", i32, C.POINTER(C.c_int16), u32)
+            self._osc2_tame_voices = fn("osc2_tame_voices", i32, vp, C.POINTER(C.c_uint64))
         self._last_batch_fbdpan = None
         if hasattr(lib, prefix + "last_batch_fbdpan"):
             self._last_batch_fbdpan = fn("last_batch_fbdpan", i32, vp, C.POINTER(a2amd_fbdpan_batch_info))
@@ -378,6 +383,25 @@
         if self._osc2_stage_rule is None:
             raise RuntimeError(f"this library has no {self.prefix}osc2_stage_rule")
         return int(self._osc2_stage_rule(size0, int(bool(periodic0)), size1, int(bool(periodic1))))
+
+    def osc2_tame_rule(self, tame0, tame1):
+        if self._osc2_tame_rule is None:
+            raise RuntimeError(f"this library has no {self.prefix}osc2_tame_rule")
+        return int(self._osc2_tame_rule(int(bool(tame0)), int(bool(tame1))))
+
+    def osc2_tame_voices(self):
+        if self._osc2_tame_rule is None:
+            raise RuntimeError(f"this library has no {self.prefix}osc2_tame_voices")
+        n = C.c_uint64(0)
+        self._chk(self._osc2_tame_voices(self.ctx, C.byref(n)), "osc2_tame_voices")
+        return int(n.value)
+
+    def wave_level_tame(self, level, size=None):
+        if self._wave_level_tame is None:
+            raise RuntimeError(f"this library has no {self.prefix}wave_level_tame")
+        arr = np.ascontiguousarray(level, dtype=np.int16)
+        n = len(arr) - WAVEPRE - WAVEPOST if size is None else size
+        return bool(self._wave_level_tame(arr.ctypes.data_as(C.POINTER(C.c_int16)), n))
 
     def wave_level_periodic(self, level):
         if self._wave_level_periodic is None:
diff --git a/include/a2amd.h b/include/a2amd.h
--- a/include/a2amd.h
+++ b/include/a2amd.h
@@ -202,6 +202,7 @@
 #include "a2amd_vmbatch.h"
 #include "a2amd_osc2.h"
 #include "a2amd_osc2lds.h"
+#include "a2amd_osc2tame.h"
 #include "a2amd_osc3filt.h"
 
 #endif
diff --git a/include/a2amd_osc2tame.h b/include/a2amd_osc2tame.h
--- /dev/null
+++ b/include/a2amd_osc2tame.h
@@ -0,0 +1,20 @@
+#ifndef A2AMD_OSC2TAME_H
+#define A2AMD_OSC2TAME_H
+#include <stdint.h>
+
+#ifdef __cplusplus
+extern "C" {
+#endif
+
+struct a2amd_ctx;
+
+int a2amd_wave_level_tame(const int16_t *level, unsigned size);
+
+unsigned a2amd_osc2_tame_rule(int tame0, int tame1);
+
+int a2amd_osc2_tame_voices(struct a2amd_ctx *ctx, uint64_t *out);
+
+#ifdef __cplusplus
+}
+#endif
+#endif
```

Measured after the change: 573.1 billion voice-samples/s, median of 6. 6.8% higher.
